# ebiggers/libdeflate

Hardware: AMD Instinct MI355X
Metric: compress+decompress MB/s, 64 KiB chunks level 6 (higher is better)
Workload: dtype u8

## Files before the change

libdeflate_amd/csrc/deflate_huffman.h:

```cpp

template <int N, typename W = u32> struct huff_scratch {
	W A[N];
	W NW[N];
	W P[N];
	u32 cntI[40];
	u32 cnt[40];
	u32 start[16];
	u32 nc[16];
	u16 S[2 * N];
};

#ifdef LDA_SMALL
typedef huff_scratch<288, u16> huff_litlen_t;
#define HUFF_LITLEN(L) ((huff_litlen_t *)(L)->nxtA)
static_assert(sizeof(((struct deflate_lds *)0)->nxtA) >= sizeof(huff_litlen_t) &&
	      sizeof(((struct deflate_lds *)0)->M) >= 2048 && RING + 1 < 65536,
	      "the staging area holds the litlen tree's scratch, M[] the keys");
#else
typedef huff_scratch<288, u32> huff_litlen_t;
#define HUFF_LITLEN(L) ((huff_litlen_t *)((L)->M + 512))
static_assert(sizeof(((struct deflate_lds *)0)->M) >= 2048 + sizeof(huff_litlen_t),
	      "M[] holds the block-end scratch");
#endif

template <int N, typename W> static __device__ void
make_code(const u32 *freq, u32 n, u32 maxlen, u8 *lens, u16 *codes,
	  u16 *sorted, huff_scratch<N, W> *H, u32 used, bool presorted, u32 lane)
{
	PROF_DECL;
	PROF_START();
	__builtin_amdgcn_s_setprio(3);
	for (u32 s = lane; s < n; s += 64)
		lens[s] = 0;
	if (!presorted) {
		used = 0;
		for (u32 s0 = 0; s0 < n; s0 += 64) {
			u32 s = s0 + lane;
			u32 f = s < n ? freq[s] : 0;
			used += __builtin_popcountll(__ballot(f != 0));
		}
		for (u32 s = lane; s < n; s += 64) {
			u32 f = freq[s];
			if (!f)
				continue;
			u32 key = (f << 9) | s, rank = 0;
			for (u32 t = 0; t < n; t++) {
				u32 ft = freq[t];
				rank += (ft != 0) & (((ft << 9) | t) < key);
			}
			sorted[rank] = (u16)s;
		}
	}
	wave_sync();
	const u32 m = used;
	if (m < 2) {
		if (lane == 0) {
			u32 s = m ? sorted[0] : 0;
			u32 other = s ? 0 : 1;
			lens[s] = 1;
			lens[other] = 1;
			for (u32 d = 0; d < 16; d++)
				H->cnt[d] = 0;
			H->cnt[1] = 2;
		}
		wave_sync();
	} else {
		for (u32 i = lane; i < m; i += 64)
			H->A[i] = freq[sorted[i]];
		if (lane < 40)
			H->cntI[lane] = 0;
		wave_sync();
		if (N == 288) PROF_MARK(13);
		u32 leaf = 0, node = 0, made = 0;
#define MERGE_ROUNDS 40u
		if (m >= 24) {
			const u32 INF = 0x7FFFFFFFu;
			for (u32 round = 0; round < MERGE_ROUNDS && made + 1 < m; round++) {
				const u32 wl0 = leaf < m ? H->A[leaf] : INF;
				const u32 wl1 = leaf + 1 < m ? H->A[leaf + 1] : INF;
				const u32 wn0 = node < made ? H->NW[node] : INF;
				const u32 wn1 = node + 1 < made ? H->NW[node + 1] : INF;
				u32 T = wl0 + wl1;
				T = wl0 + wn0 < T ? wl0 + wn0 : T;
				T = wn0 + wn1 < T ? wn0 + wn1 : T;
				u32 cl = 0;
				for (u32 b0 = leaf; b0 < m; b0 += 64) {
					const u32 i = b0 + lane;
					const u32 c = (u32)__builtin_popcountll(__ballot(i < m && H->A[i] <= T));
					cl += c;
					if (c < 64)
						break;
				}
				u32 cn = made - node;
				if ((cl + cn) & 1) {
					if (cn && (cl == 0 || H->NW[node + cn - 1] >= H->A[leaf + cl - 1]))
						cn--;
					else
						cl--;
				}
				const u32 tot = cl + cn;
				for (u32 k = lane; k < tot; k += 64)
					H->S[k] = 0xFFFF;
				wave_sync();
				const u32 wnode = lane < cn ? H->NW[node + lane] : 0;
				const u32 cn64 = cn < 64 ? cn : 64;
				for (u32 i0 = 0; i0 < cl; i0 += 64) {
					const u32 i = i0 + lane;
					const u32 wv = i < cl ? H->A[leaf + i] : 0;
					u32 r = i;
					for (u32 j = 0; j < cn64; j++)
						r += bcast_lane(wnode, j) < wv;
					for (u32 j = 64; j < cn; j++)
						r += H->NW[node + j] < wv;
					if (i < cl)
						H->S[r] = (u16)i;
				}
				wave_sync();
				u32 nfree = 0;
				for (u32 k0 = 0; k0 < tot; k0 += 64) {
					const u32 k = k0 + lane;
					const bool fr = k < tot && H->S[k] == 0xFFFF;
					const u64 mk = __ballot(fr);
					if (fr)
						H->S[k] = (u16)(0x8000u | (nfree + rank_below(mk)));
					nfree += (u32)__builtin_popcountll(mk);
				}
				wave_sync();
				for (u32 q = lane; q < tot / 2; q += 64) {
					const u32 a = H->S[2 * q], b = H->S[2 * q + 1];
					const u32 wa = a & 0x8000 ? H->NW[node + (a & 0x7FFF)] : H->A[leaf + a];
					const u32 wb = b & 0x8000 ? H->NW[node + (b & 0x7FFF)] : H->A[leaf + b];
					if (a & 0x8000)
						H->P[node + (a & 0x7FFF)] = made + q;
					if (b & 0x8000)
						H->P[node + (b & 0x7FFF)] = made + q;
					H->NW[made + q] = wa + wb;
				}
				wave_sync();
				leaf += cl;
				node += cn;
				made += tot / 2;
			}
		}
		if (lane == 0 && made + 1 < m) {
			u32 wl = leaf < m ? H->A[leaf] : 0xFFFFFFFFu;
			u32 wn = node < made ? H->NW[node] : 0xFFFFFFFFu;
			for (u32 k = made; k + 1 < m; k++) {
				u32 w;
				if (leaf < m && wl <= wn) {
					w = wl;
					leaf++;
					wl = leaf < m ? H->A[leaf] : 0xFFFFFFFFu;
				} else {
					w = wn;
					H->P[node] = k;
					node++;
					wn = node < k ? H->NW[node] : 0xFFFFFFFFu;
				}
				if (leaf < m && wl <= wn) {
					w += wl;
					leaf++;
					wl = leaf < m ? H->A[leaf] : 0xFFFFFFFFu;
				} else {
					w += wn;
					H->P[node] = k;
					node++;
					wn = node < k ? H->NW[node] : 0xFFFFFFFFu;
				}
				H->NW[k] = w;
				if (node == k)
					wn = w;
			}
		}
		wave_sync();
		if (N == 288) PROF_MARK(14);
		{
			const u32 root = m - 2;
			enum { NJ = (N + 63) / 64 };
			u32 dd[NJ], hh[NJ];
#pragma unroll
			for (u32 j = 0; j < NJ; j++) {
				u32 k = lane + 64 * j;
				dd[j] = (k < root) ? 1 : 0;
				hh[j] = (k < root) ? H->P[k] : root;
			}
			wave_sync();
#pragma unroll
			for (u32 j = 0; j < NJ; j++) {
				u32 k = lane + 64 * j;
				if (k <= root) {
					H->NW[k] = dd[j];
					H->A[k] = hh[j];
				}
			}
			wave_sync();
			for (u32 r = 0; r < 6; r++) {
#pragma unroll
				for (u32 j = 0; j < NJ; j++) {
					u32 k = lane + 64 * j;
					if (k <= root) {
						u32 h = H->A[k];
						dd[j] = H->NW[k] + H->NW[h];
						hh[j] = H->A[h];
					}
				}
				wave_sync();
#pragma unroll
				for (u32 j = 0; j < NJ; j++) {
					u32 k = lane + 64 * j;
					if (k <= root) {
						H->NW[k] = dd[j];
						H->A[k] = hh[j];
					}
				}
				wave_sync();
			}
#pragma unroll
			for (u32 j = 0; j < NJ; j++) {
				u32 k = lane + 64 * j;
				if (k <= root)
					atomicAdd((u32 *)&H->cntI[dd[j] < 39 ? dd[j] : 39], 1u);
			}
			wave_sync();
			if (lane < 40)
				H->cnt[lane] = lane ? 2 * H->cntI[lane - 1] - H->cntI[lane] : 0;
			wave_sync();
		}
		if (N == 288) PROF_MARK(15);
		if (lane == 0) {
			u32 over = 0;
			for (u32 d = maxlen + 1; d < 40; d++) {
				over += H->cnt[d];
				H->cnt[maxlen] += H->cnt[d];
				H->cnt[d] = 0;
			}
			if (over) {
				u32 kraft = 0;
				for (u32 d = 1; d <= maxlen; d++)
					kraft += H->cnt[d] << (maxlen - d);
				while (kraft > (1u << maxlen)) {
					u32 d = maxlen - 1;
					while (H->cnt[d] == 0)
						d--;
					H->cnt[d]--;
					H->cnt[d + 1] += 2;
					H->cnt[maxlen]--;
					kraft -= 1;
				}
			}
			u32 at = 0;
			for (u32 d = maxlen; d >= 1; d--) {
				H->start[d] = at;
				at += H->cnt[d];
			}
		}
		wave_sync();
		for (u32 i = lane; i < m; i += 64) {
			u32 d = 1;
			for (u32 q = 2; q <= maxlen; q++)
				if (H->cnt[q] && i >= H->start[q] &&
				    i < H->start[q] + H->cnt[q])
					d = q;
			lens[sorted[i]] = (u8)d;
		}
		wave_sync();
	}
	if (N == 288) PROF_MARK(17);
	if (lane == 0) {
		u32 code = 0;
		H->nc[0] = 0;
		for (u32 d = 1; d < 16; d++) {
			code = (code + (d > 1 ? H->cnt[d - 1] : 0)) << 1;
			H->nc[d] = code;
		}
	}
	wave_sync();
	{
		u32 run[16];
#pragma unroll
		for (u32 d = 1; d < 16; d++)
			run[d] = H->nc[d];
		for (u32 s0 = 0; s0 < n; s0 += 64) {
			u32 s = s0 + lane;
			u32 l = s < n ? lens[s] : 0;
			u32 mycode = 0;
#pragma unroll
			for (u32 d = 1; d < 16; d++) {
				u64 mm = __ballot(l == d);
				if (l == d)
					mycode = run[d] + __builtin_popcountll(mm & ((1ull << lane) - 1));
				run[d] += __builtin_popcountll(mm);
			}
			if (s < n)
				codes[s] = l ? (u16)(__brev(mycode) >> (32 - l)) : 0;
		}
	}
	wave_sync();
	__builtin_amdgcn_s_setprio(0);
}
```

libdeflate_amd/csrc/deflate_kernel.hip:

```cpp
#include <stddef.h>
#include "device_common.h"
#include "kernels.h"


#ifndef NT
#define NT LDA_DEFLATE_THREADS
#endif
#define VPT (1024 / NT)
#define NWAVES (NT / 64)
#ifndef TILE
#define TILE 4096
#endif
#ifndef RING
#define RING 32768u
#endif
#define RMASK (RING - 1)
#define LOOKAHEAD 272u
#ifndef HASH_BITS
#define HASH_BITS 13
#endif
#ifndef HASH3_BITS
#define HASH3_BITS 12
#endif
#define MAX_BLOCK_LEN 65536u
#define TOK_MATCH 0x80000000u
#define TOK_TILE_MAX (TILE + 8)
#define TOK_CAP (MAX_BLOCK_LEN + 2 * TILE + 64)
#define SEQ_GCAP (TOK_CAP / 2)
#define SEQ_STRIDE (SEQ_GCAP + (TILE + 8) / 2 + 320 + 256 + (TILE + 8) / 2)
#define S3_WALK 8
#define S3_EVMIN 1u
#define S3_TAIL 256u
#define S3_CLAIM 24u
#define S3_RA_DEPTH 2u
#define S6_ALWAYS_FLUSH 0
#define S3_HALF_SHIFT 1
#define S3_HALF 1
#define P1_PASSES 0xFFFFFFFFu
#ifdef LDA_SMALL
#define RB_DEFER 0
#define RA_PAIR 0
#else
#define RB_DEFER 1
#define RA_PAIR 1
#endif
#define RB_TAIL_WAVES 8u
static_assert(!RB_DEFER || RB_TAIL_WAVES + 3 <= NWAVES,
	      "wave 0 parses, the last two waves insert: the tail waves lie between them");
#define S3_ROUNDS 1u
#ifndef WQ_CAP
#define WQ_CAP 2048u
#endif
#define WQ_SEG (WQ_CAP / NWAVES)
#define RA_PREF_TAIL NWAVES
#define ABSH(o, pos) (pos)
#define WQ_LIMIT WQ_CAP
#define NXT_ELEMS (2 * WQ_CAP + 8)
#define STG_WORDS (NXT_ELEMS / 2 - 8)

#define M_VALID 0x40000u

struct deflate_lds {
	u8 in[RING + 32];
	u16 prev[RING];
	u16 head[1u << HASH_BITS];
	u16 head3[(1u << HASH3_BITS) + 2];
	u32 M[TILE + 8];
	u64 dhalf[TILE / 64];
	u64 dfull[TILE / 64];
	u8 seen8[256];
	u32 freq[320];
	union {
		struct {
			u8 lens[320];
			u16 codes[320];
			u16 sorted[288];
			u32 hw[288];
			u16 pre_items[320 + 8];
			u32 pre_freq[19];
			u8 pre_lens[20];
			u16 pre_codes[20];
		};
		u16 nxtB[NXT_ELEMS];
	};
	u16 nxtA[NXT_ELEMS] __attribute__((aligned(16)));
	u32 scan[2][NWAVES + 1];
	u32 carry[6];
	u32 obs[1][10];
	u32 vars[24] __attribute__((aligned(16)));
	u64 pm[TILE / 64];
	u64 lit1[TILE / 64];
	u64 lit2[TILE / 64];
	u64 pmA[TILE / 64];
	u64 lit1A[TILE / 64];
	u64 lit2A[TILE / 64];
	u32 qn[4];
	u32 gbase[TILE / 64];
	u32 rdy[TILE / 64 + 1];
	u8 lslot[256];
};

#ifdef __HIP_DEVICE_COMPILE__
#define AS3 __attribute__((address_space(3)))
#else
#define AS3
#endif
typedef AS3 struct deflate_lds lds_t;

#ifdef LDA_SMALL
static_assert(sizeof(struct deflate_lds) <= 163840 / SMALL_WGS, "SMALL_WGS workgroups per CU");
static_assert(RING >= TILE && NXT_ELEMS * 2 >= 3600, "the whole buffer is resident; block-end tables fit nxtB");
#else
static_assert(sizeof(struct deflate_lds) <= 163840, "LDS of one CU");
static_assert(NXT_ELEMS == TILE + 8, "levels 10-12 keep one u16 per position in nxtA");
#endif
static_assert(offsetof(struct deflate_lds, in) == 0, "ld32/ld64 assume in[] at LDS offset 0");
#define PREV_OFF ((u32)offsetof(struct deflate_lds, prev))

enum {
	V_NSEQ = 0, V_ENTRY, V_WALKPOS_LO, V_SPLIT, V_TMP0, V_TMP1, V_TMP2,
	V_TMP3, V_CTR, V_MINLEN, V_NPRE, V_NSEQ_PRE, V_WPOS_PRE, V_FIT, V_UNUSED0,
	V_CTR2, V_PFLAG, V_CTR3, V_STDONE, V_EMDONE, V_TAILDONE, V_CTR4, V_ST2DONE,
	V_COUNT
};
static_assert(V_COUNT <= sizeof(((struct deflate_lds *)0)->vars) / sizeof(u32), "vars[] holds them all");

#define DC_SHALLOW 0
#define DC_HALF 1
#define DC_FULL 2

struct level_params {
	u32 depth;
	u32 nice;
	u32 mode;
};


#define LDS32(byteoff) (*(const __attribute__((address_space(3))) u32 *)(uintptr_t)(byteoff))
#define LDS16(byteoff) (*(const __attribute__((address_space(3))) u16 *)(uintptr_t)(byteoff))

static __device__ __forceinline__ u32 ld32(const AS3 u8 *ring, u32 pos)
{
	(void)ring;
	u32 o = pos & RMASK, i = o & ~3u;
	return __builtin_amdgcn_alignbyte(LDS32(i + 4), LDS32(i), ABSH(o, pos));
}

static __device__ __forceinline__ u64 ld64(const AS3 u8 *ring, u32 pos)
{
	(void)ring;
	u32 o = pos & RMASK, i = o & ~3u;
	u32 a = LDS32(i), b = LDS32(i + 4), c = LDS32(i + 8);
	u32 lo = __builtin_amdgcn_alignbyte(b, a, ABSH(o, pos));
	u32 hi = __builtin_amdgcn_alignbyte(c, b, ABSH(o, pos));
	return ((u64)hi << 32) | lo;
}

static __device__ __forceinline__ u32 hash3(u32 w)
{
	return ((w & 0xFFFFFFu) * 0x1E35A7BDu) >> (32 - HASH3_BITS);
}

static __device__ __forceinline__ u32 hash4(u32 w)
{
	return (w * 0x1E35A7BDu) >> (32 - HASH_BITS);
}

struct deflate_lds;
static __device__ u32
find_len3(const lds_t *L, u32 p, u32 cur, u32 c3_16, u32 dmax,
	  u32 dlim, u32 *best);

static __device__ __forceinline__ bool lane_bit(u64 uniform_mask)
{
	return __builtin_amdgcn_inverse_ballot_w64(uniform_mask);
}

static __device__ __forceinline__ u32 rank_below(u64 uniform_mask)
{
	return __builtin_amdgcn_mbcnt_hi((u32)(uniform_mask >> 32),
					 __builtin_amdgcn_mbcnt_lo((u32)uniform_mask, 0));
}

static __device__ u32 block_scan(lds_t *L, u32 v, u32 *total)
{
	const u32 lane = threadIdx.x & 63, wave = threadIdx.x >> 6;
	u32 incl = wave_scan_incl(v);

	if (lane == 63)
		L->scan[0][wave] = incl;
	__syncthreads();
	const u32 sw = lane < NWAVES ? L->scan[0][lane] : 0;
	const u32 iw = wave_scan_incl(sw);
	const u32 base = bcast_lane(iw - sw, wave);
	__syncthreads();
	*total = bcast_lane(iw, NWAVES - 1);
	return base + incl - v;
}

static __device__ u32 block_scan1(lds_t *L, u32 v, u32 *total,
				  u32 *tog)
{
	const u32 lane = threadIdx.x & 63, wave = threadIdx.x >> 6;
	u32 incl = wave_scan_incl(v);
	u32 *sc = L->scan[*tog];

	*tog ^= 1;
	if (lane == 63)
		sc[wave] = incl;
	__syncthreads();
	const u32 sw = lane < NWAVES ? sc[lane] : 0;
	const u32 iw = wave_scan_incl(sw);
	*total = bcast_lane(iw, NWAVES - 1);
	return bcast_lane(iw - sw, wave) + incl - v;
}

static __device__ __forceinline__ void
length_code(u32 len, u32 *slot, u32 *xbits, u32 *xval)
{
	u32 l = len - 3;
	if (l < 8) {
		*slot = l; *xbits = 0; *xval = 0;
	} else if (len == 258) {
		*slot = 28; *xbits = 0; *xval = 0;
	} else {
		u32 hb = 31 - __builtin_clz(l);
		*xbits = hb - 2;
		*slot = 4 * (hb - 1) + ((l >> (hb - 2)) & 3);
		*xval = l & ((1u << (hb - 2)) - 1);
	}
}

static __device__ __forceinline__ void
dist_code(u32 dist, u32 *slot, u32 *xbits, u32 *xval)
{
	u32 d = dist - 1;
	if (d < 4) {
		*slot = d; *xbits = 0; *xval = 0;
	} else {
		u32 hb = 31 - __builtin_clz(d);
		*xbits = hb - 1;
		*slot = 2 * hb + ((d >> (hb - 1)) & 1);
		*xval = d & ((1u << (hb - 1)) - 1);
	}
}

static __device__ u32 choose_min_len(u32 used_literals, u32 depth)
{
	u32 m = used_literals >= 80 ? 3 : used_literals >= 45 ? 4 :
		used_literals >= 16 ? 5 : used_literals >= 10 ? 6 :
		used_literals >= 8 ? 7 : used_literals >= 6 ? 8 : 9;
	if (depth < 16) {
		u32 cap = depth < 5 ? 4 : depth < 10 ? 5 : 7;
		if (m > cap)
			m = cap;
	}
	return m;
}

static __device__ __forceinline__ u32
min_len_policy(u32 distinct, u32 nbytes, u32 depth, bool use3)
{
	const u32 ml = nbytes < 512 ? 3 : choose_min_len(distinct, depth);

	return use3 || ml > 4 ? ml : 4;
}

static __device__ u32
find_len3(const lds_t *L, u32 p, u32 cur, u32 c3_16, u32 dmax,
	  u32 dlim, u32 *best)
{
	if (dmax > dlim)
		dmax = dlim;
	if (p >= 8) {
		const u64 w8 = ld64(L->in, p - 8);
		const u32 A = (u32)w8, B = (u32)(w8 >> 32);
		const u32 cur3 = cur & 0xFFFFFFu;
		u32 bd = 0;
#define LEN3_TRY(d, hi, lo, sel) bd = __builtin_amdgcn_perm(hi, lo, sel) == cur3 ? (d) : bd
		LEN3_TRY(8, A, A, 0x0C020100u);
		LEN3_TRY(7, A, A, 0x0C030201u);
		LEN3_TRY(6, B, A, 0x0C040302u);
		LEN3_TRY(5, B, A, 0x0C050403u);
		LEN3_TRY(4, B, B, 0x0C020100u);
		LEN3_TRY(3, B, B, 0x0C030201u);
		LEN3_TRY(2, cur, B, 0x0C040302u);
		LEN3_TRY(1, cur, B, 0x0C050403u);
#undef LEN3_TRY
		if (bd && bd <= dmax) {
			*best = 3;
			return bd;
		}
	}
	u32 d = (p - c3_16) & 0xFFFF;
	if (d && d <= dmax && ((ld32(L->in, p - d) ^ cur) & 0xFFFFFFu) == 0) {
		*best = 3;
		return d;
	}
	return 0;
}

static __device__ __forceinline__ u32
token_step(u32 m0, u32 m1, u32 m2, u32 mode, u32 nice)
{
	const u32 l0 = m0 & 0xFFFF, l1 = m1 & 0xFFFF, l2 = m2 & 0xFFFF;
	if (mode == 0)
		return l0 ? l0 : 1;
	const s32 z0 = (s32)__builtin_clz((m0 >> 16) | 1), z1 = (s32)__builtin_clz((m1 >> 16) | 1),
		  z2 = (s32)__builtin_clz((m2 >> 16) | 1);
	const bool lazy = mode >= 1 && l0 < nice;
	const bool c1 = lazy && l1 >= l0 && 4 * (s32)(l1 - l0) + (z1 - z0) > 2;
	const bool c2 = lazy && mode >= 2 && l2 >= l0 && 4 * (s32)(l2 - l0) + (z2 - z0) > 6;
	u32 st = c2 ? 2 : l0;
	st = c1 ? 1 : st;
	return l0 == 0 ? 1 : st;
}

#include "deflate_opt.h"
#include "deflate_huffman.h"


struct outstate {
	u8 *out;
	u64 avail;
	u64 sg;
	u64 bits;
};

static __device__ __forceinline__ u32 *stg_of(lds_t *L)
{
	return (u32 *)L->nxtA;
}

static __device__ __forceinline__ void
stg_put(lds_t *L, const struct outstate *os, u64 bitpos, u64 code,
	u32 nbits)
{
	if (!nbits)
		return;
	u64 rel = bitpos - 8 * os->sg;
	u32 w = (u32)(rel >> 5), s = (u32)rel & 31;
	u32 *stg = stg_of(L);
	u64 lo = code << s;
	atomicOr((u32 *)&stg[w], (u32)lo);
	if (s + nbits > 32)
		atomicOr((u32 *)&stg[w + 1], (u32)(lo >> 32));
	if (s + nbits > 64)
		atomicOr((u32 *)&stg[w + 2], (u32)(code >> (64 - s)));
}

static __device__ __forceinline__ void
stg_flush(lds_t *L, struct outstate *os, bool final)
{
	u32 *stg = stg_of(L);
	u8 *stgb = (u8 *)stg;
	const u32 tid = threadIdx.x;
	u64 done_bytes = final ? (os->bits + 7) / 8 : os->bits / 8;
	u64 rel_end = done_bytes - os->sg;
	s64 first = -(s64)os->sg;
	u32 start = first > 0 ? (u32)first : 0;
	u32 units = final ? (u32)((rel_end + 15) / 16) : (u32)(rel_end / 16);

	__syncthreads();
	for (u32 u = tid; u < units; u += NT) {
		u32 b0 = u * 16, b1 = b0 + 16;
		u8 *g = os->out + (s64)(os->sg + b0);
		if (b0 >= start && b1 <= rel_end) {
			*(uint4 *)g = *(const uint4 *)(stgb + b0);
		} else {
			for (u32 b = b0 < start ? start : b0; b < b1 && b < rel_end; b++)
				g[b - b0] = stgb[b];
		}
	}
	u32 keep_from = units * 16;
	u32 total_words = (u32)((os->bits - 8 * os->sg + 31) / 32) + 1;
	u32 keep_words = final ? 0 : total_words - keep_from / 4;
	u32 v = 0;
	if (tid < keep_words && keep_from / 4 + tid < STG_WORDS + 8)
		v = stg[keep_from / 4 + tid];
	__syncthreads();
	for (u32 i = tid; i < STG_WORDS + 8; i += NT)
		stg[i] = 0;
	if (tid < keep_words)
		stg[tid] = v;
	os->sg += keep_from;
}

static __device__ __forceinline__ void stg_restore(lds_t *L)
{
	u32 *stg = stg_of(L);

	__syncthreads();
	for (u32 i = threadIdx.x; i < STG_WORDS + 8; i += NT)
		stg[i] = i < 6 ? L->carry[i] : 0;
	__syncthreads();
}

static __device__ __forceinline__ void stg_save(lds_t *L, struct outstate *os)
{
	stg_flush(L, os, false);
	if (threadIdx.x < 6)
		L->carry[threadIdx.x] = stg_of(L)[threadIdx.x];
	__syncthreads();
}


static __device__ __forceinline__ u32 lds_mskor_rtn(u32 byteaddr, u32 mask, u32 val)
{
	u32 old;
	asm volatile("ds_mskor_rtn_b32 %0, %1, %2, %3"
		     : "=v"(old) : "v"(byteaddr), "v"(mask), "v"(val) : "memory");
	return old;
}

static __device__ __forceinline__ void lds_wait8(u32 *o)
{
	asm volatile("s_waitcnt lgkmcnt(0)"
		     : "+v"(o[0]), "+v"(o[1]), "+v"(o[2]), "+v"(o[3]),
		       "+v"(o[4]), "+v"(o[5]), "+v"(o[6]), "+v"(o[7]) :: "memory");
}

#define HEAD_OFF ((u32)offsetof(struct deflate_lds, head))
#define HEAD3_OFF ((u32)offsetof(struct deflate_lds, head3))

#define MH_H3_SHIFT 19
#define MH_V3 0x80000000u

static __device__ __forceinline__ void
insert_tile(lds_t *L, u32 t, u32 tend, u32 n, u32 lane)
{
	const u32 ngroups = (tend - t + 63) / 64;

	for (u32 g0 = 0; g0 < ngroups; g0 += 8) {
		u32 o[8], sh[8], wv[8];
#pragma unroll
		for (u32 k = 0; k < 8; k++)
			wv[k] = ld32(L->in, t + (g0 + k) * 64 + lane);
#pragma unroll
		for (u32 k = 0; k < 8; k++) {
			const u32 p = t + (g0 + k) * 64 + lane;
			const u32 h = hash4(wv[k]);
			const bool ok = g0 + k < ngroups && p + 4 <= n;
			sh[k] = (h & 1) << 4;
			o[k] = lds_mskor_rtn(HEAD_OFF + ((h >> 1) << 2),
					     ok ? 0xFFFFu << sh[k] : 0,
					     ok ? (p & 0xFFFF) << sh[k] : 0);
		}
		lds_wait8(o);
#pragma unroll
		for (u32 k = 0; k < 8; k++) {
			const u32 i = (g0 + k) * 64 + lane;
			L->prev[(t + i) & RMASK] = (u16)(o[k] >> sh[k]);
		}
	}
}

static __device__ __forceinline__ void
insert_tile3(lds_t *L, u16 *__restrict__ c3, u32 t, u32 tend, u32 n, u32 lane)
{
	const u32 ngroups = (tend - t + 63) / 64;
	AS3 u16 *const h3tab = (AS3 u16 *)L->head3;

	for (u32 g0 = 0; g0 < ngroups; g0 += 8) {
		u32 wv[8], v[8];
#pragma unroll
		for (u32 k = 0; k < 8; k++)
			wv[k] = ld32(L->in, t + (g0 + k) * 64 + lane);
#pragma unroll
		for (u32 k = 0; k < 8; k++) {
			const u32 p = t + (g0 + k) * 64 + lane;
			const bool ok = g0 + k < ngroups && p + 3 <= n;
			const u32 slot = ok ? hash3(wv[k]) : (1u << HASH3_BITS);
			v[k] = h3tab[slot];
			h3tab[slot] = (u16)p;
			v[k] = ok ? v[k] : 0x8000;
		}
#pragma unroll
		for (u32 k = 0; k < 8; k++)
			c3[4 + (g0 + k) * 64 + lane] = (u16)v[k];
	}
}

static __device__ __forceinline__ u32 claim_issue(u32 lds_byteaddr)
{
	u32 r;
	u64 save;
	asm volatile("s_mov_b64 %1, exec\n\ts_mov_b64 exec, 1\n\tds_add_rtn_u32 %0, %2, %3\n\ts_mov_b64 exec, %1"
		     : "=&v"(r), "=&s"(save) : "v"(lds_byteaddr), "v"(1u) : "memory");
	return r;
}

static __device__ __forceinline__ u32 claim_get(u32 r)
{
	u32 g;
	asm volatile("s_waitcnt lgkmcnt(0)\n\tv_readfirstlane_b32 %0, %1"
		     : "=s"(g) : "v"(r) : "memory");
	return g;
}

static __device__ __forceinline__ void lds_add_lane0(u32 lds_byteaddr, u32 v)
{
	u64 save;
	asm volatile("s_mov_b64 %0, exec\n\ts_mov_b64 exec, 1\n\tds_add_u32 %1, %2\n\ts_mov_b64 exec, %0"
		     : "=&s"(save) : "v"(lds_byteaddr), "v"(v) : "memory");
}
#define VAR_ADDR(idx) ((u32)offsetof(struct deflate_lds, vars) + 4 * (idx))


#define RAW(i, k) LDS32((i) + (k))
#define AB(hi, lo, sh) __builtin_amdgcn_alignbyte((hi), (lo), (sh))
#define HAVE4(a, b, c, d) asm volatile("" :: "v"(a), "v"(b), "v"(c), "v"(d))
static __device__ __forceinline__ u64 mk64(u32 lo, u32 hi)
{
	return ((u64)hi << 32) | lo;
}

static __device__ __forceinline__ u32
match_length(const lds_t *L, bool ev, u32 p, u32 cp, u32 cur, u64 nxt8,
	       u32 maxlen, u32 lane)
{
	(void)L;
	const u32 op = p & RMASK, ip = op & ~3u, sp = op & 3;
	const u32 oc = cp & RMASK, ic = oc & ~3u, sc = oc & 3;
	const u32 b0 = RAW(ic, 0), b1 = RAW(ic, 4), b2 = RAW(ic, 8), b3 = RAW(ic, 12);
	const u64 x = nxt8 ^ mk64(AB(b2, b1, sc), AB(b3, b2, sc));
	u32 len = 4 + ((u32)__builtin_ctzll(x | (1ull << 63)) >> 3);
	ev = ev && AB(b1, b0, sc) == cur;
	bool more = ev && x == 0 && 12 < maxlen;
	if (__ballot(more)) {
		const u32 p3 = RAW(ip, 12), p4 = RAW(ip, 16), p5 = RAW(ip, 20);
		const u32 b4 = RAW(ic, 16), b5 = RAW(ic, 20);
		HAVE4(p3, p5, b4, b5);
		const u64 y = mk64(AB(p4, p3, sp), AB(p5, p4, sp)) ^ mk64(AB(b4, b3, sc), AB(b5, b4, sc));
		if (more) {
			len = 12 + ((u32)__builtin_ctzll(y | (1ull << 63)) >> 3);
			more = y == 0 && 20 < maxlen;
		}
		if (__ballot(more)) {
			const u32 p6 = RAW(ip, 24), p7 = RAW(ip, 28);
			const u32 b6 = RAW(ic, 24), b7 = RAW(ic, 28);
			HAVE4(p6, p7, b6, b7);
			const u64 z = mk64(AB(p6, p5, sp), AB(p7, p6, sp)) ^
				      mk64(AB(b6, b5, sc), AB(b7, b6, sc));
			if (more) {
				len = 20 + ((u32)__builtin_ctzll(z | (1ull << 63)) >> 3);
				more = z == 0 && 28 < maxlen;
			}
		}
	}
	for (u64 mm = __ballot(more); mm; mm &= mm - 1) {
		u32 src = (u32)__builtin_ctzll(mm);
		u32 bp = bcast_lane(p, src);
		u32 bc = bcast_lane(cp, src);
		u32 bmax = bcast_lane(maxlen, src);
		u32 off = 28 + 4 * lane;
		u32 x4 = 1;
		if (off < bmax) {
			const u32 o1 = (bp + off) & RMASK, i1 = o1 & ~3u;
			const u32 o2 = (bc + off) & RMASK, i2 = o2 & ~3u;
			const u32 w0 = RAW(i1, 0), w1 = RAW(i1, 4), v0 = RAW(i2, 0), v1 = RAW(i2, 4);
			x4 = AB(w1, w0, o1 & 3) ^ AB(v1, v0, o2 & 3);
		}
		u64 ne = __ballot(x4 != 0);
		u32 tot = bmax;
		if (ne) {
			u32 kk = (u32)__builtin_ctzll(ne);
			u32 xk = bcast_lane(x4, kk);
			u32 o = 28 + 4 * kk;
			if (o < bmax)
				tot = o + ((u32)__builtin_ctz(xk) >> 3);
		}
		if (lane == src)
			len = tot;
	}
	if (len > maxlen)
		len = maxlen;
	return ev ? len : 0;
}

template <class F> static __device__ __forceinline__ void
match_length2_p(const lds_t *L, bool ev1, bool ev2, u32 p, u32 cp1, u32 cp2, u32 cur,
		u64 nxt8, u32 maxlen, u32 lane, u32 *len1o, u32 *len2o, F &&hook)
{
	(void)L;
	const u32 op = p & RMASK, ip = op & ~3u, sp = op & 3;
	const u32 o1 = cp1 & RMASK, i1 = o1 & ~3u, s1 = o1 & 3;
	const u32 o2 = cp2 & RMASK, i2 = o2 & ~3u, s2 = o2 & 3;
	const u32 b0 = RAW(i1, 0), b1 = RAW(i1, 4), b2 = RAW(i1, 8), b3 = RAW(i1, 12);
	const u32 e0 = RAW(i2, 0), e1 = RAW(i2, 4), e2 = RAW(i2, 8), e3 = RAW(i2, 12);
	hook();
	const u64 x1 = nxt8 ^ mk64(AB(b2, b1, s1), AB(b3, b2, s1));
	const u64 x2 = nxt8 ^ mk64(AB(e2, e1, s2), AB(e3, e2, s2));
	u32 len1 = 4 + ((u32)__builtin_ctzll(x1 | (1ull << 63)) >> 3);
	u32 len2 = 4 + ((u32)__builtin_ctzll(x2 | (1ull << 63)) >> 3);
	ev1 = ev1 && AB(b1, b0, s1) == cur;
	ev2 = ev2 && AB(e1, e0, s2) == cur;
	bool m1 = ev1 && x1 == 0 && 12 < maxlen, m2 = ev2 && x2 == 0 && 12 < maxlen;
	if (__ballot(m1 || m2)) {
		const u32 p3 = RAW(ip, 12), p4 = RAW(ip, 16), p5 = RAW(ip, 20);
		const u32 b4 = RAW(i1, 16), b5 = RAW(i1, 20);
		const u32 e4 = RAW(i2, 16), e5 = RAW(i2, 20);
		HAVE4(p3, p5, b4, b5);
		HAVE4(p4, e4, e5, e5);
		const u64 pw = mk64(AB(p4, p3, sp), AB(p5, p4, sp));
		const u64 y1 = pw ^ mk64(AB(b4, b3, s1), AB(b5, b4, s1));
		const u64 y2 = pw ^ mk64(AB(e4, e3, s2), AB(e5, e4, s2));
		if (m1) {
			len1 = 12 + ((u32)__builtin_ctzll(y1 | (1ull << 63)) >> 3);
			m1 = y1 == 0 && 20 < maxlen;
		}
		if (m2) {
			len2 = 12 + ((u32)__builtin_ctzll(y2 | (1ull << 63)) >> 3);
			m2 = y2 == 0 && 20 < maxlen;
		}
		if (__ballot(m1 || m2)) {
			const u32 p6 = RAW(ip, 24), p7 = RAW(ip, 28);
			const u32 b6 = RAW(i1, 24), b7 = RAW(i1, 28);
			const u32 e6 = RAW(i2, 24), e7 = RAW(i2, 28);
			HAVE4(p6, p7, b6, b7);
			HAVE4(e6, e7, e7, e7);
			const u64 pz = mk64(AB(p6, p5, sp), AB(p7, p6, sp));
			const u64 z1 = pz ^ mk64(AB(b6, b5, s1), AB(b7, b6, s1));
			const u64 z2 = pz ^ mk64(AB(e6, e5, s2), AB(e7, e6, s2));
			if (m1) {
				len1 = 20 + ((u32)__builtin_ctzll(z1 | (1ull << 63)) >> 3);
				m1 = z1 == 0 && 28 < maxlen;
			}
			if (m2) {
				len2 = 20 + ((u32)__builtin_ctzll(z2 | (1ull << 63)) >> 3);
				m2 = z2 == 0 && 28 < maxlen;
			}
		}
	}
#pragma unroll
	for (u32 c = 0; c < 2; c++) {
		const u32 cp = c ? cp2 : cp1;
		for (u64 mm = __ballot(c ? m2 : m1); mm; mm &= mm - 1) {
			u32 src = (u32)__builtin_ctzll(mm);
			u32 bp = bcast_lane(p, src);
			u32 bc = bcast_lane(cp, src);
			u32 bmax = bcast_lane(maxlen, src);
			u32 off = 28 + 4 * lane;
			u32 x4 = 1;
			if (off < bmax) {
				const u32 oa = (bp + off) & RMASK, ia = oa & ~3u;
				const u32 ob = (bc + off) & RMASK, ib = ob & ~3u;
				const u32 w0 = RAW(ia, 0), w1 = RAW(ia, 4), v0 = RAW(ib, 0), v1 = RAW(ib, 4);
				x4 = AB(w1, w0, oa & 3) ^ AB(v1, v0, ob & 3);
			}
			u64 ne = __ballot(x4 != 0);
			u32 tot = bmax;
			if (ne) {
				u32 kk = (u32)__builtin_ctzll(ne);
				u32 xk = bcast_lane(x4, kk);
				u32 o = 28 + 4 * kk;
				if (o < bmax)
					tot = o + ((u32)__builtin_ctz(xk) >> 3);
			}
			if (lane == src) {
				if (c)
					len2 = tot;
				else
					len1 = tot;
			}
		}
	}
	if (len1 > maxlen)
		len1 = maxlen;
	if (len2 > maxlen)
		len2 = maxlen;
	*len1o = ev1 ? len1 : 0;
	*len2o = ev2 ? len2 : 0;
}

static __device__ __forceinline__ u32
wave_distinct_bytes(lds_t *L, u32 t0, u32 lim, u32 lane)
{
	AS3 u32 *const s32p = (AS3 u32 *)L->seen8;

	s32p[lane] = 0;
	wave_sync();
#pragma unroll
	for (u32 j = 0; j < TILE / 1024; j++) {
		const u32 off = (TILE / 64) * lane + 16 * j;
		const uint4 v = *(const AS3 uint4 *)&L->in[(t0 + off) & RMASK];
		const u32 w[4] = { v.x, v.y, v.z, v.w };
#pragma unroll
		for (u32 i = 0; i < 16; i++)
			if (off + i < lim)
				L->seen8[(w[i >> 2] >> (8 * (i & 3))) & 0xFF] = 1;
	}
	wave_sync();
	return wave_sum((u32)__builtin_popcount(s32p[lane] & 0x01010101u));
}

static __device__ __forceinline__ void
stage_input(lds_t *L, const u8 *__restrict__ inp, u32 loaded, u32 want,
	    bool aligned_in, u32 tid)
{
	if (aligned_in) {
		const u32 from = loaded & ~15u;
		for (u32 p = from + tid * 16; p < want; p += NT * 16) {
			uint4 v = *(const uint4 *)(inp + p);
			*(uint4 *)&L->in[p & RMASK] = v;
			if ((p & RMASK) < 32)
				*(uint4 *)&L->in[RING + (p & RMASK)] = v;
		}
// ... 608 lines not shown
								bestd = m >> 16;
							}
						} else {
							dep = my_i >= TILE - S3_TAIL ? drain : depth;
						}
						best0 = best;
						boff = best - 3;
						curb = boff ? ld32(L->in, p + boff) : cur;
						dprev = 0;
						cnt = 0;
						ended = false;
						have = true;
						if (best >= maxlen) {
							have = false;
							fin = true;
						}
					} else {
						fin = true;
						best = best0 = 3;
					}
				}
			}
			PROF_SEC(0);
			continue;
		}
#pragma unroll
		for (int s = 0; s < S3_WALK; s++) {
			u32 d = (p - c16) & 0xFFFF;
			bool chain = dep && d > dprev && d <= dmaxp;
			bool stall = ended || cnt >= 4;
			bool ok = !stall && chain;
			u32 cp = p - d;
			u32 w = ld32(L->in, cp + boff);
			u32 c16n = LDS16(PREV_OFF + 2 * (cp & RMASK));
			bool hit = ok && w == curb;
			c16 = ok ? c16n : c16;
			dprev = ok ? d : dprev;
			dep -= ok ? 1 : 0;
			ended = ended || (!stall && !chain);
			q = hit ? ((q << 16) | d) : q;
			cnt += hit ? 1 : 0;
		}
		if (!have)
			cnt = 0;
		PROF_SEC(1);
		bool done = false;
		u32 nev = __builtin_popcountll(__ballot(cnt > 0));
		u32 nwalk = __builtin_popcountll(__ballot(have && !ended && cnt < 4));
		while (nev && (nev >= S3_EVMIN || !nwalk)) {
			bool ev = cnt > 0;
			u32 d = (u32)(q >> (16 * ((cnt - 1) & 3))) & 0xFFFF;
			cnt -= ev ? 1 : 0;
			u32 len = match_length(L, ev, p, p - d, cur, nxt8, maxlen, lane);
			if (ev && len > best) {
				best = len;
				bestd = d;
				if (len >= nice || len >= maxlen) {
					done = true;
					cnt = 0;
				} else {
					boff = len - 3;
					curb = ld32(L->in, p + boff);
				}
			}
			if (have && (done || (ended && cnt == 0))) {
				have = false;
				fin = true;
				done = false;
			}
			nev = __builtin_popcountll(__ballot(cnt > 0));
			nwalk = __builtin_popcountll(__ballot(have && !ended && cnt < 4));
		}
		if (have && ended && cnt == 0) {
			have = false;
			fin = true;
		}
		PROF_SEC(2);
	}
	PROF_SEC_FLUSH(17);
}

#ifdef LDA_PROFILE
#define PROF_GEN(g) do { if (threadIdx.x == 0) { unsigned long long n_ = __builtin_readcyclecounter(); \
	atomicAdd(&lda_prof[35 + ((g) < 3 ? (g) : 3)], n_ - pg_); pg_ = n_; } } while (0)
#else
#define PROF_GEN(g) do { } while (0)
#endif
static __device__ __forceinline__ u32 rb_trim_depth(u32 depth)
{
	const u32 npass = depth >= 256 ? 4 : depth >= 32 ? 2 : 1;
	const u32 quantum = 8 * npass;
	for (u32 g = 1, end = quantum; end < depth; g++, end += quantum * g)
		if (depth - end <= depth / 8)
			depth = end;
	if (depth >= 16 && (depth & 7) <= depth / 8)
		depth &= ~7u;
	return depth;
}

static __device__ __forceinline__ void
rb_gen_params(u32 depth, u32 gen, u32 *before, u32 *npass_g)
{
	const u32 npass = depth >= 256 ? 4 : depth >= 32 ? 2 : 1;
	const u32 quantum = 8 * npass;
	*npass_g = npass * (gen + 1);
	*before = quantum * (gen * (gen + 1) / 2);
}

static __device__ __forceinline__ bool
rb_batch(lds_t *L, u32 t, u32 n, u32 lo_pos, u32 min_len, u32 depth, u32 nice,
	 u32 e, bool have, u32 gen, u32 lane, u32 *next)
{
	const u32 half = depth >> S3_HALF_SHIFT ? depth >> S3_HALF_SHIFT : 1;
	u32 before, npass_g;
	rb_gen_params(depth, gen, &before, &npass_g);
	const u32 qg = 8 * npass_g;
	const u32 i = e & 0xFFF, p = t + i;
	const u32 cdepth = ((e >> 12) & 3) == DC_FULL ? depth : half;
	u32 dep = before < cdepth ? cdepth - before : 0;
	dep = dep < qg ? dep : qg;
	u32 dprev = gen ? (p - (e >> 16)) & 0xFFFF : 0;
	u32 c16 = LDS16(PREV_OFF + 2 * ((p - dprev) & RMASK));
	const u32 m = L->M[4 + i], l0 = m & 0xFFFF;
	const u32 cur = ld32(L->in, p);
	const u64 nxt8 = ld64(L->in, p + 4);
	const u32 maxlen = n - p < 258 ? n - p : 258;
	const u32 dmaxp = p - lo_pos;
	const u32 nic = nice < maxlen ? nice : maxlen;
	u32 best = l0 >= 4 ? l0 : 3, bestd = l0 >= 4 ? m >> 16 : 0;
	const u32 best0 = best;
	u32 boff = best - 3;
	u32 curb = ld32(L->in, p + boff);
	bool act = have && p + 4 <= n && best < nic && dep;
	u64 endm = 0;
	for (u32 ps = 0; ps < npass_g; ps++) {
		u64 h1 = 0, h2 = 0;
		u32 qh = 0, nok = 0;
		const u32 dep0 = dep;
		const u64 actm = __ballot(act);
#pragma unroll
		for (int s = 0; s < 8; s++) {
			u32 d, c16x2;
			asm("v_sub_u16 %0, %1, %2" : "=v"(d) : "v"(p), "v"(c16));
			if (RING == 32768u)
				asm("v_lshlrev_b16 %0, 1, %1" : "=v"(c16x2) : "v"(c16));
			else
				c16x2 = 2 * (c16 & RMASK);
			const u64 chainm = __ballot(dep0 > (u32)s) & __ballot(d > dprev) &
					   __ballot(d <= dmaxp);
			const u64 stallm = endm | h2;
			const u64 okm = actm & ~stallm & chainm;
			const u32 w = ld32(L->in, c16 + boff);
			const u32 c16n = LDS16(PREV_OFF + c16x2);
			const u64 hitm = okm & __ballot(w == curb);
			const bool ok = lane_bit(okm);
			c16 = ok ? c16n : c16;
			dprev = ok ? d : dprev;
			nok = ok ? (u32)s + 1 : nok;
			endm |= actm & ~stallm & ~chainm;
			qh = lane_bit(hitm) ? ((qh << 16) | d) : qh;
			h2 |= h1 & hitm;
			h1 |= hitm;
			PROF_COUNT(20, __builtin_popcountll(okm));
			PROF_COUNT(17, __builtin_popcountll(hitm));
		}
		PROF_COUNT(13, __builtin_popcountll(__ballot(have)));
		PROF_COUNT(21, (h1 != 0) + (h2 != 0));
		dep = dep0 - nok;
		if (h1) {
			const bool ev = lane_bit(h1);
			const u32 d = lane_bit(h2) ? qh >> 16 : qh & 0xFFFF;
			const u32 len = match_length(L, ev, p, p - d, cur, nxt8, maxlen, lane);
			if (ev && len > best) {
				best = len;
				bestd = d;
			}
		}
		if (h2) {
			const bool ev = lane_bit(h2);
			const u32 d = qh & 0xFFFF;
			const u32 len = match_length(L, ev, p, p - d, cur, nxt8, maxlen, lane);
			if (ev && len > best) {
				best = len;
				bestd = d;
			}
		}
		if (best >= nic)
			act = false;
		if (npass_g > 1) {
			if (!__ballot(act && !lane_bit(endm) && dep))
				break;
			boff = best - 3;
			curb = ld32(L->in, p + boff);
		}
	}
	const bool ended = lane_bit(endm);
	if (best > best0)
		L->M[4 + i] = best >= min_len ? best | (bestd << 16) : 0;
	*next = (e & 0x3FFF) | (((p - dprev) & 0xFFFF) << 16);
	return act && !ended && before + qg < cdepth;
}

static __device__ __forceinline__ void
search_queue(lds_t *L, u32 t, u32 n, u32 lo_pos, u32 min_len, u32 depth,
	     u32 nice, AS3 u32 *WA, AS3 u32 *WB, u32 wc, u32 tid,
	     bool defer, u32 *tail_n, u32 *tail_gen, AS3 u32 **tail_list)
{
	const u32 lane = tid & 63, wave = tid >> 6;
	depth = rb_trim_depth(depth);
	const u64 lt = (1ull << lane) - 1;
	u32 ncur = wc;
#ifdef LDA_PROFILE
	unsigned long long pg_ = __builtin_readcyclecounter();
#endif

	*tail_n = 0;
	PROF_COUNT(15, wc);
	PROF_COUNT(18, 1);
	for (u32 gen = 0;; gen++) {
		PROF_COUNT(16, 1);
		PROF_COUNT(14, (ncur + 63) / 64);
		PROF_COUNT(19, ncur);
		AS3 u32 *cur_l = gen & 1 ? WB : WA, *nxt_l = gen & 1 ? WA : WB;
		AS3 u32 *ctr = &L->qn[gen % 3];
		u32 before, npass_g;
		rb_gen_params(depth, gen, &before, &npass_g);
		if (RB_DEFER && defer && gen && before + 8 * npass_g >= depth &&
		    ncur <= 64 * RB_TAIL_WAVES) {
			*tail_n = ncur;
			*tail_gen = gen;
			*tail_list = cur_l;
			return;
		}
		if (tid == 0)
			L->qn[(gen + 1) % 3] = 0;
		for (u32 base = 64 * wave; base < ncur; base += 64 * NWAVES) {
			const bool have = base + lane < ncur;
			const u32 e = have ? cur_l[base + lane] : 0;
			u32 nx;
			const bool surv = rb_batch(L, t, n, lo_pos, min_len, depth, nice, e, have,
						   gen, lane, &nx);
			const u64 b = __ballot(surv);
			u32 at = 0;
			if (lane == 0 && b)
				at = atomicAdd((u32 *)ctr, (u32)__builtin_popcountll(b));
			at = bcast_first(at);
			if (surv)
				nxt_l[at + __builtin_popcountll(b & lt)] = nx;
		}
		__syncthreads();
		PROF_GEN(gen);
		ncur = bcast_first(*(volatile AS3 u32 *)ctr);
		if (!ncur)
			break;
	}
}

static __device__ __forceinline__ void
split_stats(lds_t *L, u32 walkpos, u32 block_start, bool fit_split, u32 lane)
{
	static_assert(TOK_TILE_MAX < (1u << 13) && TOK_CAP < (1u << 17), "32-bit products");
	AS3 u32 *const acc = (AS3 u32 *)&L->scan[1][0];
	if (lane < 10)
		acc[lane] = 0;
	wave_sync();
#pragma unroll
	for (u32 j = 0; j < 4; j++)
		atomicAdd((u32 *)&acc[2 * j + (lane & 1)], L->freq[lane + 64 * j]);
	if (lane < 29)
		atomicAdd((u32 *)&acc[8 + (lane >= 6)], L->freq[257 + lane]);
	wave_sync();
	const u32 now = lane < 10 ? acc[lane] : 0;
	const u32 prev = lane < 10 ? L->obs[0][lane] : 0;
	const u32 d = now - prev;
	const u32 nprev = row16_sum(prev), nnew = row16_sum(d);
	const u32 a = d * nprev, e = prev * nnew;
	const u32 df = a > e ? a - e : e - a;
	const u64 delta = ((u64)row16_sum(df >> 16) << 16) + row16_sum(df & 0xFFFF);
	bool sp = nprev && walkpos - block_start >= 5000 &&
		  delta >= (u64)nnew * 200 / 512 * nprev;
	if (fit_split && walkpos - block_start >= 5000)
		sp = true;
	wave_sync();
	if (lane < 10)
		L->obs[0][lane] = sp ? 0 : now;
	if (lane == 0)
		L->vars[V_SPLIT] = !sp ? 0 :
			L->vars[V_WPOS_PRE] - block_start >= 5000 ? 2 : 1;
}

#ifdef LDA_DEBUG_SPLIT
static __device__ u32 lda_dbg[2048];
extern "C" __attribute__((visibility("default"))) void libdeflate_amd_debug_read(u32 *out)
{
	(void)hipDeviceSynchronize();
	(void)hipMemcpyFromSymbol(out, HIP_SYMBOL(lda_dbg), sizeof(lda_dbg));
}
#define DBG(tile, k, v) do { if ((tile) < 250) lda_dbg[8 * (tile) + (k)] = (v); } while (0)
#else
#define DBG(tile, k, v) do { } while (0)
#endif


template <bool OPT> static __device__ __forceinline__ void
deflate_batch_body(u8 *lds_raw, u64 n_chunks, int format, int level, u32 depth,
		   u32 nice, u32 mode,
		   const u8 *__restrict__ in_base,
		   const u64 *__restrict__ in_offsets,
		   const u64 *__restrict__ in_nbytes,
		   u8 *__restrict__ out_base,
		   const u64 *__restrict__ out_offsets,
		   const u64 *__restrict__ out_avail_arr,
		   u64 *__restrict__ out_nbytes,
		   const u32 *__restrict__ sums,
		   u64 *__restrict__ seq_scratch,
		   const u32 *__restrict__ seg_info,
		   u32 *__restrict__ next_chunk,
		   const u8 *__restrict__ dict_pre)
{
	lds_t *L = (lds_t *)(uintptr_t)0;
	const u32 tid = threadIdx.x;
	if ((u32)(uintptr_t)(__attribute__((address_space(3))) u8 *)lds_raw != 0)
		__builtin_trap();
	u64 *__restrict__ seqg = seq_scratch + (size_t)blockIdx.x * SEQ_STRIDE;
	u32 *__restrict__ tokg = (u32 *)seqg;
	u32 *__restrict__ msave = (u32 *)(seqg + SEQ_GCAP);
	u32 *__restrict__ fsave = msave + TILE + 8;
	u32 *__restrict__ bsave = fsave + 640;
	u16 *__restrict__ c3g = (u16 *)(bsave + 512);
	u32 tog = 0;
	PROF_DECL;

	for (u32 i = tid; i < 256; i += NT) {
		u32 sl, xb, xv;
		length_code(i + 3, &sl, &xb, &xv);
		L->lslot[i] = (u8)sl;
	}
	for (;;) {
		__syncthreads();
		if (tid == 0)
			L->vars[V_TMP0] = atomicAdd(next_chunk, 1u);
		__syncthreads();
		const u64 c = bcast_first(L->vars[V_TMP0]);
		if (c >= n_chunks)
			break;
		const u8 *inp = in_base + in_offsets[c];
		u64 n64 = in_nbytes[c];
		const u32 sinfo = dict_pre ? (n64 ? ((const u32 *)dict_pre)[0] : 0x80000000u) :
				  seg_info ? seg_info[c] : 0x80000000u;
		const u32 dict_len = sinfo & 0xFFFFu;
		const u32 lo_min = (sinfo >> 16) & 0x7FFFu;
		const bool seg_last = sinfo >> 31;
		const u32 pre_len = dict_pre ? dict_len : 0;
		inp -= pre_len;
		n64 += pre_len;
		struct outstate os;
		os.out = out_base + out_offsets[c];
		os.avail = out_avail_arr[c];
		const u32 hdr_bytes = format == LDA_FMT_GZIP ? 10 :
				      format == LDA_FMT_ZLIB ? (dict_pre ? 6 : 2) : 0;
		const u32 ftr_bytes = format == LDA_FMT_GZIP ? 8 :
				      format == LDA_FMT_ZLIB ? 4 : 0;
		bool overflow = false;

		if (os.avail <= hdr_bytes + ftr_bytes && (hdr_bytes + ftr_bytes))
			overflow = true;
		if (n64 > 0xFFFFFF00u)
			overflow = true;
#ifdef LDA_SMALL
		if (n64 > RING)
			overflow = true;
#endif
		const u32 n = (u32)n64;

		__syncthreads();
		PROF_START();
		for (u32 i = tid; i < (1u << HASH_BITS) / 2; i += NT)
			((u32 *)L->head)[i] = 0x80008000u;
		for (u32 i = tid; i < (1u << HASH3_BITS) / 2; i += NT)
			((u32 *)L->head3)[i] = 0x80008000u;
		for (u32 i = tid; i < 320; i += NT)
			L->freq[i] = 0;
		if (tid < 10)
			L->obs[0][tid] = 0;
		if (tid < TILE / 64 + 1)
			L->rdy[tid] = 0;
		for (u32 i = tid; i < STG_WORDS + 8; i += NT)
			stg_of(L)[i] = 0;
		if (tid < 8)
			L->M[tid] = 0;
		if (tid == 0) {
			L->vars[V_NSEQ] = 0;
			L->vars[V_ENTRY] = 0;
			L->vars[V_PFLAG] = 0;
		}
		os.sg = (u64)(0 - ((uintptr_t)os.out & 15));
		os.bits = 0;
		__syncthreads();

		if (!overflow && hdr_bytes) {
			if (tid == 0) {
				if (format == LDA_FMT_GZIP) {
					u32 xfl = level < 2 ? 4 : level >= 8 ? 2 : 0;
					stg_put(L, &os, 0, 0x00088B1Full, 32);
					stg_put(L, &os, 32, 0, 32);
					stg_put(L, &os, 64, xfl | (0xFFu << 8), 16);
				} else {
					u32 fl = level < 2 ? 0 : level < 6 ? 1 :
						 level < 8 ? 2 : 3;
					u32 h = (0x78u << 8) | (fl << 6);
					if (dict_pre) {
						h |= 0x20;
						h += (31 - h % 31) % 31;
						stg_put(L, &os, 16, __builtin_bswap32(((const u32 *)dict_pre)[1]), 32);
					} else {
						h |= 31 - (h % 31);
					}
					stg_put(L, &os, 0, ((h & 0xFF) << 8) | (h >> 8), 16);
				}
			}
			os.bits = 8 * hdr_bytes;
		}
		__syncthreads();
		stg_save(L, &os);

		u32 loaded = 0;
		u32 block_start = dict_len;
		u32 walkpos = dict_len;
		const bool aligned_in = ((uintptr_t)inp & 15) == 0;

		const bool stored_only = level == 0 ||
			n - dict_len <= (u32)(55 - 4 * (level > 12 ? 12 : level));
		u32 num_tiles = (n + TILE - 1) / TILE;
		if (num_tiles == 0)
			num_tiles = 1;
		if (pre_len && !stored_only && !overflow) {
			stage_prefix(L, dict_pre + 64, pre_len, tid);
			loaded = pre_len;
		}

		const bool ra_all = depth <= 4;
		const bool optm = OPT && mode == 3;
		const u32 rounds = optm || ra_all ? 0 : S3_ROUNDS;
		const u32 dlim3 = mode ? 8192u : 4096u;
		const u32 ra_depth = ra_all ? depth : S3_RA_DEPTH;
		const u32 ra_class = ra_all ? DC_FULL :
				     ra_depth >= (depth >> S3_HALF_SHIFT) ? DC_HALF : DC_SHALLOW;
		const u32 wq_limit = mode == 1 && depth < 100 && WQ_LIMIT > 64 * NWAVES ?
				     64 * NWAVES : WQ_LIMIT;
		const bool use3 = level >= 2;
		const bool splits = use3 && n - dict_len >= 5000;
		bool mx_pending = false;
		u32 tail_n = 0, tail_gen = 0, tail_e = 0;
		u32 ml_cur = 3, ml_nxt = 3;
		u32 carryv = 0;

		for (u32 it = 0; it <= num_tiles && !overflow; it++) {
			const bool have_cur = it >= 1;
			const u32 tile = it - 1;
			const u32 t = have_cur ? tile * TILE : 0;
			const u32 tend = t + TILE < n ? t + TILE : n;
			const bool last_tile = it == num_tiles;
			const bool cur_real = have_cur && t >= dict_len;
			const u32 tn = it * TILE;
			const u32 tnend = tn + TILE < n ? tn + TILE : n;
			const bool nxt_real = it < num_tiles && tn >= dict_len;
			const bool have_ins = it + 1 < num_tiles;
			u32 tid_opaque = threadIdx.x;
			asm volatile("" : "+v"(tid_opaque));
			const u32 tid = tid_opaque, lane = tid & 63, wave = tid >> 6;

			PROF_MARK(0);
			if (stored_only) {
				if (!cur_real)
					continue;
				walkpos = tend;
			} else {
				AS3 u32 *const MX = (AS3 u32 *)L->nxtB;
#ifdef LDA_SMALL
				const u32 lo_cur = 0, lo_nxt = 0;
				(void)lo_min;
#else
				const s32 lo_s = (s32)(t + 2 * TILE + LOOKAHEAD) - (s32)RING;
				const u32 lo_cur = lo_s > (s32)lo_min ? (u32)lo_s : lo_min;
				const s32 lo_n = (s32)(tn + 2 * TILE + LOOKAHEAD) - (s32)RING;
				const u32 lo_nxt = lo_n > (s32)lo_min ? (u32)lo_n : lo_min;
#endif
				u16 *c3nxt = c3g + (it & 1) * (TILE + 8);
				u16 *c3ins = c3g + ((it + 1) & 1) * (TILE + 8);
				const s32 limit = last_tile ? (s32)(tend - t) : (s32)TILE - 2;

				const bool wl_copies = cur_real && !optm && rounds && mx_pending;
				if (cur_real) {
					if (mx_pending && !wl_copies)
						for (u32 i = tid; i < TILE; i += NT)
							L->M[4 + i] = MX[4 + i];
					if (tid < 4) {
						L->M[tid] = carryv;
						L->M[TILE + 4 + tid] = 0;
					}
					mx_pending = false;
					ml_cur = ml_nxt;
					for (u32 i = tid; i < 320; i += NT)
						fsave[i] = L->freq[i];
					if (tid == 0) {
						L->vars[V_NSEQ_PRE] = L->vars[V_NSEQ];
						L->vars[V_WPOS_PRE] = walkpos;
					}
					if (!wl_copies)
						__syncthreads();
					PROF_MARK(6);
				}
				const u32 s0_want0 = (it + 2) * TILE + LOOKAHEAD;
				const u32 s0_want = s0_want0 < n ? s0_want0 : n;
				const u32 s0_p = (loaded & ~15u) + tid * 16;
				const bool s0_pre = aligned_in && s0_p < s0_want;
				uint4 s0_v = make_uint4(0, 0, 0, 0);
				if (s0_pre)
					s0_v = *(const uint4 *)(inp + s0_p);
				tail_n = 0;
				if (cur_real && !optm) {
					if (rounds) {
						const u32 wc = build_worklist(L, (AS3 u32 *)L->nxtB,
									      wl_copies ? (const AS3 u32 *)MX : NULL,
									      mode, nice, wq_limit, tid);
						PROF_MARK(39);
						if (wc) {
							AS3 u32 *tl = (AS3 u32 *)L->nxtB;
							search_queue(L, t, n, lo_cur, ml_cur, depth, nice,
								     (AS3 u32 *)L->nxtB, (AS3 u32 *)L->nxtA, wc, tid,
								     nxt_real, &tail_n, &tail_gen, &tl);
							if (tail_n && wave >= 1 && wave <= RB_TAIL_WAVES) {
								const u32 k = 64 * (wave - 1) + lane;
								tail_e = k < tail_n ? tl[k] : 0;
							}
						}
						PROF_MARK(3);
					}
					if (!tail_n)
						stage_steps(L, limit, mode, nice, tid);
				}
				if (cur_real && optm) {
					const bool opt_first = walkpos == block_start;
					const u32 opt_last = level >= 11 ? 2 : 1;
					u32 opt_stage = 0;
					const u32 ent0 = L->vars[V_ENTRY], nseq0 = L->vars[V_NSEQ];
					if (opt_first) {
						for (u32 i = tid; i < TILE + 8; i += NT)
							msave[i] = L->M[i];
						if (tid == 0)
							L->vars[V_FIT] = 0;
					} else {
						const u32 fit = opt_build_costs(L, tid, false, true, t, tend - t, bsave);
						opt_stage = fit ? 0 : 1;
						if (tid == 0) {
							L->vars[V_FIT] = fit;
							if (c == 0) {
								DBG(tile, 6, 100 + fit);
								DBG(tile, 7, L->vars[V_TMP3]);
							}
						}
					}
					for (;;) {
						u32 tid_opaque2 = threadIdx.x;
						asm volatile("" : "+v"(tid_opaque2));
						const u32 tid = tid_opaque2, lane = tid & 63, wave = tid >> 6;
						const u32 s4mode = opt_stage ? 0 : 2;
						if (opt_stage) {
							const s32 ent = (s32)ent0;
							const s32 pend = (s32)(tend - t);
							s32 lo = (s32)(OPT_SEG * wave), hi = lo + OPT_SEG;
							if (wave == 0 && ent < 0)
								lo = ent;
							if (hi > limit)
								hi = limit;
							s32 e = hi + OPT_WARM;
							if (e > pend)
								e = pend;
							if (lo < hi)
								opt_parse_wave(L, L->nxtA, t, lo, hi, e, lane);
							__syncthreads();
							for (s32 i = (s32)tid + (ent < 0 ? ent : 0); i < limit; i += NT) {
								u32 c = L->nxtA[i + 4], m = L->M[i + 4];
								L->M[i + 4] = c >= 3 ? c | (m & 0xFFFF0000u) : 0;
							}
							__syncthreads();
						}
						stage_steps(L, limit, s4mode, nice, tid);
						if (tid == 0)
							L->vars[V_CTR2] = 0;
						__syncthreads();
						if (wave == 0)
							parse_and_base(L, tokg, t, limit, s4mode, nice, lane);
						__syncthreads();
						PROF_MARK(12);
						emit_groups(L, tokg, t, lane);
						__syncthreads();
						PROF_MARK(5);
						if (!opt_first || opt_stage == opt_last)
							break;
						opt_build_costs(L, tid, opt_stage == 0, false, t, tend - t, bsave);
						for (u32 i = tid; i < 320; i += NT)
							L->freq[i] = 0;
						for (u32 i = tid; i < TILE + 8; i += NT)
							L->M[i] = msave[i];
						if (tid == 0) {
							L->vars[V_ENTRY] = ent0;
							L->vars[V_NSEQ] = nseq0;
						}
						__syncthreads();
						opt_stage++;
					}
				}

				{
					const u32 want = s0_want;
					if (s0_pre) {
						*(uint4 *)&L->in[s0_p & RMASK] = s0_v;
						if ((s0_p & RMASK) < 32)
							*(uint4 *)&L->in[RING + (s0_p & RMASK)] = s0_v;
					}
					if (aligned_in) {
						if ((loaded & ~15u) + NT * 16 < want)
							stage_input(L, inp, (loaded & ~15u) + NT * 16, want, true, tid);
					} else {
						stage_input(L, inp, loaded, want, false, tid);
					}
					loaded = want > loaded ? want : loaded;
					if (tid == 0) {
						L->vars[V_CTR] = 0;
						L->vars[V_CTR2] = 0;
						L->vars[V_CTR3] = 0;
						L->vars[V_STDONE] = 0;
						L->vars[V_EMDONE] = 0;
						L->vars[V_TAILDONE] = 0;
						L->vars[V_CTR4] = 0;
						L->vars[V_ST2DONE] = 0;
					}
					if (tid < 4 && nxt_real) {
						AS3 u32 *const Mo = cur_real ? MX : (AS3 u32 *)L->M;
						if (!tail_n)
							Mo[tid] = cur_real ? L->M[TILE + tid] : 0;
						Mo[TILE + 4 + tid] = 0;
					}
					if (nxt_real && it)
						ml_nxt = bcast_first(L->vars[V_MINLEN]);
					__syncthreads();
				}
				PROF_MARK(1);
				if (it == 0) {
					if (wave == NWAVES - 1)
						insert_tile(L, 0, tnend, n, lane);
					if (wave == NWAVES - 2 && use3) {
						insert_tile3(L, c3nxt, 0, tnend, n, lane);
						__builtin_amdgcn_fence(__ATOMIC_RELEASE, "workgroup");
					}
					if (wave == NWAVES - 3 && nxt_real) {
						const u32 nd = wave_distinct_bytes(L, 0, loaded < TILE ? loaded : TILE, lane);
						if (lane == 0)
							L->vars[V_MINLEN] = min_len_policy(nd, n - dict_len, depth, use3);
					}
					__syncthreads();
					if (nxt_real)
						ml_nxt = bcast_first(L->vars[V_MINLEN]);
					PROF_MARK(2);
				}
				__builtin_amdgcn_fence(__ATOMIC_ACQUIRE, "workgroup");

				{
					const bool do_p2 = cur_real && !optm;
					AS3 u32 *const Mo = cur_real ? MX : (AS3 u32 *)L->M;
					PROF_WDECL;
					PROF_W0();
					if (wave == NWAVES - 1) {
						__builtin_amdgcn_s_setprio(3);
						if (have_ins)
							insert_tile(L, tnend, tnend + TILE < n ? tnend + TILE : n,
								    n, lane);
						__builtin_amdgcn_s_setprio(0);
						PROF_W(24);
					} else if (wave == NWAVES - 2) {
						__builtin_amdgcn_s_setprio(2);
						if (have_ins && use3) {
							insert_tile3(L, c3ins, tnend,
								     tnend + TILE < n ? tnend + TILE : n, n, lane);
							__builtin_amdgcn_fence(__ATOMIC_RELEASE, "workgroup");
						}
						__builtin_amdgcn_s_setprio(0);
						if (have_ins && tnend >= dict_len) {
							const u32 nd = wave_distinct_bytes(L, tnend,
								loaded - tnend < TILE ? loaded - tnend : TILE, lane);
							if (lane == 0)
								L->vars[V_MINLEN] = min_len_policy(nd, n - dict_len, depth, use3);
						}
						PROF_W(25);
					} else if (wave == 0 && do_p2) {
						if (tail_n)
							wait_lds_eq(L, V_ST2DONE, TILE / 64);
						__builtin_amdgcn_s_setprio(3);
						parse_and_base(L, tokg, t, limit, mode, nice, lane);
						__builtin_amdgcn_fence(__ATOMIC_RELEASE, "workgroup");
						if (lane == 0)
							*(volatile AS3 u32 *)&L->vars[V_PFLAG] = it;
						__builtin_amdgcn_s_setprio(0);
						if (tail_n && nxt_real && lane < 4)
							Mo[lane] = L->M[TILE + lane];
						PROF_W(26);
					} else if (RB_DEFER && tail_n && wave <= RB_TAIL_WAVES) {
						__builtin_amdgcn_s_setprio(2);
						if (64 * (wave - 1) < tail_n) {
							u32 nx;
							(void)rb_batch(L, t, n, lo_nxt, ml_cur, rb_trim_depth(depth), nice,
								       tail_e, tail_e != 0, tail_gen, lane, &nx);
						}
						__builtin_amdgcn_fence(__ATOMIC_RELEASE, "workgroup");
						if (lane == 0)
							atomicAdd((u32 *)&L->vars[V_TAILDONE], 1u);
						wait_lds_eq(L, V_TAILDONE, RB_TAIL_WAVES);
						stage_steps_cur_claimed(L, limit, mode, nice, lane);
						__builtin_amdgcn_s_setprio(0);
					}
					if (nxt_real) {
						if (optm) {
							if (wave < NWAVES - 2)
								search_items(L, Mo, tn, n, lo_nxt, ml_nxt, depth, nice,
									     NULL, TILE, NWAVES - 2, tid);
						} else {
							round_a(L, Mo, c3nxt, tn, tnend, n, lo_nxt, ml_nxt, ra_depth,
								ra_class, nice, dlim3, it + 1, tid);
						}
					}
					if (wave == 1)
						PROF_W(27);
					if (nxt_real && rounds) {
						const s32 lim_n = it + 1 == num_tiles ? (s32)(tnend - tn) : (s32)TILE - 2;
						stage_steps_claimed(L, Mo, lim_n, mode, nice, it + 1, lane);
						if (wave == 0) {
							u64 mk;
							wait_lds_eq(L, V_STDONE, TILE / 64);
							const u32 e = entry_skip(Mo, (s32)L->vars[V_ENTRY],
										 (u32)(lim_n + 4), mode, nice);
							(void)parse_tile(Mo, (const AS3 u64 *)L->lit1A,
									 (const AS3 u64 *)L->lit2A, (AS3 u64 *)L->pmA,
									 lane, (s32)e - 4, lim_n, &mk, P1_PASSES);
						}
						if (wave == 1)
							PROF_W(33);
						if (wave == 0)
							PROF_W(34);
					}
					if (do_p2) {
						while (*(volatile AS3 u32 *)&L->vars[V_PFLAG] != it)
							__builtin_amdgcn_s_sleep(4);
						__builtin_amdgcn_fence(__ATOMIC_ACQUIRE, "workgroup");
						if (wave == 1)
							PROF_W(28);
						emit_groups(L, tokg, t, lane);
						if (wave == 1)
							PROF_W(29);
						if (wave == NWAVES - 1 && splits && !last_tile) {
							wait_lds_eq(L, V_EMDONE, TILE / 64);
							split_stats(L, bcast_first(L->vars[V_WALKPOS_LO]), block_start, false, lane);
						}
					}
					__syncthreads();
					if (wave == 1)
						PROF_W(30);
					if (wave == 0)
						PROF_W(31);
					if (optm && nxt_real) {
						PROF_MARK(16);
						if (ml_nxt <= 3) {
							for (u32 i = tid; i < TILE; i += NT) {
								u32 p = tn + i, b3 = 0;
								if (p + 3 <= n && Mo[4 + i] == 0) {
									u32 bd = find_len3(L, p, ld32(L->in, p),
											   c3nxt[4 + i], p - lo_nxt,
											   dlim3, &b3);
									if (bd)
										Mo[4 + i] = 3 | (bd << 16);
								}
							}
						}
						__syncthreads();
					}
					mx_pending = cur_real && nxt_real;
				}
				PROF_MARK(4);
				if (!cur_real)
					continue;

				if (OPT && mode == 3)
					walkpos = bcast_first(L->vars[V_WALKPOS_LO]);
				if (tid < 4)
					carryv = L->M[TILE + tid];
				if (splits && wave == NWAVES - 1 && optm) {
					split_stats(L, walkpos, block_start, L->vars[V_FIT] == 2, lane);
				}
			}
			if (OPT && mode == 3)
				__syncthreads();
			PROF_MARK(32);

			u32 splitv, nseq_now;
			if (OPT && mode == 3) {
				splitv = splits && !stored_only && !last_tile ?
					 bcast_first(L->vars[V_SPLIT]) : 0;
				nseq_now = stored_only ? 0 : bcast_first(L->vars[V_NSEQ]);
			} else {
				const uint4 pv = *(const AS3 uint4 *)&L->vars[V_NSEQ];
				static_assert(V_NSEQ == 0 && V_WALKPOS_LO == 2 && V_SPLIT == 3, "one 16-byte read");
				if (!stored_only)
					walkpos = bcast_first(pv.z);
				splitv = splits && !stored_only && !last_tile ? bcast_first(pv.w) : 0;
				nseq_now = stored_only ? 0 : bcast_first(pv.x);
			}
			bool end_block = last_tile || splitv ||
				(!stored_only && nseq_now + 2 * TOK_TILE_MAX > TOK_CAP) ||
				walkpos - block_start > MAX_BLOCK_LEN;
			if (!end_block)
				continue;
			if (tid < 10)
				L->obs[0][tid] = 0;

			const bool retro = splitv == 2;
			const u32 bstart = block_start;
			const u32 bend = last_tile ? n : retro ? bcast_first(L->vars[V_WPOS_PRE]) : walkpos;
			const u32 blen = bend - bstart;
			const u32 nseq_all = nseq_now;
			const u32 nseq = retro ? bcast_first(L->vars[V_NSEQ_PRE]) : nseq_all;
			const u32 is_final = last_tile && seg_last ? 1 : 0;
			if (retro) {
				for (u32 i = tid; i < 320; i += NT) {
					u32 f = L->freq[i], fp = fsave[i];
					fsave[320 + i] = f - fp;
					L->freq[i] = fp;
				}
				__syncthreads();
			}

			u32 btype = 0;
			if (!stored_only) {
				if (mx_pending) {
					const AS3 u32 *MXs = (const AS3 u32 *)L->nxtB;
					for (u32 i = tid; i < TILE; i += NT)
						msave[4 + i] = MXs[4 + i];
				}
				if (tid == 0)
					L->freq[256]++;
				__syncthreads();
				{
					u32 *keys = L->M;
					u32 *usedv = L->M + 320;
					u16 *sortedO = (u16 *)(L->M + 324);
					if (tid < 2)
						usedv[tid] = 0;
					__syncthreads();
					for (u32 vt = tid; vt < 320; vt += NT) {
						const u32 f = L->freq[vt];
						if (f) {
							if (vt < 288)
								keys[atomicAdd(&usedv[0], 1u)] = (f << 9) | vt;
							else
								keys[288 + atomicAdd(&usedv[1], 1u)] =
									(f << 9) | (vt - 288);
						}
					}
					__syncthreads();
					{
						const u32 m1 = usedv[0], m2 = usedv[1];
						for (u32 i = tid; i < m1 + m2; i += NT) {
							const bool lit = i < m1;
							const u32 lo = lit ? 0 : 288, m = lit ? m1 : m2;
							const u32 key = keys[lit ? i : 288 + i - m1];
							u32 r = 0;
							for (u32 q = 0; q < m; q++)
								r += keys[lo + q] < key;
							if (lit)
								L->sorted[r] = (u16)(key & 511);
							else
								sortedO[r] = (u16)(key & 511);
						}
					}
					__syncthreads();
					PROF_MARK(10);
					if (wave == 0)
						make_code(L->freq, 288, 15, L->lens, L->codes,
							  L->sorted, HUFF_LITLEN(L),
							  usedv[0], true, lane);
					else if (wave == 1)
						make_code(L->freq + 288, 32, 15, L->lens + 288,
							  L->codes + 288, sortedO,
							  (huff_scratch<32> *)L->hw,
							  usedv[1], true, lane);
				}
				__syncthreads();
				PROF_MARK(11);
				{
					u32 *starts = L->M;
					if (tid == 0) {
						L->vars[V_TMP1] = 257;
						L->vars[V_TMP2] = 1;
					}
					if (tid < 19)
						L->pre_freq[tid] = 0;
					__syncthreads();
					for (u32 vt = tid; vt < 320; vt += NT) {
						if (vt < 288 && vt >= 257 && L->lens[vt])
							atomicMax((u32 *)&L->vars[V_TMP1], vt + 1);
						if (vt >= 288 && L->lens[vt])
							atomicMax((u32 *)&L->vars[V_TMP2], vt - 288 + 1);
					}
					__syncthreads();
					const u32 nlit = L->vars[V_TMP1], noff = L->vars[V_TMP2];
					const u32 total = nlit + noff;
					u32 isst[VPT], nst = 0;
#pragma unroll
					for (u32 j = 0; j < VPT; j++) {
						const u32 e = tid * VPT + j;
						isst[j] = 0;
						if (e < total) {
							u32 v = L->lens[e < nlit ? e : 288 + (e - nlit)];
							u32 pv = 0xFF;
							if (e)
								pv = L->lens[e - 1 < nlit ? e - 1 :
									     288 + (e - 1 - nlit)];
							isst[j] = pv != v;
						}
						nst += isst[j];
					}
					u32 nruns;
					u32 ridx = block_scan(L, nst, &nruns);
#pragma unroll
					for (u32 j = 0; j < VPT; j++) {
						if (isst[j])
							starts[ridx] = tid * VPT + j;
						ridx += isst[j];
					}
					if (tid == 0)
						starts[nruns] = total;
					__syncthreads();
					u32 rv[VPT], rlen[VPT], nitems[VPT], nit = 0;
#pragma unroll
					for (u32 j = 0; j < VPT; j++) {
						const u32 r = tid * VPT + j;
						rv[j] = rlen[j] = nitems[j] = 0;
						if (r < nruns) {
							u32 st = starts[r];
							rlen[j] = starts[r + 1] - st;
							rv[j] = L->lens[st < nlit ? st : 288 + (st - nlit)];
							if (rv[j] == 0) {
								u32 full = rlen[j] / 138, rem = rlen[j] % 138;
								nitems[j] = full + (rem >= 3 ? 1 : rem);
							} else if (rlen[j] >= 4) {
								u32 l1 = rlen[j] - 1;
								nitems[j] = 1 + l1 / 6 + (l1 % 6 >= 3 ? 1 : l1 % 6);
							} else {
								nitems[j] = rlen[j];
							}
						}
						nit += nitems[j];
					}
					u32 ni;
					u32 at = block_scan(L, nit, &ni);
#pragma unroll
					for (u32 j = 0; j < VPT; j++) {
						if (tid * VPT + j < nruns) {
							u32 left = rlen[j];
							const u32 rvj = rv[j];
							if (rvj == 0) {
								while (left >= 11) {
									u32 r = left > 138 ? 138 : left;
									L->pre_items[at++] = 18 | ((r - 11) << 5);
									atomicAdd((u32 *)&L->pre_freq[18], 1u);
									left -= r;
								}
								if (left >= 3) {
									L->pre_items[at++] = 17 | ((left - 3) << 5);
									atomicAdd((u32 *)&L->pre_freq[17], 1u);
									left = 0;
								}
							} else if (left >= 4) {
								L->pre_items[at++] = (u16)rvj;
								left--;
								u32 n16 = 0;
								while (left >= 3) {
									u32 r = left > 6 ? 6 : left;
									L->pre_items[at++] = 16 | ((r - 3) << 5);
									n16++;
									left -= r;
								}
								atomicAdd((u32 *)&L->pre_freq[16], n16);
								atomicAdd((u32 *)&L->pre_freq[rvj], 1u);
							}
							if (left)
								atomicAdd((u32 *)&L->pre_freq[rvj], left);
							while (left) {
								L->pre_items[at++] = (u16)rvj;
								left--;
							}
						}
					}
					if (tid == 0)
						L->vars[V_NPRE] = ni;
				}
				__syncthreads();
				PROF_MARK(23);
				if (wave == 0)
					make_code(L->pre_freq, 19, 7, L->pre_lens, L->pre_codes,
						  L->sorted, (huff_scratch<32> *)L->hw,
						  0, false, lane);
				__syncthreads();
				PROF_MARK(22);
				u32 dyn = 0, stat = 0;
				for (u32 vt = tid; vt < 320; vt += NT) {
					u32 f = L->freq[vt];
					u32 xb = 0, sl = 8;
					if (vt < 288) {
						sl = vt < 144 ? 8 : vt < 256 ? 9 : vt < 280 ? 7 : 8;
						if (vt >= 265 && vt < 285)
							xb = (vt - 261) >> 2;
					} else {
						u32 ds = vt - 288;
						sl = 5;
						if (ds >= 4)
							xb = (ds >> 1) - 1;
					}
					dyn += f * (L->lens[vt] + xb);
					stat += f * (sl + xb);
				}
				if (tid < 19) {
					u32 xb = tid == 16 ? 2 : tid == 17 ? 3 : tid == 18 ? 7 : 0;
					dyn += L->pre_freq[tid] * (L->pre_lens[tid] + xb);
				}
				u32 dyn_tot, stat_tot;
				(void)block_scan(L, dyn, &dyn_tot);
				(void)block_scan(L, stat, &stat_tot);
				static const u8 perm[19] = { 16, 17, 18, 0, 8, 7, 9, 6, 10,
							     5, 11, 4, 12, 3, 13, 2, 14,
							     1, 15 };
				u32 nexp = 19;
				while (nexp > 4 && L->pre_lens[perm[nexp - 1]] == 0)
					nexp--;
				u32 cost_dyn = 3 + 5 + 5 + 4 + 3 * nexp + dyn_tot;
				u32 cost_stat = 3 + stat_tot;
				u32 pieces = blen ? (blen + 65534) / 65535 : 1;
				u32 pad = (u32)((0 - (os.bits + 3)) & 7);
				u64 cost_stored = 3 + pad + 32 + 8ull * blen +
						  (u64)(pieces - 1) * 40;
				u64 best = cost_stored;
				btype = 0;
				if (cost_stat < best) {
					best = cost_stat;
					btype = 1;
				}
				if (cost_dyn < best) {
					best = cost_dyn;
					btype = 2;
				}
				if ((os.bits + best + 7) / 8 + ftr_bytes > os.avail)
					overflow = true;
				L->vars[V_TMP3] = nexp;
			} else {
				u32 pieces = blen ? (blen + 65534) / 65535 : 1;
				u64 cost = (u64)pieces * 40 + 8ull * blen;
				if ((os.bits + cost + 7) / 8 + ftr_bytes > os.avail)
					overflow = true;
			}
			if (overflow)
				break;

			PROF_MARK(7);
			stg_restore(L);
			if (btype == 0) {
				u32 done = 0;
				do {
					u32 piece = blen - done > 65535 ? 65535 : blen - done;
					u32 fin = (is_final && done + piece == blen) ? 1 : 0;
					u32 pad = (u32)((0 - (os.bits + 3)) & 7);
					if (tid == 0) {
						stg_put(L, &os, os.bits, fin, 3);
						u64 b = os.bits + 3 + pad;
						stg_put(L, &os, b, piece | ((u64)(piece ^ 0xFFFF) << 16), 32);
					}
					os.bits += 3 + pad + 32;
					__syncthreads();
					for (u32 w0 = 0; w0 < piece; w0 += 2048) {
						u32 cnt = piece - w0 < 2048 ? piece - w0 : 2048;
						stg_flush(L, &os, false);
						__syncthreads();
						for (u32 j = tid; j < cnt; j += NT) {
							u32 pos = bstart + done + w0 + j;
							stg_put(L, &os, os.bits + 8ull * j, inp[pos], 8);
						}
						os.bits += 8ull * cnt;
						__syncthreads();
					}
					done += piece;
				} while (done < blen);
				stg_flush(L, &os, false);
			} else {
				if (btype == 1) {
					__syncthreads();
					for (u32 s = tid; s < 320; s += NT)
						L->lens[s] = s < 144 ? 8 : s < 256 ? 9 :
							     s < 280 ? 7 : s < 288 ? 8 : 5;
					__syncthreads();
					if (tid == 0) {
						u32 nc[16] = { 0 }, bl[16] = { 0 };
						for (u32 s = 0; s < 288; s++)
							bl[L->lens[s]]++;
						u32 code = 0;
						for (u32 d = 1; d < 16; d++) {
							code = (code + bl[d - 1]) << 1;
							nc[d] = code;
						}
						for (u32 s = 0; s < 288; s++) {
							u32 l = L->lens[s];
							L->codes[s] = (u16)(__brev(nc[l]++) >> (32 - l));
						}
						for (u32 s = 0; s < 32; s++)
							L->codes[288 + s] = (u16)(__brev(s) >> 27);
					}
					__syncthreads();
				}
				{
					u64 hcode[VPT];
					u32 hbits[VPT], hsum = 0;
					const u32 nexp = btype == 2 ? L->vars[V_TMP3] : 0;
					const u32 ni = btype == 2 ? L->vars[V_NPRE] : 0;
#pragma unroll
					for (u32 j = 0; j < VPT; j++) {
						const u32 vt = tid * VPT + j;
						hcode[j] = 0;
						hbits[j] = 0;
						if (vt == 0) {
							hcode[j] = is_final | (btype << 1);
							hbits[j] = 3;
							if (btype == 2) {
								u32 nlit = L->vars[V_TMP1], noff = L->vars[V_TMP2];
								hcode[j] |= (u64)((nlit - 257) | ((noff - 1) << 5) |
										  ((nexp - 4) << 10)) << 3;
								hbits[j] = 17;
							}
						} else if (vt <= nexp) {
							static const u8 perm2[19] = { 16, 17, 18, 0, 8, 7,
								9, 6, 10, 5, 11, 4, 12, 3, 13, 2, 14, 1, 15 };
							hcode[j] = L->pre_lens[perm2[vt - 1]];
							hbits[j] = 3;
						} else if (vt <= nexp + ni) {
							u32 it = L->pre_items[vt - nexp - 1];
							u32 sym = it & 31, ex = it >> 5;
							u32 l = L->pre_lens[sym];
							u32 xb = sym == 16 ? 2 : sym == 17 ? 3 :
								 sym == 18 ? 7 : 0;
							hcode[j] = L->pre_codes[sym] | ((u64)ex << l);
							hbits[j] = l + xb;
						}
						hsum += hbits[j];
					}
					u32 htot;
					u32 hoff = block_scan(L, hsum, &htot);
#pragma unroll
					for (u32 j = 0; j < VPT; j++) {
						stg_put(L, &os, os.bits + hoff, hcode[j], hbits[j]);
						hoff += hbits[j];
					}
					os.bits += htot;
				}
				stg_flush(L, &os, false);

				PROF_MARK(9);
				__builtin_amdgcn_fence(__ATOMIC_ACQUIRE, "workgroup");
				u32 tok_nxt = tid < nseq ? tokg[tid] : 0;
				for (u32 b0 = 0; b0 < nseq; b0 += NT) {
					u64 code = 0;
					u32 nb = 0;
					const u32 tok = tok_nxt;
					if (b0 + NT + tid < nseq)
						tok_nxt = tokg[b0 + NT + tid];
					if (b0 + tid < nseq) {
						if (tok & TOK_MATCH) {
							const u32 len = (tok & 0xFF) + 3, dist = ((tok >> 8) & 0x7FFF) + 1;
							u32 sl, xb, xv, ds, dxb, dxv;
							length_code(len, &sl, &xb, &xv);
							dist_code(dist, &ds, &dxb, &dxv);
							u32 ll = L->lens[257 + sl];
							u32 dl = L->lens[288 + ds];
							u64 v = L->codes[257 + sl];
							u32 sh = ll;
							v |= (u64)xv << sh;
							sh += xb;
							v |= (u64)L->codes[288 + ds] << sh;
							sh += dl;
							v |= (u64)dxv << sh;
							sh += dxb;
							code = v;
							nb = sh;
						} else {
							code = L->codes[tok];
							nb = L->lens[tok];
						}
					}
					u32 tot;
					u32 off = block_scan1(L, nb, &tot, &tog);
					stg_put(L, &os, os.bits + off, code, nb);
					os.bits += tot;
					if (S6_ALWAYS_FLUSH || os.bits - 8 * os.sg + 48 * NT + 64 > 32 * STG_WORDS)
						stg_flush(L, &os, false);
				}
				stg_flush(L, &os, false);
				__syncthreads();
				if (tid == 0)
					stg_put(L, &os, os.bits, L->codes[256], L->lens[256]);
				os.bits += L->lens[256];
				__syncthreads();
			}

			stg_save(L, &os);
			PROF_MARK(8);
			if (OPT && mode == 3 && tid < 256)
				bsave[tid] = 0;
			if (retro) {
				const u32 cnt = nseq_all - nseq;
				enum { RPT = (TOK_TILE_MAX + NT - 1) / NT };
				u32 mv[RPT];
#pragma unroll
				for (u32 k = 0; k < RPT; k++)
					mv[k] = tid + NT * k < cnt ? tokg[nseq + tid + NT * k] : 0;
				__syncthreads();
#pragma unroll
				for (u32 k = 0; k < RPT; k++)
					if (tid + NT * k < cnt)
						tokg[tid + NT * k] = mv[k];
				for (u32 i = tid; i < 320; i += NT)
					L->freq[i] = fsave[320 + i];
				if (tid == 0)
					L->vars[V_NSEQ] = cnt;
				__builtin_amdgcn_fence(__ATOMIC_RELEASE, "workgroup");
			} else {
				for (u32 i = tid; i < 320; i += NT)
					L->freq[i] = 0;
				if (tid == 0)
					L->vars[V_NSEQ] = 0;
			}
			carryv = 0;
			if (mx_pending) {
				for (u32 i = tid; i < TILE; i += NT)
					L->M[4 + i] = msave[4 + i];
				mx_pending = false;
			}
			block_start = bend;
			__syncthreads();
		}

		__syncthreads();
		if (!overflow && !seg_last &&
		    (os.bits + 3 + 7) / 8 + 4 > os.avail)
			overflow = true;
		if (!overflow) {
			stg_restore(L);
			if (!seg_last) {
				u64 fb = 8 * ((os.bits + 3 + 7) / 8);
				if (tid == 0)
					stg_put(L, &os, fb, 0xFFFF0000ull, 32);
				os.bits = fb + 32;
				__syncthreads();
			}
			if (ftr_bytes) {
				u32 sum = sums ? sums[c] : 0;
				u64 fb = 8 * ((os.bits + 7) / 8);
				if (tid == 0) {
					if (format == LDA_FMT_GZIP) {
						stg_put(L, &os, fb, sum, 32);
						stg_put(L, &os, fb + 32, n, 32);
					} else {
						stg_put(L, &os, fb, __builtin_bswap32(sum), 32);
					}
				}
				os.bits = fb + 8 * ftr_bytes;
				__syncthreads();
			}
			stg_flush(L, &os, true);
			if (tid == 0)
				out_nbytes[c] = (os.bits + 7) / 8;
		} else if (tid == 0) {
			out_nbytes[c] = 0;
		}
		__syncthreads();
	}
}

#define DEFLATE_KERNEL_PARAMS                                                  \
	u64 n_chunks, int format, int level, u32 depth, u32 nice, u32 mode,    \
	const u8 *__restrict__ in_base, const u64 *__restrict__ in_offsets,    \
	const u64 *__restrict__ in_nbytes, u8 *__restrict__ out_base,          \
	const u64 *__restrict__ out_offsets,                                   \
	const u64 *__restrict__ out_avail_arr, u64 *__restrict__ out_nbytes,   \
	const u32 *__restrict__ sums, u64 *__restrict__ seq_scratch,           \
	const u32 *__restrict__ seg_info, u32 *__restrict__ next_chunk,       \
	const u8 *__restrict__ dict_pre
#define DEFLATE_KERNEL_ARGS                                                    \
	lds_raw, n_chunks, format, level, depth, nice, mode, in_base,          \
	in_offsets, in_nbytes, out_base, out_offsets, out_avail_arr,           \
	out_nbytes, sums, seq_scratch, seg_info, next_chunk, dict_pre

#ifdef LDA_SMALL
extern "C" __global__ void __launch_bounds__(NT, SMALL_WGS)
lda_deflate_small_kernel(DEFLATE_KERNEL_PARAMS)
{
	extern __shared__ __attribute__((aligned(16))) u8 lds_raw[];
	deflate_batch_body<false>(DEFLATE_KERNEL_ARGS);
}

extern "C" size_t lda_deflate_small_lds_bytes(void)
{
	return sizeof(struct deflate_lds);
}

extern "C" size_t lda_deflate_small_max(void)
{
	return RING;
}

extern "C" size_t lda_deflate_small_wgs(void)
{
	return SMALL_WGS;
}

LDA_PROF_DEFINE_READER(libdeflate_amd_profile_read_deflate_small)
#else
extern "C" __global__ void __launch_bounds__(NT)
lda_deflate_batch_kernel(DEFLATE_KERNEL_PARAMS)
{
	extern __shared__ __attribute__((aligned(16))) u8 lds_raw[];
	deflate_batch_body<false>(DEFLATE_KERNEL_ARGS);
}

extern "C" __global__ void __launch_bounds__(NT)
lda_deflate_opt_kernel(DEFLATE_KERNEL_PARAMS)
{
	extern __shared__ __attribute__((aligned(16))) u8 lds_raw[];
	deflate_batch_body<true>(DEFLATE_KERNEL_ARGS);
}

extern "C" size_t lda_deflate_lds_bytes(void)
{
	return sizeof(struct deflate_lds);
}

extern "C" size_t lda_deflate_tile(void)
{
	return TILE;
}

extern "C" size_t lda_deflate_seq_words(void)
{
	return SEQ_STRIDE;
}

LDA_PROF_DEFINE_READER(libdeflate_amd_profile_read_deflate)

#endif
```

libdeflate_amd/csrc/host_compress.hip:

```cpp
#include <stdio.h>
#include <stdlib.h>
#include <string.h>
#include <atomic>
#include <new>
#include <algorithm>
#include <vector>

#include "host_objects.h"
#include "kernels.h"

namespace lda {
bool pick_allocator(const struct libdeflate_options *options,
		    malloc_func_t *m, free_func_t *f);
}
using namespace lda;

struct level_cfg { uint32_t depth, nice, mode; };
static const level_cfg k_levels[13] = {
	{ 0, 0, 0 },
	{ 2, 32, 0 },
	{ 6, 10, 0 },
	{ 12, 14, 0 },
	{ 16, 30, 0 },
	{ 16, 30, 1 },
	{ 35, 65, 1 },
	{ 100, 130, 1 },
	{ 300, 258, 2 },
	{ 600, 258, 2 },
	{ 150, 258, 3 },
	{ 300, 258, 3 },
	{ 2000, 258, 3 },
};

extern "C" LIBDEFLATEAPI struct libdeflate_compressor *
libdeflate_alloc_compressor_ex(int level, const struct libdeflate_options *options)
{
	malloc_func_t m;
	free_func_t f;

	if (!pick_allocator(options, &m, &f))
		return NULL;
	if (level == -1)
		level = 6;
	if (level < 0 || level > 12)
		return NULL;
	if (!device_ctx()) {
		fprintf(stderr, "libdeflate_amd: alloc_compressor: no usable "
			"gfx950 device (%s); no CPU fallback\n",
			libdeflate_amd_last_error());
		return NULL;
	}
	void *mem = m(sizeof(struct libdeflate_compressor));
	if (!mem)
		return NULL;
	struct libdeflate_compressor *c = new (mem) libdeflate_compressor();
	c->free_func = f;
	c->malloc_func = m;
	c->level = level;
	c->device = 0;
	(void)hipGetDevice(&c->device);
	for (int k = 0; k < LDA_MAX_SHARDS; k++)
		c->shard[k] = NULL;
	return c;
}

extern "C" LIBDEFLATEAPI struct libdeflate_compressor *
libdeflate_alloc_compressor(int level)
{
	return libdeflate_alloc_compressor_ex(level, NULL);
}

extern "C" LIBDEFLATEAPI void
libdeflate_free_compressor(struct libdeflate_compressor *c)
{
	if (!c)
		return;
	for (int k = 0; k < LDA_MAX_SHARDS; k++)
		libdeflate_free_compressor(c->shard[k]);
	DeviceGuard on(c->device);
	c->scratch.release();
	c->stage.release();
	c->pinned.release();
	c->meta.release();
	c->streams.release();
	free_func_t f = c->free_func;
	c->~libdeflate_compressor();
	f(c);
}

extern "C" LIBDEFLATEAPI size_t
libdeflate_deflate_compress_bound(struct libdeflate_compressor *c, size_t n)
{
	(void)c;
	size_t blocks = (n + 4999) / 5000;
	if (blocks < 1)
		blocks = 1;
	return 5 * blocks + n;
}

extern "C" LIBDEFLATEAPI size_t
libdeflate_zlib_compress_bound(struct libdeflate_compressor *c, size_t n)
{
	return 6 + libdeflate_deflate_compress_bound(c, n);
}

extern "C" LIBDEFLATEAPI size_t
libdeflate_gzip_compress_bound(struct libdeflate_compressor *c, size_t n)
{
	return 18 + libdeflate_deflate_compress_bound(c, n);
}

static size_t dict_window(void)
{
	const size_t tile = lda_deflate_tile();
	return (32768 - 2 * tile - 272) / tile * tile;
}

struct dict_shape { uint32_t tail, pre_len, sinfo; };

static dict_shape shape_dict(int level, size_t dict_nbytes)
{
	const size_t tile = lda_deflate_tile();
	dict_shape d;
	d.tail = level == 0 ? 0 : (uint32_t)std::min(dict_nbytes, dict_window());
	d.pre_len = (uint32_t)((d.tail + tile - 1) / tile * tile);
	d.sinfo = d.pre_len | ((d.pre_len - d.tail) << 16) | 0x80000000u;
	return d;
}

static int
compress_batch_impl(struct libdeflate_compressor *c, int format, size_t n,
		    const void *d_in, const uint64_t *d_in_offsets,
		    const uint64_t *d_in_nbytes, void *d_out,
		    const uint64_t *d_out_offsets, const uint64_t *d_out_avail,
		    uint64_t *d_out_nbytes, void *stream,
		    const uint32_t *d_seg_info, size_t max_in_nbytes = SIZE_MAX,
		    const void *d_dict = NULL, size_t dict_nbytes = 0)
{
	if (!c) {
		set_error("compress_batch: bad argument");
		return LIBDEFLATE_AMD_BAD_ARG;
	}
	DeviceGuard on(c->device);
	if (!on.ok())
		return LIBDEFLATE_AMD_NO_DEVICE;
	DeviceCtx *ctx = device_ctx();
	hipStream_t st = (hipStream_t)stream;

	if (!ctx)
		return LIBDEFLATE_AMD_NO_DEVICE;
	if (n == 0)
		return LIBDEFLATE_AMD_OK;
	if (!c || !d_in || !d_in_offsets || !d_in_nbytes || !d_out ||
	    !d_out_offsets || !d_out_avail || !d_out_nbytes ||
	    format < LIBDEFLATE_AMD_DEFLATE || format > LIBDEFLATE_AMD_GZIP) {
		set_error("compress_batch: bad argument");
		return LIBDEFLATE_AMD_BAD_ARG;
	}
	const bool dict = d_dict && dict_nbytes;
	const bool small = max_in_nbytes <= lda_deflate_small_max() &&
			   c->level <= 9 && !d_seg_info && !dict && !env_cfg().no_small;
	size_t grid_max = (size_t)ctx->num_cus * (small ? lda_deflate_small_wgs() : 1);
	size_t grid = n < grid_max ? n : grid_max;
	size_t seq_bytes = grid * lda_deflate_seq_words() * 8;
	const size_t blk_at = align_up(seq_bytes + 16 + n * 4, 64);
	uint8_t *scr = (uint8_t *)c->scratch.reserve(
		dict ? blk_at + LDA_DICT_BLK_HDR + dict_window() : seq_bytes + 16 + n * 4);
	if (!scr)
		return LIBDEFLATE_AMD_OOM;
	uint32_t *next_chunk = (uint32_t *)(scr + seq_bytes);
	LDA_HIP_TRY(hipMemsetAsync(next_chunk, 0, 16, st), LIBDEFLATE_AMD_NO_DEVICE);
	uint8_t *blk = NULL;
	if (dict) {
		const dict_shape sh = shape_dict(c->level, dict_nbytes);
		blk = scr + blk_at;
		hipLaunchKernelGGL(lda_dict_prep_kernel, dim3(1), dim3(256), 0, st,
				   (const uint8_t *)d_dict, (uint64_t)dict_nbytes, sh.tail,
				   sh.pre_len, sh.sinfo, blk);
		LDA_HIP_TRY(hipGetLastError(), LIBDEFLATE_AMD_NO_DEVICE);
		if (format == LIBDEFLATE_AMD_ZLIB) {
			int rc = libdeflate_amd_adler32_batch(1, d_dict, (const uint64_t *)(blk + 16),
							      (const uint64_t *)(blk + 24), NULL,
							      (uint32_t *)(blk + 4), stream);
			if (rc != LIBDEFLATE_AMD_OK)
				return rc;
		}
	}
	uint32_t *sums = NULL;
	if (format != LIBDEFLATE_AMD_DEFLATE) {
		sums = (uint32_t *)(scr + seq_bytes + 16);
		int rc = format == LIBDEFLATE_AMD_GZIP ?
			libdeflate_amd_crc32_batch(n, d_in, d_in_offsets,
						   d_in_nbytes, NULL, sums, stream) :
			libdeflate_amd_adler32_batch(n, d_in, d_in_offsets,
						     d_in_nbytes, NULL, sums, stream);
		if (rc != LIBDEFLATE_AMD_OK)
			return rc;
	}
	const size_t lds = small ? lda_deflate_small_lds_bytes() : lda_deflate_lds_bytes();
	if (!ctx->deflate_attr_set.load(std::memory_order_acquire)) {
		LDA_HIP_TRY(hipFuncSetAttribute(
				(const void *)lda_deflate_small_kernel,
				hipFuncAttributeMaxDynamicSharedMemorySize,
				(int)lda_deflate_small_lds_bytes()), LIBDEFLATE_AMD_NO_DEVICE);
		LDA_HIP_TRY(hipFuncSetAttribute(
				(const void *)lda_deflate_batch_kernel,
				hipFuncAttributeMaxDynamicSharedMemorySize,
				(int)lda_deflate_lds_bytes()), LIBDEFLATE_AMD_NO_DEVICE);
		LDA_HIP_TRY(hipFuncSetAttribute(
				(const void *)lda_deflate_opt_kernel,
				hipFuncAttributeMaxDynamicSharedMemorySize,
				(int)lda_deflate_lds_bytes()), LIBDEFLATE_AMD_NO_DEVICE);
		ctx->deflate_attr_set.store(true, std::memory_order_release);
	}
	const level_cfg &lv = k_levels[c->level];
	hipLaunchKernelGGL(small ? lda_deflate_small_kernel :
			   lv.mode == 3 ? lda_deflate_opt_kernel :
					  lda_deflate_batch_kernel, dim3((unsigned)grid),
			   dim3(small ? LDA_DEFLATE_SMALL_THREADS : LDA_DEFLATE_THREADS),
			   lds, st, (uint64_t)n, format, c->level,
			   lv.depth, lv.nice, lv.mode, (const uint8_t *)d_in,
			   d_in_offsets, d_in_nbytes, (uint8_t *)d_out,
			   d_out_offsets, d_out_avail, d_out_nbytes, sums,
			   (uint64_t *)scr, d_seg_info, next_chunk, (const uint8_t *)blk);
	LDA_HIP_TRY(hipGetLastError(), LIBDEFLATE_AMD_NO_DEVICE);
	return LIBDEFLATE_AMD_OK;
}

extern "C" LIBDEFLATEAPI int
libdeflate_amd_compress_batch_dict(struct libdeflate_compressor *c, int format,
				   size_t n, const void *d_dict, size_t dict_nbytes,
				   const void *d_in, const uint64_t *d_in_offsets,
				   const uint64_t *d_in_nbytes, void *d_out,
				   const uint64_t *d_out_offsets,
				   const uint64_t *d_out_avail,
				   uint64_t *d_out_nbytes, void *stream)
{
	if (format != LIBDEFLATE_AMD_DEFLATE && format != LIBDEFLATE_AMD_ZLIB) {
		set_error("compress_batch_dict: format %d takes no dictionary", format);
		return LIBDEFLATE_AMD_BAD_ARG;
	}
	if (dict_nbytes && !d_dict) {
		set_error("compress_batch_dict: bad argument");
		return LIBDEFLATE_AMD_BAD_ARG;
	}
	return compress_batch_impl(c, format, n, d_in, d_in_offsets, d_in_nbytes,
				   d_out, d_out_offsets, d_out_avail,
				   d_out_nbytes, stream, NULL, SIZE_MAX, d_dict, dict_nbytes);
}

extern "C" LIBDEFLATEAPI int
libdeflate_amd_compress_batch(struct libdeflate_compressor *c, int format,
			      size_t n, const void *d_in,
			      const uint64_t *d_in_offsets,
			      const uint64_t *d_in_nbytes, void *d_out,
			      const uint64_t *d_out_offsets,
			      const uint64_t *d_out_avail,
			      uint64_t *d_out_nbytes, void *stream)
{
	return compress_batch_impl(c, format, n, d_in, d_in_offsets, d_in_nbytes,
				   d_out, d_out_offsets, d_out_avail,
				   d_out_nbytes, stream, NULL);
}

extern "C" LIBDEFLATEAPI int
libdeflate_amd_compress_batch_bounded(struct libdeflate_compressor *c, int format,
				      size_t n, const void *d_in,
				      const uint64_t *d_in_offsets,
				      const uint64_t *d_in_nbytes, void *d_out,
				      const uint64_t *d_out_offsets,
				      const uint64_t *d_out_avail,
				      uint64_t *d_out_nbytes, size_t max_in_nbytes,
				      void *stream)
{
	return compress_batch_impl(c, format, n, d_in, d_in_offsets, d_in_nbytes,
				   d_out, d_out_offsets, d_out_avail,
				   d_out_nbytes, stream, NULL, max_in_nbytes);
}

static int compress_batch_host_body(struct libdeflate_compressor *c, int format,
				   size_t n, const void *const *in,
				   const size_t *in_nbytes, void *const *out,
				   const size_t *out_avail, size_t *out_nbytes);

extern "C" LIBDEFLATEAPI int
libdeflate_amd_compress_batch_host(struct libdeflate_compressor *c, int format,
				   size_t n, const void *const *in,
				   const size_t *in_nbytes, void *const *out,
				   const size_t *out_avail, size_t *out_nbytes)
{
	return no_unwind("compress_batch_host", (int)LIBDEFLATE_AMD_OOM, [&]() {
		if (!c || !in_nbytes || n == 0)
			return compress_batch_host_body(c, format, n, in, in_nbytes, out, out_avail,
							out_nbytes);
		size_t bounds[LDA_MAX_SHARDS + 1];
		int devs[LDA_MAX_SHARDS];
		const size_t shards = fanout_plan(c->device, n, in_nbytes, bounds, devs);
		fanout_note(shards);
		if (shards < 2)
			return compress_batch_host_body(c, format, n, in, in_nbytes, out, out_avail,
							out_nbytes);
		if (!in || !out || !out_avail || !out_nbytes) {
			set_error("compress_batch_host: NULL argument");
			return (int)LIBDEFLATE_AMD_BAD_ARG;
		}
		for (size_t k = 1; k < shards; k++) {
			if (c->shard[k])
				continue;
			DeviceGuard on(devs[k]);
			struct libdeflate_options o = {};
			o.sizeof_options = sizeof(o);
			o.malloc_func = c->malloc_func;
			o.free_func = c->free_func;
			if (on.ok())
				c->shard[k] = libdeflate_alloc_compressor_ex(c->level, &o);
			if (!c->shard[k]) {
				fanout_note(1);
				return compress_batch_host_body(c, format, n, in, in_nbytes, out, out_avail,
							out_nbytes);
			}
		}
		return fanout_run(shards, [&](size_t k) {
			const size_t lo = bounds[k], cnt = bounds[k + 1] - lo;
			return compress_batch_host_body(k ? c->shard[k] : c, format, cnt, in + lo,
							in_nbytes + lo, out + lo, out_avail + lo,
							out_nbytes + lo);
		});
	});
}

static int compress_batch_host_body(struct libdeflate_compressor *c, int format,
				   size_t n, const void *const *in,
				   const size_t *in_nbytes, void *const *out,
				   const size_t *out_avail, size_t *out_nbytes)
{
	if (n == 0)
		return device_ctx() ? LIBDEFLATE_AMD_OK : LIBDEFLATE_AMD_NO_DEVICE;
	if (!c || !in || !in_nbytes || !out || !out_avail || !out_nbytes) {
		set_error("compress_batch_host: NULL argument");
		return LIBDEFLATE_AMD_BAD_ARG;
	}
	DeviceGuard on(c->device);
	if (!on.ok() || !device_ctx())
		return LIBDEFLATE_AMD_NO_DEVICE;
	enum { MAX_SLICES = 8 };
	size_t bounds[MAX_SLICES + 1];
	const size_t ns = slice_by_bytes(n, in_nbytes, MAX_SLICES, (size_t)64 << 20, bounds);
	size_t cmp_len[MAX_SLICES], cmp_pos[MAX_SLICES], ncmp = 0;
	for (size_t k = 0; k < ns; k++) {
		cmp_pos[k] = ncmp;
		cmp_len[k] = libdeflate_amd_compact_offsets_len(bounds[k + 1] - bounds[k]);
		ncmp += cmp_len[k];
	}
	std::vector<uint64_t> desc(5 * n + ncmp);
	uint64_t *in_off = &desc[0], *in_n = &desc[n], *out_off = &desc[2 * n],
		 *out_av = &desc[3 * n], *out_n = &desc[4 * n], *cmp_off = &desc[5 * n];
	size_t pos = align_up(desc.size() * 8, 64);
	for (size_t i = 0; i < n; i++) {
		in_off[i] = pos;
		in_n[i] = in_nbytes[i];
		pos = align_up(pos + in_nbytes[i] + 16, 16);
	}
	size_t total_avail = 0;
	size_t avail_before[MAX_SLICES + 1];
	for (size_t k = 0, i = 0; k < ns; k++) {
		avail_before[k] = total_avail;
		for (; i < bounds[k + 1]; i++) {
			out_off[i] = pos;
			out_av[i] = out_avail[i];
			pos = align_up(pos + out_avail[i] + 16, 16);
			total_avail += out_avail[i];
		}
	}
	const size_t cmp_at = pos;
	uint8_t *st = (uint8_t *)c->stage.reserve(cmp_at + total_avail + 64 * ns + 64);
	if (!st)
		return LIBDEFLATE_AMD_OOM;
	if (!c->streams.ensure())
		return LIBDEFLATE_AMD_NO_DEVICE;
	size_t max_in = 0;
	for (size_t i = 0; i < n; i++)
		max_in = in_nbytes[i] > max_in ? in_nbytes[i] : max_in;
	{
		size_t max_nk = 0;
		for (size_t k = 0; k < ns; k++)
			max_nk = bounds[k + 1] - bounds[k] > max_nk ? bounds[k + 1] - bounds[k] : max_nk;
		const bool small = max_in <= lda_deflate_small_max() && c->level <= 9 &&
				   !env_cfg().no_small;
		const size_t grid_max = (size_t)device_ctx()->num_cus * (small ? lda_deflate_small_wgs() : 1);
		const size_t grid = max_nk < grid_max ? max_nk : grid_max;
		if (!c->scratch.reserve(grid * lda_deflate_seq_words() * 8 + 16 + max_nk * 4))
			return LIBDEFLATE_AMD_OOM;
	}
	uint64_t *h_back = (uint64_t *)c->meta.ensure((n + ncmp) * 8);
	if (!h_back)
		return LIBDEFLATE_AMD_OOM;
	out_n = h_back;
	cmp_off = h_back + n;
	hipStream_t s_copy = c->streams.copy, s_comp = c->streams.comp;
	LDA_HIP_TRY(hipMemcpyAsync(st, desc.data(), 4 * n * 8, hipMemcpyHostToDevice,
				   s_copy), LIBDEFLATE_AMD_NO_DEVICE);
	uint64_t *d_desc = (uint64_t *)st;
	hipEvent_t ev_done[MAX_SLICES] = {};
	int rc = LIBDEFLATE_AMD_OK;
	auto cleanup = [&]() {
		(void)hipStreamSynchronize(s_comp);
		(void)hipStreamSynchronize(s_copy);
		for (size_t k = 0; k < ns; k++)
			if (ev_done[k])
				(void)hipEventDestroy(ev_done[k]);
	};
	auto drain = [&](size_t k) -> int {
		const size_t lo = bounds[k], nk = bounds[k + 1] - lo;
		LDA_HIP_TRY(hipEventSynchronize(ev_done[k]), LIBDEFLATE_AMD_NO_DEVICE);
		for (size_t i = lo; i < lo + nk; i++)
			out_nbytes[i] = out_n[i];
		return copy_out_packed(&c->pinned, st + cmp_at + avail_before[k] + 64 * k, nk,
				       out + lo, out_n + lo, cmp_off + cmp_pos[k], s_copy);
	};
	for (size_t k = 0; k < ns && rc == LIBDEFLATE_AMD_OK; k++) {
		const size_t lo = bounds[k], nk = bounds[k + 1] - lo;
		rc = copy_in_packed(&c->pinned, st, nk, in + lo, in_nbytes + lo, in_off + lo, s_copy);
		if (rc != LIBDEFLATE_AMD_OK)
			break;
		rc = libdeflate_amd_compress_batch_bounded(
			c, format, nk, st, d_desc + lo, d_desc + n + lo, st, d_desc + 2 * n + lo,
			d_desc + 3 * n + lo, d_desc + 4 * n + lo, max_in, s_comp);
		if (rc != LIBDEFLATE_AMD_OK)
			break;
		rc = libdeflate_amd_compact_batch(nk, st, d_desc + 2 * n + lo, d_desc + 4 * n + lo,
						  st + cmp_at + avail_before[k] + 64 * k,
						  d_desc + 5 * n + cmp_pos[k], s_comp);
		if (rc != LIBDEFLATE_AMD_OK)
			break;
		if (hipMemcpyAsync(out_n + lo, d_desc + 4 * n + lo, nk * 8, hipMemcpyDeviceToHost,
				   s_comp) != hipSuccess ||
		    hipMemcpyAsync(cmp_off + cmp_pos[k], d_desc + 5 * n + cmp_pos[k], (nk + 1) * 8,
				   hipMemcpyDeviceToHost, s_comp) != hipSuccess ||
		    hipEventCreateWithFlags(&ev_done[k], hipEventDisableTiming) != hipSuccess ||
		    hipEventRecord(ev_done[k], s_comp) != hipSuccess) {
			set_error("compress_batch_host: %s", hipGetErrorString(hipGetLastError()));
			rc = LIBDEFLATE_AMD_NO_DEVICE;
			break;
		}
		if (k)
			rc = drain(k - 1);
	}
	if (rc == LIBDEFLATE_AMD_OK)
		rc = drain(ns - 1);
	cleanup();
	return rc;
}

#define LDA_SEG_BYTES 65536u
#define LDA_LARGE_MIN (2 * LDA_SEG_BYTES)

static uint32_t crc_mulmod(uint32_t a, uint32_t b)
{
	uint32_t p = 0;
	for (uint32_t m = 0x80000000u; m; m >>= 1) {
		if (a & m)
			p ^= b;
		b = (b & 1) ? (b >> 1) ^ 0xEDB88320u : b >> 1;
	}
	return p;
}

uint32_t lda::crc32_shift(uint64_t len)
{
	uint32_t xp = 0x80000000u;
	uint32_t base = 0x00800000u;
	for (uint64_t k = len; k; k >>= 1) {
		if (k & 1)
			xp = crc_mulmod(xp, base);
		base = crc_mulmod(base, base);
	}
	return xp;
}

uint32_t lda::crc32_concat_shift(uint32_t crc_a, uint32_t crc_b, uint32_t shift_b)
{
	return crc_mulmod(crc_a, shift_b) ^ crc_b;
}

uint32_t lda::crc32_concat(uint32_t crc_a, uint32_t crc_b, uint64_t len_b)
{
	return crc32_concat_shift(crc_a, crc_b, crc32_shift(len_b));
}

uint32_t lda::adler32_concat(uint32_t ad_a, uint32_t ad_b, uint64_t len_b)
{
	const uint32_t M = 65521;
	uint32_t a1 = ad_a & 0xFFFF, b1 = ad_a >> 16;
	uint32_t a2 = ad_b & 0xFFFF, b2 = ad_b >> 16;
	uint32_t rem = (uint32_t)(len_b % M);
	uint32_t a = (a1 + a2 + M - 1) % M;
	uint32_t b = (uint32_t)(((uint64_t)rem * a1 + b1 + b2 + M - rem) % M);
	return (b << 16) | a;
}

static size_t large_fail(const char *what)
{
	hipError_t e = hipGetLastError();
	if (e != hipSuccess)
		set_error("%s: %s", what, hipGetErrorString(e));
	complain("libdeflate_*_compress", LIBDEFLATE_AMD_NO_DEVICE);
	return 0;
}

static size_t compress_large(struct libdeflate_compressor *c, int format,
			     const uint8_t *in, size_t n, uint8_t *out,
			     size_t out_avail, const uint8_t *dict = NULL,
			     size_t dict_nbytes = 0)
{
	size_t S = LDA_SEG_BYTES;
	if (dict && n < LDA_LARGE_MIN)
		S = n ? n : 1;
	else if (env_cfg().seg_bytes)
		S = env_cfg().seg_bytes;
	else if (n <= ((size_t)4 << 20))
		S = 16384;
	else if (n <= ((size_t)8 << 20))
		S = 32768;
	const size_t tile = lda_deflate_tile();
	const size_t D = dict_window();
	const size_t nseg = n ? (n + S - 1) / S : 1;
	const size_t slot = align_up(libdeflate_deflate_compress_bound(c, S) + 32, 16);
	const dict_shape dsh = shape_dict(c->level, dict ? dict_nbytes : 0);
	const size_t pre = dict && n ? dsh.pre_len : 0;
	const uint32_t hdr = format == LIBDEFLATE_AMD_GZIP ? 10 :
			     format == LIBDEFLATE_AMD_ZLIB ? (dict ? 6 : 2) : 0;
	const uint32_t ftr = format == LIBDEFLATE_AMD_GZIP ? 8 :
			     format == LIBDEFLATE_AMD_ZLIB ? 4 : 0;

	if (out_avail <= hdr + ftr)
		return 0;
	DeviceCtx *ctx = device_ctx();
	if (!ctx || !c->streams.ensure())
		return large_fail("streams");
	hipStream_t s_copy = c->streams.copy, s_comp = c->streams.comp;
	const size_t per_slice = std::max<size_t>(1, ((size_t)32 << 20) / S);
	const size_t ns = (nseg + per_slice - 1) / per_slice;
	std::vector<size_t> cmp_pos(ns + 1);
	cmp_pos[0] = 0;
	for (size_t k = 0; k < ns; k++)
		cmp_pos[k + 1] = cmp_pos[k] + libdeflate_amd_compact_offsets_len(
			std::min(per_slice, nseg - k * per_slice));
	const size_t ncmp = cmp_pos[ns];
	const size_t desc_bytes = align_up(nseg * (7 * 8 + 4 + 4) + 64, 64);
	const size_t cmp_at = desc_bytes, in_at = align_up(cmp_at + ncmp * 8 + 64, 64) + pre;
	const size_t out_at = align_up(in_at + n + 64, 64);
	const size_t pk_at = align_up(out_at + nseg * slot + 64, 64);
	uint8_t *st = (uint8_t *)c->stage.reserve(pk_at + nseg * slot + 64);
	if (!st) {
		complain("libdeflate_*_compress (device memory)", LIBDEFLATE_AMD_OOM);
		return 0;
	}
	{
		const size_t g = std::min<size_t>(std::min(per_slice, nseg), (size_t)ctx->num_cus);
		if (!c->scratch.reserve(g * lda_deflate_seq_words() * 8 + 16 + std::min(per_slice, nseg) * 4)) {
			complain("libdeflate_*_compress (device memory)", LIBDEFLATE_AMD_OOM);
			return 0;
		}
	}
	std::vector<uint64_t> d64(7 * nseg);
	std::vector<uint32_t> d32(nseg);
	uint64_t *in_off = &d64[0], *in_n = &d64[nseg], *out_off = &d64[2 * nseg],
		 *out_av = &d64[3 * nseg], *pc_off = &d64[5 * nseg], *pc_n = &d64[6 * nseg];
	for (size_t i = 0; i < nseg; i++) {
		const size_t prime = i ? std::min(D, i * S) / tile * tile : 0;
		const size_t len = i + 1 < nseg ? S : n - i * S;
		in_off[i] = in_at + i * S - prime;
		in_n[i] = prime + len;
		out_off[i] = out_at + i * slot;
		out_av[i] = slot;
		pc_off[i] = in_at + i * S;
		pc_n[i] = len;
		d32[i] = (uint32_t)prime | (i + 1 == nseg ? 0x80000000u : 0);
	}
	std::vector<uint8_t> prefix(pre);
	if (pre) {
		in_off[0] -= pre;
		in_n[0] += pre;
		d32[0] |= dsh.sinfo & 0x7FFFFFFFu;
		memcpy(&prefix[pre - dsh.tail], dict + dict_nbytes - dsh.tail, dsh.tail);
	}
	uint64_t *d_desc = (uint64_t *)st;
	uint32_t *d_seg = (uint32_t *)(st + 7 * 8 * nseg);
	uint32_t *d_sums = d_seg + nseg;
	uint64_t *d_cmp = (uint64_t *)(st + cmp_at);
	uint64_t *h_back = (uint64_t *)c->meta.ensure(nseg * 12 + ns * 8 + 64);
	if (!h_back)
		return large_fail("pinned memory");
	uint64_t *h_out_n = h_back, *h_tot = h_back + nseg;
	uint32_t *h_sums = (uint32_t *)(h_back + nseg + ns);
	if (hipMemcpyAsync(d_desc, d64.data(), 7 * 8 * nseg, hipMemcpyHostToDevice, s_copy) != hipSuccess ||
	    hipMemcpyAsync(d_seg, d32.data(), 4 * nseg, hipMemcpyHostToDevice, s_copy) != hipSuccess ||
	    (pre && hipMemcpyAsync(st + in_at - pre, prefix.data(), pre, hipMemcpyHostToDevice,
				   s_copy) != hipSuccess))
		return large_fail("copy in");
	std::vector<hipEvent_t> ev_done(ns, nullptr);
	const size_t piece = ns > 1 ? (size_t)1 << 20 : 0;
	size_t total = hdr;
	bool fits = true, failed = false;
	auto cleanup = [&]() {
		(void)hipStreamSynchronize(s_comp);
		(void)hipStreamSynchronize(s_copy);
		for (size_t k = 0; k < ns; k++)
			if (ev_done[k])
				(void)hipEventDestroy(ev_done[k]);
	};
	auto drain = [&](size_t k) -> bool {
		const size_t lo = k * per_slice, nk = std::min(per_slice, nseg - lo);
		if (hipEventSynchronize(ev_done[k]) != hipSuccess)
			return false;
		for (size_t i = lo; i < lo + nk; i++)
			if (h_out_n[i] == 0)
				fits = false;
		const size_t tk = (size_t)h_tot[k];
		if (!fits || total + tk + ftr > out_avail) {
			fits = false;
			return true;
		}
		if (tk && span_out(&c->pinned, st, pk_at + lo * slot, out + total, tk, s_copy, piece) != LIBDEFLATE_AMD_OK)
			return false;
		total += tk;
		return true;
	};
	for (size_t k = 0; k < ns && fits && !failed; k++) {
		const size_t lo = k * per_slice, nk = std::min(per_slice, nseg - lo);
		const size_t a = lo * S, b = std::min(n, (lo + nk) * S);
		if (b > a ? span_in(&c->pinned, st, in_at + a, in + a, b - a, s_copy, piece) != LIBDEFLATE_AMD_OK :
			    hipStreamSynchronize(s_copy) != hipSuccess) {
			failed = true;
			break;
		}
		int rc = compress_batch_impl(c, LIBDEFLATE_AMD_DEFLATE, nk, st, d_desc + lo,
					     d_desc + nseg + lo, st, d_desc + 2 * nseg + lo,
					     d_desc + 3 * nseg + lo, d_desc + 4 * nseg + lo, s_comp,
					     d_seg + lo);
		if (rc == LIBDEFLATE_AMD_OK && ftr)
			rc = format == LIBDEFLATE_AMD_GZIP ?
				libdeflate_amd_crc32_batch(nk, st, d_desc + 5 * nseg + lo,
							   d_desc + 6 * nseg + lo, NULL, d_sums + lo, s_comp) :
				libdeflate_amd_adler32_batch(nk, st, d_desc + 5 * nseg + lo,
							     d_desc + 6 * nseg + lo, NULL, d_sums + lo, s_comp);
		if (rc == LIBDEFLATE_AMD_OK)
			rc = libdeflate_amd_compact_batch(nk, st, d_desc + 2 * nseg + lo,
							  d_desc + 4 * nseg + lo, st + pk_at + lo * slot,
							  d_cmp + cmp_pos[k], s_comp);
		if (rc != LIBDEFLATE_AMD_OK ||
		    hipMemcpyAsync(h_out_n + lo, d_desc + 4 * nseg + lo, nk * 8, hipMemcpyDeviceToHost,
				   s_comp) != hipSuccess ||
		    hipMemcpyAsync(h_tot + k, d_cmp + cmp_pos[k] + nk, 8, hipMemcpyDeviceToHost,
				   s_comp) != hipSuccess ||
		    (ftr && hipMemcpyAsync(h_sums + lo, d_sums + lo, nk * 4, hipMemcpyDeviceToHost,
					   s_comp) != hipSuccess) ||
		    hipEventCreateWithFlags(&ev_done[k], hipEventDisableTiming) != hipSuccess ||
		    hipEventRecord(ev_done[k], s_comp) != hipSuccess) {
			failed = true;
			break;
		}
		if (k && !drain(k - 1))
			failed = true;
	}
	if (!failed && fits && !drain(ns - 1))
		failed = true;
	cleanup();
	if (failed)
		return large_fail("segmented compress");
	if (!fits || total + ftr > out_avail)
		return 0;
	const size_t at = total;
	total += ftr;
	if (format == LIBDEFLATE_AMD_GZIP) {
		uint32_t crc = 0;
		const uint32_t shS = crc32_shift(S);
		for (size_t i = 0; i < nseg; i++)
			crc = !i ? h_sums[0] :
			      pc_n[i] == S ? crc32_concat_shift(crc, h_sums[i], shS) :
					     crc32_concat(crc, h_sums[i], pc_n[i]);
		const uint8_t xfl = c->level < 2 ? 4 : c->level >= 8 ? 2 : 0;
		const uint8_t h[10] = { 0x1F, 0x8B, 8, 0, 0, 0, 0, 0, xfl, 0xFF };
		memcpy(out, h, 10);
		uint32_t isize = (uint32_t)n;
		for (int k = 0; k < 4; k++) {
			out[at + k] = (uint8_t)(crc >> (8 * k));
			out[at + 4 + k] = (uint8_t)(isize >> (8 * k));
		}
	} else if (format == LIBDEFLATE_AMD_ZLIB) {
		uint32_t ad = 1;
		for (size_t i = 0; i < nseg; i++)
			ad = i ? adler32_concat(ad, h_sums[i], pc_n[i]) : h_sums[0];
		uint32_t fl = c->level < 2 ? 0 : c->level < 6 ? 1 : c->level < 8 ? 2 : 3;
		uint32_t hw = (0x78u << 8) | (fl << 6);
		if (dict) {
			hw |= 0x20;
			hw += (31 - hw % 31) % 31;
			const uint32_t id = libdeflate_adler32(1, dict, dict_nbytes);
			for (int k = 0; k < 4; k++)
				out[2 + k] = (uint8_t)(id >> (8 * (3 - k)));
		} else {
			hw |= 31 - (hw % 31);
		}
		out[0] = (uint8_t)(hw >> 8);
		out[1] = (uint8_t)hw;
		for (int k = 0; k < 4; k++)
			out[at + k] = (uint8_t)(ad >> (8 * (3 - k)));
	}
	return total;
}

static size_t compress_one(struct libdeflate_compressor *c, int format,
			   const void *in, size_t in_nbytes, void *out,
			   size_t out_avail)
{
	if (!c)
		return 0;
	DeviceGuard on(c->device);
	if (!on.ok()) {
		complain("libdeflate_*_compress", LIBDEFLATE_AMD_NO_DEVICE);
		return 0;
	}
	if (in_nbytes >= LDA_LARGE_MIN && c->level > 0 &&
	    (!env_cfg().no_segments || in_nbytes >= 0xFFFF0000u))
		return no_unwind("libdeflate_*_compress", (size_t)0, [&]() {
			return compress_large(c, format, (const uint8_t *)in, in_nbytes,
					      (uint8_t *)out, out_avail);
		});
	const void *ins[1] = { in };
	void *outs[1] = { out };
	size_t got = 0;
	int rc = libdeflate_amd_compress_batch_host(c, format, 1, ins, &in_nbytes,
						    outs, &out_avail, &got);

	if (rc != LIBDEFLATE_AMD_OK) {
		complain("libdeflate_*_compress", rc);
		return 0;
	}
	return got;
}

extern "C" LIBDEFLATEAPI size_t
libdeflate_deflate_compress(struct libdeflate_compressor *c, const void *in,
			    size_t in_nbytes, void *out, size_t out_avail)
{
	return compress_one(c, LIBDEFLATE_AMD_DEFLATE, in, in_nbytes, out,
			    out_avail);
}

extern "C" LIBDEFLATEAPI size_t
libdeflate_zlib_compress(struct libdeflate_compressor *c, const void *in,
			 size_t in_nbytes, void *out, size_t out_avail)
{
	return compress_one(c, LIBDEFLATE_AMD_ZLIB, in, in_nbytes, out, out_avail);
}

extern "C" LIBDEFLATEAPI size_t
libdeflate_gzip_compress(struct libdeflate_compressor *c, const void *in,
			 size_t in_nbytes, void *out, size_t out_avail)
{
	return compress_one(c, LIBDEFLATE_AMD_GZIP, in, in_nbytes, out, out_avail);
}

extern "C" LIBDEFLATEAPI size_t
libdeflate_amd_compress_dict(struct libdeflate_compressor *c, int format,
			     const void *dict, size_t dict_nbytes, const void *in,
			     size_t in_nbytes, void *out, size_t out_avail)
{
	if (format != LIBDEFLATE_AMD_DEFLATE && format != LIBDEFLATE_AMD_ZLIB) {
		set_error("libdeflate_amd_compress_dict: format %d takes no dictionary", format);
		return 0;
	}
	if (!dict_nbytes)
		return compress_one(c, format, in, in_nbytes, out, out_avail);
	if (!c || !dict || (!in && in_nbytes) || !out) {
		set_error("libdeflate_amd_compress_dict: bad argument");
		return 0;
	}
	DeviceGuard on(c->device);
	if (!on.ok()) {
		complain("libdeflate_amd_compress_dict", LIBDEFLATE_AMD_NO_DEVICE);
		return 0;
	}
	return no_unwind("libdeflate_amd_compress_dict", (size_t)0, [&]() {
		return compress_large(c, format, (const uint8_t *)in, in_nbytes, (uint8_t *)out,
				      out_avail, (const uint8_t *)dict, dict_nbytes);
	});
}
```

libdeflate_amd/csrc/kernels.h:

```cpp
#ifndef LDA_KERNELS_H
#define LDA_KERNELS_H

#include <hip/hip_runtime.h>
#include <stdint.h>

extern "C" __global__ void
lda_crc32_batch_kernel(uint64_t n_chunks, const uint8_t *base,
		       const uint64_t *offsets, const uint64_t *nbytes,
		       const uint32_t *init, uint32_t *out,
		       const uint32_t *g_tables, const uint32_t *xpow8);
extern "C" __global__ void
lda_adler32_batch_kernel(uint64_t n_chunks, const uint8_t *base,
			 const uint64_t *offsets, const uint64_t *nbytes,
			 const uint32_t *init, uint32_t *out);
#define LDA_DICT_BLK_HDR 64
extern "C" __global__ void
lda_dict_prep_kernel(const uint8_t *dict, uint64_t dict_nbytes, uint32_t tail,
		     uint32_t pre_len, uint32_t sinfo, uint8_t *blk);

extern "C" __global__ void
lda_inflate_batch_kernel(uint64_t n_chunks, int format, uint32_t lpw,
			 const uint8_t *in_base,
			 const uint64_t *in_offsets, const uint64_t *in_nbytes,
			 uint8_t *out_base, const uint64_t *out_offsets,
			 const uint64_t *out_avail, int32_t *results,
			 uint64_t *actual_in, uint64_t *actual_out,
			 const uint8_t *dict, uint32_t dict_len,
			 const uint32_t *dict_id);
extern "C" __global__ void
lda_inflate_wave_kernel(uint64_t n_chunks, int format, uint32_t *tokscratch,
			uint32_t *next_stream, const uint32_t *order,
			const uint8_t *in_base,
			const uint64_t *in_offsets, const uint64_t *in_nbytes,
			uint8_t *out_base, const uint64_t *out_offsets,
			const uint64_t *out_avail, int32_t *results,
			uint64_t *actual_in, uint64_t *actual_out,
			const uint8_t *dict, uint32_t dict_len,
			const uint32_t *dict_id);
extern "C" __global__ void
lda_inflate_order_kernel(uint64_t n, const uint64_t *in_nbytes, const uint64_t *out_avail,
			 uint32_t *order);
extern "C" size_t lda_inflate_tokcap(void);
extern "C" size_t lda_inflate_window_bytes(void);
extern "C" __global__ void
lda_inflate_finalize_kernel(uint64_t n_chunks, int format, int exact_fill,
			    const uint8_t *in_base, const uint64_t *in_offsets,
			    const uint64_t *out_avail, const uint32_t *sums,
			    int32_t *results, uint64_t *actual_in,
			    uint64_t *actual_out);

#define LDA_DEFLATE_THREADS 1024
extern "C" __global__ void
lda_deflate_batch_kernel(uint64_t n_chunks, int format, int level,
			 uint32_t depth, uint32_t nice, uint32_t mode,
			 const uint8_t *in_base, const uint64_t *in_offsets,
			 const uint64_t *in_nbytes, uint8_t *out_base,
			 const uint64_t *out_offsets, const uint64_t *out_avail,
			 uint64_t *out_nbytes, const uint32_t *sums,
			 uint64_t *seq_scratch, const uint32_t *seg_info,
			 uint32_t *next_chunk, const uint8_t *dict_pre);
extern "C" __global__ void
lda_deflate_opt_kernel(uint64_t n_chunks, int format, int level,
		       uint32_t depth, uint32_t nice, uint32_t mode,
		       const uint8_t *in_base, const uint64_t *in_offsets,
		       const uint64_t *in_nbytes, uint8_t *out_base,
		       const uint64_t *out_offsets, const uint64_t *out_avail,
		       uint64_t *out_nbytes, const uint32_t *sums,
		       uint64_t *seq_scratch, const uint32_t *seg_info,
		       uint32_t *next_chunk, const uint8_t *dict_pre);
#define LDA_DEFLATE_SMALL_THREADS 256
extern "C" __global__ void
lda_deflate_small_kernel(uint64_t n_chunks, int format, int level,
			 uint32_t depth, uint32_t nice, uint32_t mode,
			 const uint8_t *in_base, const uint64_t *in_offsets,
			 const uint64_t *in_nbytes, uint8_t *out_base,
			 const uint64_t *out_offsets, const uint64_t *out_avail,
			 uint64_t *out_nbytes, const uint32_t *sums,
			 uint64_t *seq_scratch, const uint32_t *seg_info,
			 uint32_t *next_chunk, const uint8_t *dict_pre);
extern "C" size_t lda_deflate_small_lds_bytes(void);
extern "C" size_t lda_deflate_small_max(void);
extern "C" size_t lda_deflate_small_wgs(void);
extern "C" size_t lda_deflate_tile(void);
extern "C" size_t lda_deflate_lds_bytes(void);
extern "C" size_t lda_deflate_seq_words(void);

extern "C" size_t lda_inflate_lds_per_stream(void);
extern "C" size_t lda_inflate_lds_shared(void);

extern "C" __global__ void
lda_scan_local_kernel(uint64_t n, const uint64_t *sizes, uint64_t *offsets,
		      uint64_t *block_sums);
extern "C" __global__ void
lda_scan_blocks_kernel(uint64_t nblocks, uint64_t *block_sums);
extern "C" __global__ void
lda_compact_copy_kernel(uint64_t n, const uint8_t *in_base,
			const uint64_t *in_offsets, const uint64_t *sizes,
			uint8_t *out_base, uint64_t *offsets,
			const uint64_t *block_sums);

extern "C" __global__ void
lda_selfcheck_lds_order_kernel(uint64_t *counters);
extern "C" __global__ void
lda_selfcheck_visibility_kernel(uint8_t *buf, uint64_t *counters);
extern "C" size_t lda_selfcheck_region_bytes(void);

#define LDA_CRC_TABLE_WORDS (17 * 256)
#define LDA_CRC_XPOW_WORDS 1024

#endif
```

Measured before the change: 30760.

## Split deflate into match-finding, separate entropy kernel, and fused fallback

Adds a separate entropy-coding kernel of 256-thread workgroups that builds Huffman codes and emits bits from tokens and per-block frequencies written to global buffers by the match-finding batch kernel. Large batches are processed in slices with three launches each (batch, entropy, fused fallback), so block-end Huffman work no longer runs inside the 1024-thread match-finding workgroup. Non-split cases launch a fused kernel instead. The cost is extra global traffic for tokens and block descriptors, more launches, and larger scratch reservations.

Result: faster. 33170, median of 6 (+7.8%).

```diff
diff --git a/libdeflate_amd/csrc/deflate_blockend.h b/libdeflate_amd/csrc/deflate_blockend.h
--- /dev/null
+++ b/libdeflate_amd/csrc/deflate_blockend.h
@@ -0,0 +1,599 @@
+
+static __device__ u32 block_scan(lds_t *L, u32 v, u32 *total)
+{
+	const u32 lane = threadIdx.x & 63, wave = threadIdx.x >> 6;
+	u32 incl = wave_scan_incl(v);
+
+	if (lane == 63)
+		L->scan[0][wave] = incl;
+	__syncthreads();
+	const u32 sw = lane < NWAVES ? L->scan[0][lane] : 0;
+	const u32 iw = wave_scan_incl(sw);
+	const u32 base = bcast_lane(iw - sw, wave);
+	__syncthreads();
+	*total = bcast_lane(iw, NWAVES - 1);
+	return base + incl - v;
+}
+
+static __device__ u32 block_scan1(lds_t *L, u32 v, u32 *total,
+				  u32 *tog)
+{
+	const u32 lane = threadIdx.x & 63, wave = threadIdx.x >> 6;
+	u32 incl = wave_scan_incl(v);
+	u32 *sc = L->scan[*tog];
+
+	*tog ^= 1;
+	if (lane == 63)
+		sc[wave] = incl;
+	__syncthreads();
+	const u32 sw = lane < NWAVES ? sc[lane] : 0;
+	const u32 iw = wave_scan_incl(sw);
+	*total = bcast_lane(iw, NWAVES - 1);
+	return bcast_lane(iw - sw, wave) + incl - v;
+}
+
+static __device__ __forceinline__ void
+length_code(u32 len, u32 *slot, u32 *xbits, u32 *xval)
+{
+	u32 l = len - 3;
+	if (l < 8) {
+		*slot = l; *xbits = 0; *xval = 0;
+	} else if (len == 258) {
+		*slot = 28; *xbits = 0; *xval = 0;
+	} else {
+		u32 hb = 31 - __builtin_clz(l);
+		*xbits = hb - 2;
+		*slot = 4 * (hb - 1) + ((l >> (hb - 2)) & 3);
+		*xval = l & ((1u << (hb - 2)) - 1);
+	}
+}
+
+static __device__ __forceinline__ void
+dist_code(u32 dist, u32 *slot, u32 *xbits, u32 *xval)
+{
+	u32 d = dist - 1;
+	if (d < 4) {
+		*slot = d; *xbits = 0; *xval = 0;
+	} else {
+		u32 hb = 31 - __builtin_clz(d);
+		*xbits = hb - 1;
+		*slot = 2 * hb + ((d >> (hb - 1)) & 1);
+		*xval = d & ((1u << (hb - 1)) - 1);
+	}
+}
+
+
+struct outstate {
+	u8 *out;
+	u64 avail;
+	u64 sg;
+	u64 bits;
+};
+
+static __device__ __forceinline__ u32 *stg_of(lds_t *L)
+{
+	return (u32 *)L->nxtA;
+}
+
+static __device__ __forceinline__ void
+stg_put(lds_t *L, const struct outstate *os, u64 bitpos, u64 code,
+	u32 nbits)
+{
+	if (!nbits)
+		return;
+	u64 rel = bitpos - 8 * os->sg;
+	u32 w = (u32)(rel >> 5), s = (u32)rel & 31;
+	u32 *stg = stg_of(L);
+	u64 lo = code << s;
+	atomicOr((u32 *)&stg[w], (u32)lo);
+	if (s + nbits > 32)
+		atomicOr((u32 *)&stg[w + 1], (u32)(lo >> 32));
+	if (s + nbits > 64)
+		atomicOr((u32 *)&stg[w + 2], (u32)(code >> (64 - s)));
+}
+
+static __device__ __forceinline__ void
+stg_flush(lds_t *L, struct outstate *os, bool final)
+{
+	u32 *stg = stg_of(L);
+	u8 *stgb = (u8 *)stg;
+	const u32 tid = threadIdx.x;
+	u64 done_bytes = final ? (os->bits + 7) / 8 : os->bits / 8;
+	u64 rel_end = done_bytes - os->sg;
+	s64 first = -(s64)os->sg;
+	u32 start = first > 0 ? (u32)first : 0;
+	u32 units = final ? (u32)((rel_end + 15) / 16) : (u32)(rel_end / 16);
+
+	__syncthreads();
+	for (u32 u = tid; u < units; u += NT) {
+		u32 b0 = u * 16, b1 = b0 + 16;
+		u8 *g = os->out + (s64)(os->sg + b0);
+		if (b0 >= start && b1 <= rel_end) {
+			*(uint4 *)g = *(const uint4 *)(stgb + b0);
+		} else {
+			for (u32 b = b0 < start ? start : b0; b < b1 && b < rel_end; b++)
+				g[b - b0] = stgb[b];
+		}
+	}
+	u32 keep_from = units * 16;
+	u32 total_words = (u32)((os->bits - 8 * os->sg + 31) / 32) + 1;
+	u32 keep_words = final ? 0 : total_words - keep_from / 4;
+	u32 v = 0;
+	if (tid < keep_words && keep_from / 4 + tid < STG_WORDS + 8)
+		v = stg[keep_from / 4 + tid];
+	__syncthreads();
+	for (u32 i = tid; i < STG_WORDS + 8; i += NT)
+		stg[i] = 0;
+	if (tid < keep_words)
+		stg[tid] = v;
+	os->sg += keep_from;
+}
+
+static __device__ __forceinline__ void stg_restore(lds_t *L)
+{
+	u32 *stg = stg_of(L);
+
+	__syncthreads();
+	for (u32 i = threadIdx.x; i < STG_WORDS + 8; i += NT)
+		stg[i] = i < 6 ? L->carry[i] : 0;
+	__syncthreads();
+}
+
+static __device__ __forceinline__ void stg_save(lds_t *L, struct outstate *os)
+{
+	stg_flush(L, os, false);
+	if (threadIdx.x < 6)
+		L->carry[threadIdx.x] = stg_of(L)[threadIdx.x];
+	__syncthreads();
+}
+
+static __device__ __forceinline__ void
+put_container_header(lds_t *L, struct outstate *os, int format, int level,
+		     const u8 *__restrict__ dict_pre, u32 hdr_bytes, u32 tid)
+{
+	if (tid == 0) {
+		if (format == LDA_FMT_GZIP) {
+			u32 xfl = level < 2 ? 4 : level >= 8 ? 2 : 0;
+			stg_put(L, os, 0, 0x00088B1Full, 32);
+			stg_put(L, os, 32, 0, 32);
+			stg_put(L, os, 64, xfl | (0xFFu << 8), 16);
+		} else {
+			u32 fl = level < 2 ? 0 : level < 6 ? 1 :
+				 level < 8 ? 2 : 3;
+			u32 h = (0x78u << 8) | (fl << 6);
+			if (dict_pre) {
+				h |= 0x20;
+				h += (31 - h % 31) % 31;
+				stg_put(L, os, 16, __builtin_bswap32(((const u32 *)dict_pre)[1]), 32);
+			} else {
+				h |= 31 - (h % 31);
+			}
+			stg_put(L, os, 0, ((h & 0xFF) << 8) | (h >> 8), 16);
+		}
+	}
+	os->bits = 8 * hdr_bytes;
+}
+
+static __device__ __forceinline__ bool
+block_emit(lds_t *L, struct outstate *os, const u32 *__restrict__ tokg, u32 nseq,
+	   const u8 *__restrict__ inp, u32 bstart, u32 blen, u32 is_final,
+	   bool stored_only, u32 ftr_bytes, u32 *tog, u32 tid, u32 lane, u32 wave)
+{
+	PROF_DECL;
+	PROF_START();
+	u32 btype = 0;
+	if (!stored_only) {
+		if (tid == 0)
+			L->freq[256]++;
+		__syncthreads();
+		{
+			u32 *keys = L->M;
+			u32 *usedv = L->M + 320;
+			u16 *sortedO = (u16 *)(L->M + 324);
+			if (tid < 2)
+				usedv[tid] = 0;
+			__syncthreads();
+			for (u32 vt = tid; vt < 320; vt += NT) {
+				const u32 f = L->freq[vt];
+				if (f) {
+					if (vt < 288)
+						keys[atomicAdd(&usedv[0], 1u)] = (f << 9) | vt;
+					else
+						keys[288 + atomicAdd(&usedv[1], 1u)] =
+							(f << 9) | (vt - 288);
+				}
+			}
+			__syncthreads();
+			{
+				const u32 m1 = usedv[0], m2 = usedv[1];
+				for (u32 i = tid; i < m1 + m2; i += NT) {
+					const bool lit = i < m1;
+					const u32 lo = lit ? 0 : 288, m = lit ? m1 : m2;
+					const u32 key = keys[lit ? i : 288 + i - m1];
+					u32 r = 0;
+					for (u32 q = 0; q < m; q++)
+						r += keys[lo + q] < key;
+					if (lit)
+						L->sorted[r] = (u16)(key & 511);
+					else
+						sortedO[r] = (u16)(key & 511);
+				}
+			}
+			__syncthreads();
+			PROF_MARK(10);
+			if (wave == 0)
+				make_code(L->freq, 288, 15, L->lens, L->codes,
+					  L->sorted, HUFF_LITLEN(L),
+					  usedv[0], true, lane);
+			else if (wave == 1)
+				make_code(L->freq + 288, 32, 15, L->lens + 288,
+					  L->codes + 288, sortedO,
+					  (huff_scratch<32> *)L->hw,
+					  usedv[1], true, lane);
+		}
+		__syncthreads();
+		PROF_MARK(11);
+		{
+			u32 *starts = L->M;
+			if (tid == 0) {
+				L->vars[V_TMP1] = 257;
+				L->vars[V_TMP2] = 1;
+			}
+			if (tid < 19)
+				L->pre_freq[tid] = 0;
+			__syncthreads();
+			for (u32 vt = tid; vt < 320; vt += NT) {
+				if (vt < 288 && vt >= 257 && L->lens[vt])
+					atomicMax((u32 *)&L->vars[V_TMP1], vt + 1);
+				if (vt >= 288 && L->lens[vt])
+					atomicMax((u32 *)&L->vars[V_TMP2], vt - 288 + 1);
+			}
+			__syncthreads();
+			const u32 nlit = L->vars[V_TMP1], noff = L->vars[V_TMP2];
+			const u32 total = nlit + noff;
+			u32 isst[VPT], nst = 0;
+#pragma unroll
+			for (u32 j = 0; j < VPT; j++) {
+				const u32 e = tid * VPT + j;
+				isst[j] = 0;
+				if (e < total) {
+					u32 v = L->lens[e < nlit ? e : 288 + (e - nlit)];
+					u32 pv = 0xFF;
+					if (e)
+						pv = L->lens[e - 1 < nlit ? e - 1 :
+							     288 + (e - 1 - nlit)];
+					isst[j] = pv != v;
+				}
+				nst += isst[j];
+			}
+			u32 nruns;
+			u32 ridx = block_scan(L, nst, &nruns);
+#pragma unroll
+			for (u32 j = 0; j < VPT; j++) {
+				if (isst[j])
+					starts[ridx] = tid * VPT + j;
+				ridx += isst[j];
+			}
+			if (tid == 0)
+				starts[nruns] = total;
+			__syncthreads();
+			u32 rv[VPT], rlen[VPT], nitems[VPT], nit = 0;
+#pragma unroll
+			for (u32 j = 0; j < VPT; j++) {
+				const u32 r = tid * VPT + j;
+				rv[j] = rlen[j] = nitems[j] = 0;
+				if (r < nruns) {
+					u32 st = starts[r];
+					rlen[j] = starts[r + 1] - st;
+					rv[j] = L->lens[st < nlit ? st : 288 + (st - nlit)];
+					if (rv[j] == 0) {
+						u32 full = rlen[j] / 138, rem = rlen[j] % 138;
+						nitems[j] = full + (rem >= 3 ? 1 : rem);
+					} else if (rlen[j] >= 4) {
+						u32 l1 = rlen[j] - 1;
+						nitems[j] = 1 + l1 / 6 + (l1 % 6 >= 3 ? 1 : l1 % 6);
+					} else {
+						nitems[j] = rlen[j];
+					}
+				}
+				nit += nitems[j];
+			}
+			u32 ni;
+			u32 at = block_scan(L, nit, &ni);
+#pragma unroll
+			for (u32 j = 0; j < VPT; j++) {
+				if (tid * VPT + j < nruns) {
+					u32 left = rlen[j];
+					const u32 rvj = rv[j];
+					if (rvj == 0) {
+						while (left >= 11) {
+							u32 r = left > 138 ? 138 : left;
+							L->pre_items[at++] = 18 | ((r - 11) << 5);
+							atomicAdd((u32 *)&L->pre_freq[18], 1u);
+							left -= r;
+						}
+						if (left >= 3) {
+							L->pre_items[at++] = 17 | ((left - 3) << 5);
+							atomicAdd((u32 *)&L->pre_freq[17], 1u);
+							left = 0;
+						}
+					} else if (left >= 4) {
+						L->pre_items[at++] = (u16)rvj;
+						left--;
+						u32 n16 = 0;
+						while (left >= 3) {
+							u32 r = left > 6 ? 6 : left;
+							L->pre_items[at++] = 16 | ((r - 3) << 5);
+							n16++;
+							left -= r;
+						}
+						atomicAdd((u32 *)&L->pre_freq[16], n16);
+						atomicAdd((u32 *)&L->pre_freq[rvj], 1u);
+					}
+					if (left)
+						atomicAdd((u32 *)&L->pre_freq[rvj], left);
+					while (left) {
+						L->pre_items[at++] = (u16)rvj;
+						left--;
+					}
+				}
+			}
+			if (tid == 0)
+				L->vars[V_NPRE] = ni;
+		}
+		__syncthreads();
+		PROF_MARK(23);
+		if (wave == 0)
+			make_code(L->pre_freq, 19, 7, L->pre_lens, L->pre_codes,
+				  L->sorted, (huff_scratch<32> *)L->hw,
+				  0, false, lane);
+		__syncthreads();
+		PROF_MARK(22);
+		u32 dyn = 0, stat = 0;
+		for (u32 vt = tid; vt < 320; vt += NT) {
+			u32 f = L->freq[vt];
+			u32 xb = 0, sl = 8;
+			if (vt < 288) {
+				sl = vt < 144 ? 8 : vt < 256 ? 9 : vt < 280 ? 7 : 8;
+				if (vt >= 265 && vt < 285)
+					xb = (vt - 261) >> 2;
+			} else {
+				u32 ds = vt - 288;
+				sl = 5;
+				if (ds >= 4)
+					xb = (ds >> 1) - 1;
+			}
+			dyn += f * (L->lens[vt] + xb);
+			stat += f * (sl + xb);
+		}
+		if (tid < 19) {
+			u32 xb = tid == 16 ? 2 : tid == 17 ? 3 : tid == 18 ? 7 : 0;
+			dyn += L->pre_freq[tid] * (L->pre_lens[tid] + xb);
+		}
+		u32 dyn_tot, stat_tot;
+		(void)block_scan(L, dyn, &dyn_tot);
+		(void)block_scan(L, stat, &stat_tot);
+		static const u8 perm[19] = { 16, 17, 18, 0, 8, 7, 9, 6, 10,
+					     5, 11, 4, 12, 3, 13, 2, 14,
+					     1, 15 };
+		u32 nexp = 19;
+		while (nexp > 4 && L->pre_lens[perm[nexp - 1]] == 0)
+			nexp--;
+		u32 cost_dyn = 3 + 5 + 5 + 4 + 3 * nexp + dyn_tot;
+		u32 cost_stat = 3 + stat_tot;
+		u32 pieces = blen ? (blen + 65534) / 65535 : 1;
+		u32 pad = (u32)((0 - (os->bits + 3)) & 7);
+		u64 cost_stored = 3 + pad + 32 + 8ull * blen +
+				  (u64)(pieces - 1) * 40;
+		u64 best = cost_stored;
+		btype = 0;
+		if (cost_stat < best) {
+			best = cost_stat;
+			btype = 1;
+		}
+		if (cost_dyn < best) {
+			best = cost_dyn;
+			btype = 2;
+		}
+		if ((os->bits + best + 7) / 8 + ftr_bytes > os->avail)
+			return false;
+		L->vars[V_TMP3] = nexp;
+	} else {
+		u32 pieces = blen ? (blen + 65534) / 65535 : 1;
+		u64 cost = (u64)pieces * 40 + 8ull * blen;
+		if ((os->bits + cost + 7) / 8 + ftr_bytes > os->avail)
+			return false;
+	}
+
+	PROF_MARK(7);
+	stg_restore(L);
+	if (btype == 0) {
+		u32 done = 0;
+		do {
+			u32 piece = blen - done > 65535 ? 65535 : blen - done;
+			u32 fin = (is_final && done + piece == blen) ? 1 : 0;
+			u32 pad = (u32)((0 - (os->bits + 3)) & 7);
+			if (tid == 0) {
+				stg_put(L, os, os->bits, fin, 3);
+				u64 b = os->bits + 3 + pad;
+				stg_put(L, os, b, piece | ((u64)(piece ^ 0xFFFF) << 16), 32);
+			}
+			os->bits += 3 + pad + 32;
+			__syncthreads();
+			for (u32 w0 = 0; w0 < piece; w0 += 2048) {
+				u32 cnt = piece - w0 < 2048 ? piece - w0 : 2048;
+				stg_flush(L, os, false);
+				__syncthreads();
+				for (u32 j = tid; j < cnt; j += NT) {
+					u32 pos = bstart + done + w0 + j;
+					stg_put(L, os, os->bits + 8ull * j, inp[pos], 8);
+				}
+				os->bits += 8ull * cnt;
+				__syncthreads();
+			}
+			done += piece;
+		} while (done < blen);
+		stg_flush(L, os, false);
+	} else {
+		if (btype == 1) {
+			__syncthreads();
+			for (u32 s = tid; s < 320; s += NT)
+				L->lens[s] = s < 144 ? 8 : s < 256 ? 9 :
+					     s < 280 ? 7 : s < 288 ? 8 : 5;
+			__syncthreads();
+			if (tid == 0) {
+				u32 nc[16] = { 0 }, bl[16] = { 0 };
+				for (u32 s = 0; s < 288; s++)
+					bl[L->lens[s]]++;
+				u32 code = 0;
+				for (u32 d = 1; d < 16; d++) {
+					code = (code + bl[d - 1]) << 1;
+					nc[d] = code;
+				}
+				for (u32 s = 0; s < 288; s++) {
+					u32 l = L->lens[s];
+					L->codes[s] = (u16)(__brev(nc[l]++) >> (32 - l));
+				}
+				for (u32 s = 0; s < 32; s++)
+					L->codes[288 + s] = (u16)(__brev(s) >> 27);
+			}
+			__syncthreads();
+		}
+		{
+			u64 hcode[VPT];
+			u32 hbits[VPT], hsum = 0;
+			const u32 nexp = btype == 2 ? L->vars[V_TMP3] : 0;
+			const u32 ni = btype == 2 ? L->vars[V_NPRE] : 0;
+#pragma unroll
+			for (u32 j = 0; j < VPT; j++) {
+				const u32 vt = tid * VPT + j;
+				hcode[j] = 0;
+				hbits[j] = 0;
+				if (vt == 0) {
+					hcode[j] = is_final | (btype << 1);
+					hbits[j] = 3;
+					if (btype == 2) {
+						u32 nlit = L->vars[V_TMP1], noff = L->vars[V_TMP2];
+						hcode[j] |= (u64)((nlit - 257) | ((noff - 1) << 5) |
+								  ((nexp - 4) << 10)) << 3;
+						hbits[j] = 17;
+					}
+				} else if (vt <= nexp) {
+					static const u8 perm2[19] = { 16, 17, 18, 0, 8, 7,
+						9, 6, 10, 5, 11, 4, 12, 3, 13, 2, 14, 1, 15 };
+					hcode[j] = L->pre_lens[perm2[vt - 1]];
+					hbits[j] = 3;
+				} else if (vt <= nexp + ni) {
+					u32 it = L->pre_items[vt - nexp - 1];
+					u32 sym = it & 31, ex = it >> 5;
+					u32 l = L->pre_lens[sym];
+					u32 xb = sym == 16 ? 2 : sym == 17 ? 3 :
+						 sym == 18 ? 7 : 0;
+					hcode[j] = L->pre_codes[sym] | ((u64)ex << l);
+					hbits[j] = l + xb;
+				}
+				hsum += hbits[j];
+			}
+			u32 htot;
+			u32 hoff = block_scan(L, hsum, &htot);
+#pragma unroll
+			for (u32 j = 0; j < VPT; j++) {
+				stg_put(L, os, os->bits + hoff, hcode[j], hbits[j]);
+				hoff += hbits[j];
+			}
+			os->bits += htot;
+		}
+		stg_flush(L, os, false);
+
+		PROF_MARK(9);
+		__builtin_amdgcn_fence(__ATOMIC_ACQUIRE, "workgroup");
+		u32 tok_nxt = tid < nseq ? tokg[tid] : 0;
+		for (u32 b0 = 0; b0 < nseq; b0 += NT) {
+			u64 code = 0;
+			u32 nb = 0;
+			const u32 tok = tok_nxt;
+			if (b0 + NT + tid < nseq)
+				tok_nxt = tokg[b0 + NT + tid];
+			if (b0 + tid < nseq) {
+				if (tok & TOK_MATCH) {
+					const u32 len = (tok & 0xFF) + 3, dist = ((tok >> 8) & 0x7FFF) + 1;
+					u32 sl, xb, xv, ds, dxb, dxv;
+					length_code(len, &sl, &xb, &xv);
+					dist_code(dist, &ds, &dxb, &dxv);
+					u32 ll = L->lens[257 + sl];
+					u32 dl = L->lens[288 + ds];
+					u64 v = L->codes[257 + sl];
+					u32 sh = ll;
+					v |= (u64)xv << sh;
+					sh += xb;
+					v |= (u64)L->codes[288 + ds] << sh;
+					sh += dl;
+					v |= (u64)dxv << sh;
+					sh += dxb;
+					code = v;
+					nb = sh;
+				} else {
+					code = L->codes[tok];
+					nb = L->lens[tok];
+				}
+			}
+			u32 tot;
+			u32 off = block_scan1(L, nb, &tot, tog);
+			stg_put(L, os, os->bits + off, code, nb);
+			os->bits += tot;
+			if (os->bits - 8 * os->sg + 48 * NT + 64 > 32 * STG_WORDS)
+				stg_flush(L, os, false);
+		}
+		stg_flush(L, os, false);
+		__syncthreads();
+		if (tid == 0)
+			stg_put(L, os, os->bits, L->codes[256], L->lens[256]);
+		os->bits += L->lens[256];
+		__syncthreads();
+	}
+
+	stg_save(L, os);
+	PROF_MARK(8);
+	return true;
+}
+
+static __device__ __forceinline__ void
+finish_stream(lds_t *L, struct outstate *os, bool overflow, bool seg_last,
+	      int format, u32 ftr_bytes, const u32 *__restrict__ sums, u64 c, u32 n,
+	      u64 *__restrict__ out_nbytes, u32 tid)
+{
+	__syncthreads();
+	if (!overflow && !seg_last &&
+	    (os->bits + 3 + 7) / 8 + 4 > os->avail)
+		overflow = true;
+	if (!overflow) {
+		stg_restore(L);
+		if (!seg_last) {
+			u64 fb = 8 * ((os->bits + 3 + 7) / 8);
+			if (tid == 0)
+				stg_put(L, os, fb, 0xFFFF0000ull, 32);
+			os->bits = fb + 32;
+			__syncthreads();
+		}
+		if (ftr_bytes) {
+			u32 sum = sums ? sums[c] : 0;
+			u64 fb = 8 * ((os->bits + 7) / 8);
+			if (tid == 0) {
+				if (format == LDA_FMT_GZIP) {
+					stg_put(L, os, fb, sum, 32);
+					stg_put(L, os, fb + 32, n, 32);
+				} else {
+					stg_put(L, os, fb, __builtin_bswap32(sum), 32);
+				}
+			}
+			os->bits = fb + 8 * ftr_bytes;
+			__syncthreads();
+		}
+		stg_flush(L, os, true);
+		if (tid == 0)
+			out_nbytes[c] = (os->bits + 7) / 8;
+	} else if (tid == 0) {
+		out_nbytes[c] = 0;
+	}
+	__syncthreads();
+}
diff --git a/libdeflate_amd/csrc/deflate_entropy.hip b/libdeflate_amd/csrc/deflate_entropy.hip
--- /dev/null
+++ b/libdeflate_amd/csrc/deflate_entropy.hip
@@ -0,0 +1,112 @@
+#include <stddef.h>
+#include "device_common.h"
+#include "kernels.h"
+
+#define LDA_ENTROPY 1
+#define NT LDA_DEFLATE_ENTROPY_THREADS
+#define VPT (1024 / NT)
+#define NWAVES (NT / 64)
+#ifndef ENTROPY_WGS
+#define ENTROPY_WGS 4
+#endif
+static_assert(NT == 256, "ENTROPY_WGS waves per EU are ENTROPY_WGS workgroups per CU");
+#define TOK_MATCH 0x80000000u
+#define STG_WORDS 1020
+
+struct deflate_lds {
+	u32 M[1776];
+	u32 freq[320];
+	u8 lens[320];
+	u16 codes[320];
+	u16 sorted[288];
+	u32 hw[288];
+	u16 pre_items[320 + 8];
+	u32 pre_freq[19];
+	u8 pre_lens[20];
+	u16 pre_codes[20];
+	u32 nxtA[STG_WORDS + 8] __attribute__((aligned(16)));
+	u32 scan[2][NWAVES + 1];
+	u32 carry[6];
+	u32 vars[4];
+};
+static_assert(sizeof(struct deflate_lds) * ENTROPY_WGS <= 163840, "ENTROPY_WGS workgroups per CU");
+
+#ifdef __HIP_DEVICE_COMPILE__
+#define AS3 __attribute__((address_space(3)))
+#else
+#define AS3
+#endif
+typedef AS3 struct deflate_lds lds_t;
+
+enum { V_TMP1 = 0, V_TMP2, V_TMP3, V_NPRE, V_COUNT };
+static_assert(V_COUNT <= sizeof(((struct deflate_lds *)0)->vars) / sizeof(u32), "vars[] holds them all");
+
+#include "deflate_huffman.h"
+#include "deflate_blockend.h"
+
+extern "C" __global__ void __launch_bounds__(NT, ENTROPY_WGS)
+lda_deflate_entropy_kernel(u64 n_chunks, int format, int level,
+			   const u8 *__restrict__ in_base, const u64 *__restrict__ in_offsets,
+			   const u64 *__restrict__ in_nbytes, u8 *__restrict__ out_base,
+			   const u64 *__restrict__ out_offsets,
+			   const u64 *__restrict__ out_avail_arr, u64 *__restrict__ out_nbytes,
+			   const u32 *__restrict__ sums, const u32 *__restrict__ seg_info,
+			   const u32 *__restrict__ tok_buf, const u32 *__restrict__ blk_buf,
+			   u32 tok_stride, u32 blk_stride)
+{
+	extern __shared__ __attribute__((aligned(16))) u8 lds_raw[];
+	lds_t *L = (lds_t *)(uintptr_t)0;
+	const u32 tid = threadIdx.x, lane = tid & 63, wave = tid >> 6;
+	if ((u32)(uintptr_t)(__attribute__((address_space(3))) u8 *)lds_raw != 0)
+		__builtin_trap();
+	const u64 c = blockIdx.x;
+	if (c >= n_chunks)
+		return;
+	const u32 nb = blk_buf[c];
+	if (nb == LDA_BLK_FUSED)
+		return;
+	const u32 *__restrict__ desc = blk_buf + LDA_BLK_HDR_WORDS(n_chunks) +
+				       c * blk_stride * LDA_BLK_WORDS;
+	const u32 *__restrict__ tokg = tok_buf + c * tok_stride;
+	const u8 *__restrict__ inp = in_base + in_offsets[c];
+	const u32 n = (u32)in_nbytes[c];
+	const bool seg_last = seg_info ? seg_info[c] >> 31 : true;
+	const u32 hdr_bytes = format == LDA_FMT_GZIP ? 10 : format == LDA_FMT_ZLIB ? 2 : 0;
+	const u32 ftr_bytes = format == LDA_FMT_GZIP ? 8 : format == LDA_FMT_ZLIB ? 4 : 0;
+	bool overflow = nb == LDA_BLK_OVERFLOW;
+	struct outstate os;
+	os.out = out_base + out_offsets[c];
+	os.avail = out_avail_arr[c];
+	os.sg = (u64)(0 - ((uintptr_t)os.out & 15));
+	os.bits = 0;
+	u32 tog = 0;
+
+	for (u32 i = tid; i < STG_WORDS + 8; i += NT)
+		stg_of(L)[i] = 0;
+	__syncthreads();
+	if (!overflow && hdr_bytes)
+		put_container_header(L, &os, format, level, NULL, hdr_bytes, tid);
+	__syncthreads();
+	stg_save(L, &os);
+
+	for (u32 b = 0; b < nb && !overflow; b++) {
+		const u32 *__restrict__ d = desc + (size_t)b * LDA_BLK_WORDS;
+		for (u32 i = tid; i < 320; i += NT)
+			L->freq[i] = d[LDA_BLK_FREQ + i];
+		const u32 tok0 = d[LDA_BLK_TOK0], ntok = d[LDA_BLK_NTOK];
+		const u32 bstart = d[LDA_BLK_START], bend = d[LDA_BLK_END];
+		const u32 flags = d[LDA_BLK_FLAGS];
+		__syncthreads();
+		if (!block_emit(L, &os, tokg + tok0, ntok, inp, bstart, bend - bstart, flags & 1,
+				(flags & LDA_BLK_STORED) != 0, ftr_bytes, &tog, tid, lane, wave))
+			overflow = true;
+	}
+	finish_stream(L, &os, overflow, seg_last, format, ftr_bytes, sums, c, n, out_nbytes, tid);
+}
+
+extern "C" size_t lda_deflate_entropy_lds_bytes(void)
+{
+	return sizeof(struct deflate_lds);
+}
+
+LDA_PROF_DEFINE_READER(libdeflate_amd_profile_read_deflate_entropy)
diff --git a/libdeflate_amd/csrc/deflate_huffman.h b/libdeflate_amd/csrc/deflate_huffman.h
--- a/libdeflate_amd/csrc/deflate_huffman.h
+++ b/libdeflate_amd/csrc/deflate_huffman.h
@@ -1,3 +1,9 @@
+static __device__ __forceinline__ u32 rank_below(u64 uniform_mask)
+{
+	return __builtin_amdgcn_mbcnt_hi((u32)(uniform_mask >> 32),
+					 __builtin_amdgcn_mbcnt_lo((u32)uniform_mask, 0));
+}
+
 
 template <int N, typename W = u32> struct huff_scratch {
 	W A[N];
diff --git a/libdeflate_amd/csrc/deflate_kernel.hip b/libdeflate_amd/csrc/deflate_kernel.hip
--- a/libdeflate_amd/csrc/deflate_kernel.hip
+++ b/libdeflate_amd/csrc/deflate_kernel.hip
@@ -33,7 +33,6 @@
 #define S3_TAIL 256u
 #define S3_CLAIM 24u
 #define S3_RA_DEPTH 2u
-#define S6_ALWAYS_FLUSH 0
 #define S3_HALF_SHIFT 1
 #define S3_HALF 1
 #define P1_PASSES 0xFFFFFFFFu
@@ -176,75 +175,6 @@
 	return __builtin_amdgcn_inverse_ballot_w64(uniform_mask);
 }
 
-static __device__ __forceinline__ u32 rank_below(u64 uniform_mask)
-{
-	return __builtin_amdgcn_mbcnt_hi((u32)(uniform_mask >> 32),
-					 __builtin_amdgcn_mbcnt_lo((u32)uniform_mask, 0));
-}
-
-static __device__ u32 block_scan(lds_t *L, u32 v, u32 *total)
-{
-	const u32 lane = threadIdx.x & 63, wave = threadIdx.x >> 6;
-	u32 incl = wave_scan_incl(v);
-
-	if (lane == 63)
-		L->scan[0][wave] = incl;
-	__syncthreads();
-	const u32 sw = lane < NWAVES ? L->scan[0][lane] : 0;
-	const u32 iw = wave_scan_incl(sw);
-	const u32 base = bcast_lane(iw - sw, wave);
-	__syncthreads();
-	*total = bcast_lane(iw, NWAVES - 1);
-	return base + incl - v;
-}
-
-static __device__ u32 block_scan1(lds_t *L, u32 v, u32 *total,
-				  u32 *tog)
-{
-	const u32 lane = threadIdx.x & 63, wave = threadIdx.x >> 6;
-	u32 incl = wave_scan_incl(v);
-	u32 *sc = L->scan[*tog];
-
-	*tog ^= 1;
-	if (lane == 63)
-		sc[wave] = incl;
-	__syncthreads();
-	const u32 sw = lane < NWAVES ? sc[lane] : 0;
-	const u32 iw = wave_scan_incl(sw);
-	*total = bcast_lane(iw, NWAVES - 1);
-	return bcast_lane(iw - sw, wave) + incl - v;
-}
-
-static __device__ __forceinline__ void
-length_code(u32 len, u32 *slot, u32 *xbits, u32 *xval)
-{
-	u32 l = len - 3;
-	if (l < 8) {
-		*slot = l; *xbits = 0; *xval = 0;
-	} else if (len == 258) {
-		*slot = 28; *xbits = 0; *xval = 0;
-	} else {
-		u32 hb = 31 - __builtin_clz(l);
-		*xbits = hb - 2;
-		*slot = 4 * (hb - 1) + ((l >> (hb - 2)) & 3);
-		*xval = l & ((1u << (hb - 2)) - 1);
-	}
-}
-
-static __device__ __forceinline__ void
-dist_code(u32 dist, u32 *slot, u32 *xbits, u32 *xval)
-{
-	u32 d = dist - 1;
-	if (d < 4) {
-		*slot = d; *xbits = 0; *xval = 0;
-	} else {
-		u32 hb = 31 - __builtin_clz(d);
-		*xbits = hb - 1;
-		*slot = 2 * hb + ((d >> (hb - 1)) & 1);
-		*xval = d & ((1u << (hb - 1)) - 1);
-	}
-}
-
 static __device__ u32 choose_min_len(u32 used_literals, u32 depth)
 {
 	u32 m = used_literals >= 80 ? 3 : used_literals >= 45 ? 4 :
@@ -316,93 +246,9 @@
 	return l0 == 0 ? 1 : st;
 }
 
+#include "deflate_huffman.h"
+#include "deflate_blockend.h"
 #include "deflate_opt.h"
-#include "deflate_huffman.h"
-
-
-struct outstate {
-	u8 *out;
-	u64 avail;
-	u64 sg;
-	u64 bits;
-};
-
-static __device__ __forceinline__ u32 *stg_of(lds_t *L)
-{
-	return (u32 *)L->nxtA;
-}
-
-static __device__ __forceinline__ void
-stg_put(lds_t *L, const struct outstate *os, u64 bitpos, u64 code,
-	u32 nbits)
-{
-	if (!nbits)
-		return;
-	u64 rel = bitpos - 8 * os->sg;
-	u32 w = (u32)(rel >> 5), s = (u32)rel & 31;
-	u32 *stg = stg_of(L);
-	u64 lo = code << s;
-	atomicOr((u32 *)&stg[w], (u32)lo);
-	if (s + nbits > 32)
-		atomicOr((u32 *)&stg[w + 1], (u32)(lo >> 32));
-	if (s + nbits > 64)
-		atomicOr((u32 *)&stg[w + 2], (u32)(code >> (64 - s)));
-}
-
-static __device__ __forceinline__ void
-stg_flush(lds_t *L, struct outstate *os, bool final)
-{
-	u32 *stg = stg_of(L);
-	u8 *stgb = (u8 *)stg;
-	const u32 tid = threadIdx.x;
-	u64 done_bytes = final ? (os->bits + 7) / 8 : os->bits / 8;
-	u64 rel_end = done_bytes - os->sg;
-	s64 first = -(s64)os->sg;
-	u32 start = first > 0 ? (u32)first : 0;
-	u32 units = final ? (u32)((rel_end + 15) / 16) : (u32)(rel_end / 16);
-
-	__syncthreads();
-	for (u32 u = tid; u < units; u += NT) {
-		u32 b0 = u * 16, b1 = b0 + 16;
-		u8 *g = os->out + (s64)(os->sg + b0);
-		if (b0 >= start && b1 <= rel_end) {
-			*(uint4 *)g = *(const uint4 *)(stgb + b0);
-		} else {
-			for (u32 b = b0 < start ? start : b0; b < b1 && b < rel_end; b++)
-				g[b - b0] = stgb[b];
-		}
-	}
-	u32 keep_from = units * 16;
-	u32 total_words = (u32)((os->bits - 8 * os->sg + 31) / 32) + 1;
-	u32 keep_words = final ? 0 : total_words - keep_from / 4;
-	u32 v = 0;
-	if (tid < keep_words && keep_from / 4 + tid < STG_WORDS + 8)
-		v = stg[keep_from / 4 + tid];
-	__syncthreads();
-	for (u32 i = tid; i < STG_WORDS + 8; i += NT)
-		stg[i] = 0;
-	if (tid < keep_words)
-		stg[tid] = v;
-	os->sg += keep_from;
-}
-
-static __device__ __forceinline__ void stg_restore(lds_t *L)
-{
-	u32 *stg = stg_of(L);
-
-	__syncthreads();
-	for (u32 i = threadIdx.x; i < STG_WORDS + 8; i += NT)
-		stg[i] = i < 6 ? L->carry[i] : 0;
-	__syncthreads();
-}
-
-static __device__ __forceinline__ void stg_save(lds_t *L, struct outstate *os)
-{
-	stg_flush(L, os, false);
-	if (threadIdx.x < 6)
-		L->carry[threadIdx.x] = stg_of(L)[threadIdx.x];
-	__syncthreads();
-}
 
 
 static __device__ __forceinline__ u32 lds_mskor_rtn(u32 byteaddr, u32 mask, u32 val)
@@ -1617,7 +1463,7 @@
 #endif
 
 
-template <bool OPT> static __device__ __forceinline__ void
+template <bool OPT, bool SPLIT = false> static __device__ __forceinline__ void
 deflate_batch_body(u8 *lds_raw, u64 n_chunks, int format, int level, u32 depth,
 		   u32 nice, u32 mode,
 		   const u8 *__restrict__ in_base,
@@ -1631,14 +1477,16 @@
 		   u64 *__restrict__ seq_scratch,
 		   const u32 *__restrict__ seg_info,
 		   u32 *__restrict__ next_chunk,
-		   const u8 *__restrict__ dict_pre)
-{
+		   const u8 *__restrict__ dict_pre,
+		   u32 *__restrict__ tok_buf = NULL, u32 *__restrict__ blk_buf = NULL,
+		   u32 tok_stride = 0, u32 blk_stride = 0, u32 *__restrict__ fused_cnt = NULL)
+{
+	static_assert(!(OPT && SPLIT), "levels 10-12 keep the fused block end");
 	lds_t *L = (lds_t *)(uintptr_t)0;
 	const u32 tid = threadIdx.x;
 	if ((u32)(uintptr_t)(__attribute__((address_space(3))) u8 *)lds_raw != 0)
 		__builtin_trap();
 	u64 *__restrict__ seqg = seq_scratch + (size_t)blockIdx.x * SEQ_STRIDE;
-	u32 *__restrict__ tokg = (u32 *)seqg;
 	u32 *__restrict__ msave = (u32 *)(seqg + SEQ_GCAP);
 	u32 *__restrict__ fsave = msave + TILE + 8;
 	u32 *__restrict__ bsave = fsave + 640;
@@ -1651,16 +1499,23 @@
 		length_code(i + 3, &sl, &xb, &xv);
 		L->lslot[i] = (u8)sl;
 	}
+	const u32 *__restrict__ only = !SPLIT && blk_buf ? blk_buf + LDA_BLK_LIST(n_chunks) : NULL;
+	const u64 n_todo = only ? bcast_first(*fused_cnt) : n_chunks;
 	for (;;) {
 		__syncthreads();
 		if (tid == 0)
 			L->vars[V_TMP0] = atomicAdd(next_chunk, 1u);
 		__syncthreads();
-		const u64 c = bcast_first(L->vars[V_TMP0]);
-		if (c >= n_chunks)
+		const u64 i_todo = bcast_first(L->vars[V_TMP0]);
+		if (i_todo >= n_todo)
 			break;
+		const u64 c = only ? bcast_first(only[i_todo]) : i_todo;
 		const u8 *inp = in_base + in_offsets[c];
 		u64 n64 = in_nbytes[c];
+		u32 *__restrict__ const tokg = SPLIT ? tok_buf + c * tok_stride : (u32 *)seqg;
+		u32 *__restrict__ const blk_desc = SPLIT ?
+			blk_buf + LDA_BLK_HDR_WORDS(n_chunks) + c * blk_stride * LDA_BLK_WORDS : NULL;
+		u32 nblocks = 0, blk_tok0 = 0;
 		const u32 sinfo = dict_pre ? (n64 ? ((const u32 *)dict_pre)[0] : 0x80000000u) :
 				  seg_info ? seg_info[c] : 0x80000000u;
 		const u32 dict_len = sinfo & 0xFFFFu;
@@ -1686,6 +1541,9 @@
 		if (n64 > RING)
 			overflow = true;
 #endif
+		const bool over_bound = SPLIT && n64 > tok_stride;
+		if (over_bound)
+			overflow = true;
 		const u32 n = (u32)n64;
 
 		__syncthreads();
@@ -1713,31 +1571,12 @@
 		os.bits = 0;
 		__syncthreads();
 
-		if (!overflow && hdr_bytes) {
-			if (tid == 0) {
-				if (format == LDA_FMT_GZIP) {
-					u32 xfl = level < 2 ? 4 : level >= 8 ? 2 : 0;
-					stg_put(L, &os, 0, 0x00088B1Full, 32);
-					stg_put(L, &os, 32, 0, 32);
-					stg_put(L, &os, 64, xfl | (0xFFu << 8), 16);
-				} else {
-					u32 fl = level < 2 ? 0 : level < 6 ? 1 :
-						 level < 8 ? 2 : 3;
-					u32 h = (0x78u << 8) | (fl << 6);
-					if (dict_pre) {
-						h |= 0x20;
-						h += (31 - h % 31) % 31;
-						stg_put(L, &os, 16, __builtin_bswap32(((const u32 *)dict_pre)[1]), 32);
-					} else {
-						h |= 31 - (h % 31);
-					}
-					stg_put(L, &os, 0, ((h & 0xFF) << 8) | (h >> 8), 16);
-				}
-			}
-			os.bits = 8 * hdr_bytes;
-		}
-		__syncthreads();
-		stg_save(L, &os);
+		if (!SPLIT) {
+			if (!overflow && hdr_bytes)
+				put_container_header(L, &os, format, level, dict_pre, hdr_bytes, tid);
+			__syncthreads();
+			stg_save(L, &os);
+		}
 
 		u32 loaded = 0;
 		u32 block_start = dict_len;
@@ -2131,7 +1970,7 @@
 				nseq_now = stored_only ? 0 : bcast_first(pv.x);
 			}
 			bool end_block = last_tile || splitv ||
-				(!stored_only && nseq_now + 2 * TOK_TILE_MAX > TOK_CAP) ||
+				(!stored_only && nseq_now - blk_tok0 + 2 * TOK_TILE_MAX > TOK_CAP) ||
 				walkpos - block_start > MAX_BLOCK_LEN;
 			if (!end_block)
 				continue;
@@ -2145,6 +1984,27 @@
 			const u32 nseq_all = nseq_now;
 			const u32 nseq = retro ? bcast_first(L->vars[V_NSEQ_PRE]) : nseq_all;
 			const u32 is_final = last_tile && seg_last ? 1 : 0;
+			if (SPLIT) {
+				u32 *d = blk_desc + (size_t)nblocks * LDA_BLK_WORDS;
+				for (u32 i = tid; i < 320; i += NT) {
+					const u32 f = L->freq[i], fp = retro ? fsave[i] : f;
+					d[LDA_BLK_FREQ + i] = fp;
+					L->freq[i] = f - fp;
+				}
+				if (tid == 0) {
+					d[LDA_BLK_TOK0] = blk_tok0;
+					d[LDA_BLK_NTOK] = nseq - blk_tok0;
+					d[LDA_BLK_START] = bstart;
+					d[LDA_BLK_END] = bend;
+					d[LDA_BLK_FLAGS] = is_final | (stored_only ? LDA_BLK_STORED : 0);
+				}
+				nblocks++;
+				blk_tok0 = nseq;
+				carryv = 0;
+				block_start = bend;
+				__syncthreads();
+				continue;
+			}
 			if (retro) {
 				for (u32 i = tid; i < 320; i += NT) {
 					u32 f = L->freq[i], fp = fsave[i];
@@ -2154,386 +2014,18 @@
 				__syncthreads();
 			}
 
-			u32 btype = 0;
-			if (!stored_only) {
-				if (mx_pending) {
-					const AS3 u32 *MXs = (const AS3 u32 *)L->nxtB;
-					for (u32 i = tid; i < TILE; i += NT)
-						msave[4 + i] = MXs[4 + i];
-				}
-				if (tid == 0)
-					L->freq[256]++;
-				__syncthreads();
-				{
-					u32 *keys = L->M;
-					u32 *usedv = L->M + 320;
-					u16 *sortedO = (u16 *)(L->M + 324);
-					if (tid < 2)
-						usedv[tid] = 0;
-					__syncthreads();
-					for (u32 vt = tid; vt < 320; vt += NT) {
-						const u32 f = L->freq[vt];
-						if (f) {
-							if (vt < 288)
-								keys[atomicAdd(&usedv[0], 1u)] = (f << 9) | vt;
-							else
-								keys[288 + atomicAdd(&usedv[1], 1u)] =
-									(f << 9) | (vt - 288);
-						}
-					}
-					__syncthreads();
-					{
-						const u32 m1 = usedv[0], m2 = usedv[1];
-						for (u32 i = tid; i < m1 + m2; i += NT) {
-							const bool lit = i < m1;
-							const u32 lo = lit ? 0 : 288, m = lit ? m1 : m2;
-							const u32 key = keys[lit ? i : 288 + i - m1];
-							u32 r = 0;
-							for (u32 q = 0; q < m; q++)
-								r += keys[lo + q] < key;
-							if (lit)
-								L->sorted[r] = (u16)(key & 511);
-							else
-								sortedO[r] = (u16)(key & 511);
-						}
-					}
-					__syncthreads();
-					PROF_MARK(10);
-					if (wave == 0)
-						make_code(L->freq, 288, 15, L->lens, L->codes,
-							  L->sorted, HUFF_LITLEN(L),
-							  usedv[0], true, lane);
-					else if (wave == 1)
-						make_code(L->freq + 288, 32, 15, L->lens + 288,
-							  L->codes + 288, sortedO,
-							  (huff_scratch<32> *)L->hw,
-							  usedv[1], true, lane);
-				}
-				__syncthreads();
-				PROF_MARK(11);
-				{
-					u32 *starts = L->M;
-					if (tid == 0) {
-						L->vars[V_TMP1] = 257;
-						L->vars[V_TMP2] = 1;
-					}
-					if (tid < 19)
-						L->pre_freq[tid] = 0;
-					__syncthreads();
-					for (u32 vt = tid; vt < 320; vt += NT) {
-						if (vt < 288 && vt >= 257 && L->lens[vt])
-							atomicMax((u32 *)&L->vars[V_TMP1], vt + 1);
-						if (vt >= 288 && L->lens[vt])
-							atomicMax((u32 *)&L->vars[V_TMP2], vt - 288 + 1);
-					}
-					__syncthreads();
-					const u32 nlit = L->vars[V_TMP1], noff = L->vars[V_TMP2];
-					const u32 total = nlit + noff;
-					u32 isst[VPT], nst = 0;
-#pragma unroll
-					for (u32 j = 0; j < VPT; j++) {
-						const u32 e = tid * VPT + j;
-						isst[j] = 0;
-						if (e < total) {
-							u32 v = L->lens[e < nlit ? e : 288 + (e - nlit)];
-							u32 pv = 0xFF;
-							if (e)
-								pv = L->lens[e - 1 < nlit ? e - 1 :
-									     288 + (e - 1 - nlit)];
-							isst[j] = pv != v;
-						}
-						nst += isst[j];
-					}
-					u32 nruns;
-					u32 ridx = block_scan(L, nst, &nruns);
-#pragma unroll
-					for (u32 j = 0; j < VPT; j++) {
-						if (isst[j])
-							starts[ridx] = tid * VPT + j;
-						ridx += isst[j];
-					}
-					if (tid == 0)
-						starts[nruns] = total;
-					__syncthreads();
-					u32 rv[VPT], rlen[VPT], nitems[VPT], nit = 0;
-#pragma unroll
-					for (u32 j = 0; j < VPT; j++) {
-						const u32 r = tid * VPT + j;
-						rv[j] = rlen[j] = nitems[j] = 0;
-						if (r < nruns) {
-							u32 st = starts[r];
-							rlen[j] = starts[r + 1] - st;
-							rv[j] = L->lens[st < nlit ? st : 288 + (st - nlit)];
-							if (rv[j] == 0) {
-								u32 full = rlen[j] / 138, rem = rlen[j] % 138;
-								nitems[j] = full + (rem >= 3 ? 1 : rem);
-							} else if (rlen[j] >= 4) {
-								u32 l1 = rlen[j] - 1;
-								nitems[j] = 1 + l1 / 6 + (l1 % 6 >= 3 ? 1 : l1 % 6);
-							} else {
-								nitems[j] = rlen[j];
-							}
-						}
-						nit += nitems[j];
-					}
-					u32 ni;
-					u32 at = block_scan(L, nit, &ni);
-#pragma unroll
-					for (u32 j = 0; j < VPT; j++) {
-						if (tid * VPT + j < nruns) {
-							u32 left = rlen[j];
-							const u32 rvj = rv[j];
-							if (rvj == 0) {
-								while (left >= 11) {
-									u32 r = left > 138 ? 138 : left;
-									L->pre_items[at++] = 18 | ((r - 11) << 5);
-									atomicAdd((u32 *)&L->pre_freq[18], 1u);
-									left -= r;
-								}
-								if (left >= 3) {
-									L->pre_items[at++] = 17 | ((left - 3) << 5);
-									atomicAdd((u32 *)&L->pre_freq[17], 1u);
-									left = 0;
-								}
-							} else if (left >= 4) {
-								L->pre_items[at++] = (u16)rvj;
-								left--;
-								u32 n16 = 0;
-								while (left >= 3) {
-									u32 r = left > 6 ? 6 : left;
-									L->pre_items[at++] = 16 | ((r - 3) << 5);
-									n16++;
-									left -= r;
-								}
-								atomicAdd((u32 *)&L->pre_freq[16], n16);
-								atomicAdd((u32 *)&L->pre_freq[rvj], 1u);
-							}
-							if (left)
-								atomicAdd((u32 *)&L->pre_freq[rvj], left);
-							while (left) {
-								L->pre_items[at++] = (u16)rvj;
-								left--;
-							}
-						}
-					}
-					if (tid == 0)
-						L->vars[V_NPRE] = ni;
-				}
-				__syncthreads();
-				PROF_MARK(23);
-				if (wave == 0)
-					make_code(L->pre_freq, 19, 7, L->pre_lens, L->pre_codes,
-						  L->sorted, (huff_scratch<32> *)L->hw,
-						  0, false, lane);
-				__syncthreads();
-				PROF_MARK(22);
-				u32 dyn = 0, stat = 0;
-				for (u32 vt = tid; vt < 320; vt += NT) {
-					u32 f = L->freq[vt];
-					u32 xb = 0, sl = 8;
-					if (vt < 288) {
-						sl = vt < 144 ? 8 : vt < 256 ? 9 : vt < 280 ? 7 : 8;
-						if (vt >= 265 && vt < 285)
-							xb = (vt - 261) >> 2;
-					} else {
-						u32 ds = vt - 288;
-						sl = 5;
-						if (ds >= 4)
-							xb = (ds >> 1) - 1;
-					}
-					dyn += f * (L->lens[vt] + xb);
-					stat += f * (sl + xb);
-				}
-				if (tid < 19) {
-					u32 xb = tid == 16 ? 2 : tid == 17 ? 3 : tid == 18 ? 7 : 0;
-					dyn += L->pre_freq[tid] * (L->pre_lens[tid] + xb);
-				}
-				u32 dyn_tot, stat_tot;
-				(void)block_scan(L, dyn, &dyn_tot);
-				(void)block_scan(L, stat, &stat_tot);
-				static const u8 perm[19] = { 16, 17, 18, 0, 8, 7, 9, 6, 10,
-							     5, 11, 4, 12, 3, 13, 2, 14,
-							     1, 15 };
-				u32 nexp = 19;
-				while (nexp > 4 && L->pre_lens[perm[nexp - 1]] == 0)
-					nexp--;
-				u32 cost_dyn = 3 + 5 + 5 + 4 + 3 * nexp + dyn_tot;
-				u32 cost_stat = 3 + stat_tot;
-				u32 pieces = blen ? (blen + 65534) / 65535 : 1;
-				u32 pad = (u32)((0 - (os.bits + 3)) & 7);
-				u64 cost_stored = 3 + pad + 32 + 8ull * blen +
-						  (u64)(pieces - 1) * 40;
-				u64 best = cost_stored;
-				btype = 0;
-				if (cost_stat < best) {
-					best = cost_stat;
-					btype = 1;
-				}
-				if (cost_dyn < best) {
-					best = cost_dyn;
-					btype = 2;
-				}
-				if ((os.bits + best + 7) / 8 + ftr_bytes > os.avail)
-					overflow = true;
-				L->vars[V_TMP3] = nexp;
-			} else {
-				u32 pieces = blen ? (blen + 65534) / 65535 : 1;
-				u64 cost = (u64)pieces * 40 + 8ull * blen;
-				if ((os.bits + cost + 7) / 8 + ftr_bytes > os.avail)
-					overflow = true;
-			}
-			if (overflow)
+			if (!stored_only && mx_pending) {
+				const AS3 u32 *MXs = (const AS3 u32 *)L->nxtB;
+				for (u32 i = tid; i < TILE; i += NT)
+					msave[4 + i] = MXs[4 + i];
+			}
+			PROF_MARK(10);
+			if (!block_emit(L, &os, tokg, nseq, inp, bstart, blen, is_final, stored_only,
+					ftr_bytes, &tog, tid, lane, wave)) {
+				overflow = true;
 				break;
-
-			PROF_MARK(7);
-			stg_restore(L);
-			if (btype == 0) {
-				u32 done = 0;
-				do {
-					u32 piece = blen - done > 65535 ? 65535 : blen - done;
-					u32 fin = (is_final && done + piece == blen) ? 1 : 0;
-					u32 pad = (u32)((0 - (os.bits + 3)) & 7);
-					if (tid == 0) {
-						stg_put(L, &os, os.bits, fin, 3);
-						u64 b = os.bits + 3 + pad;
-						stg_put(L, &os, b, piece | ((u64)(piece ^ 0xFFFF) << 16), 32);
-					}
-					os.bits += 3 + pad + 32;
-					__syncthreads();
-					for (u32 w0 = 0; w0 < piece; w0 += 2048) {
-						u32 cnt = piece - w0 < 2048 ? piece - w0 : 2048;
-						stg_flush(L, &os, false);
-						__syncthreads();
-						for (u32 j = tid; j < cnt; j += NT) {
-							u32 pos = bstart + done + w0 + j;
-							stg_put(L, &os, os.bits + 8ull * j, inp[pos], 8);
-						}
-						os.bits += 8ull * cnt;
-						__syncthreads();
-					}
-					done += piece;
-				} while (done < blen);
-				stg_flush(L, &os, false);
-			} else {
-				if (btype == 1) {
-					__syncthreads();
-					for (u32 s = tid; s < 320; s += NT)
-						L->lens[s] = s < 144 ? 8 : s < 256 ? 9 :
-							     s < 280 ? 7 : s < 288 ? 8 : 5;
-					__syncthreads();
-					if (tid == 0) {
-						u32 nc[16] = { 0 }, bl[16] = { 0 };
-						for (u32 s = 0; s < 288; s++)
-							bl[L->lens[s]]++;
-						u32 code = 0;
-						for (u32 d = 1; d < 16; d++) {
-							code = (code + bl[d - 1]) << 1;
-							nc[d] = code;
-						}
-						for (u32 s = 0; s < 288; s++) {
-							u32 l = L->lens[s];
-							L->codes[s] = (u16)(__brev(nc[l]++) >> (32 - l));
-						}
-						for (u32 s = 0; s < 32; s++)
-							L->codes[288 + s] = (u16)(__brev(s) >> 27);
-					}
-					__syncthreads();
-				}
-				{
-					u64 hcode[VPT];
-					u32 hbits[VPT], hsum = 0;
-					const u32 nexp = btype == 2 ? L->vars[V_TMP3] : 0;
-					const u32 ni = btype == 2 ? L->vars[V_NPRE] : 0;
-#pragma unroll
-					for (u32 j = 0; j < VPT; j++) {
-						const u32 vt = tid * VPT + j;
-						hcode[j] = 0;
-						hbits[j] = 0;
-						if (vt == 0) {
-							hcode[j] = is_final | (btype << 1);
-							hbits[j] = 3;
-							if (btype == 2) {
-								u32 nlit = L->vars[V_TMP1], noff = L->vars[V_TMP2];
-								hcode[j] |= (u64)((nlit - 257) | ((noff - 1) << 5) |
-										  ((nexp - 4) << 10)) << 3;
-								hbits[j] = 17;
-							}
-						} else if (vt <= nexp) {
-							static const u8 perm2[19] = { 16, 17, 18, 0, 8, 7,
-								9, 6, 10, 5, 11, 4, 12, 3, 13, 2, 14, 1, 15 };
-							hcode[j] = L->pre_lens[perm2[vt - 1]];
-							hbits[j] = 3;
-						} else if (vt <= nexp + ni) {
-							u32 it = L->pre_items[vt - nexp - 1];
-							u32 sym = it & 31, ex = it >> 5;
-							u32 l = L->pre_lens[sym];
-							u32 xb = sym == 16 ? 2 : sym == 17 ? 3 :
-								 sym == 18 ? 7 : 0;
-							hcode[j] = L->pre_codes[sym] | ((u64)ex << l);
-							hbits[j] = l + xb;
-						}
-						hsum += hbits[j];
-					}
-					u32 htot;
-					u32 hoff = block_scan(L, hsum, &htot);
-#pragma unroll
-					for (u32 j = 0; j < VPT; j++) {
-						stg_put(L, &os, os.bits + hoff, hcode[j], hbits[j]);
-						hoff += hbits[j];
-					}
-					os.bits += htot;
-				}
-				stg_flush(L, &os, false);
-
-				PROF_MARK(9);
-				__builtin_amdgcn_fence(__ATOMIC_ACQUIRE, "workgroup");
-				u32 tok_nxt = tid < nseq ? tokg[tid] : 0;
-				for (u32 b0 = 0; b0 < nseq; b0 += NT) {
-					u64 code = 0;
-					u32 nb = 0;
-					const u32 tok = tok_nxt;
-					if (b0 + NT + tid < nseq)
-						tok_nxt = tokg[b0 + NT + tid];
-					if (b0 + tid < nseq) {
-						if (tok & TOK_MATCH) {
-							const u32 len = (tok & 0xFF) + 3, dist = ((tok >> 8) & 0x7FFF) + 1;
-							u32 sl, xb, xv, ds, dxb, dxv;
-							length_code(len, &sl, &xb, &xv);
-							dist_code(dist, &ds, &dxb, &dxv);
-							u32 ll = L->lens[257 + sl];
-							u32 dl = L->lens[288 + ds];
-							u64 v = L->codes[257 + sl];
-							u32 sh = ll;
-							v |= (u64)xv << sh;
-							sh += xb;
-							v |= (u64)L->codes[288 + ds] << sh;
-							sh += dl;
-							v |= (u64)dxv << sh;
-							sh += dxb;
-							code = v;
-							nb = sh;
-						} else {
-							code = L->codes[tok];
-							nb = L->lens[tok];
-						}
-					}
-					u32 tot;
-					u32 off = block_scan1(L, nb, &tot, &tog);
-					stg_put(L, &os, os.bits + off, code, nb);
-					os.bits += tot;
-					if (S6_ALWAYS_FLUSH || os.bits - 8 * os.sg + 48 * NT + 64 > 32 * STG_WORDS)
-						stg_flush(L, &os, false);
-				}
-				stg_flush(L, &os, false);
-				__syncthreads();
-				if (tid == 0)
-					stg_put(L, &os, os.bits, L->codes[256], L->lens[256]);
-				os.bits += L->lens[256];
-				__syncthreads();
-			}
-
-			stg_save(L, &os);
-			PROF_MARK(8);
+			}
+			PROF_START();
 			if (OPT && mode == 3 && tid < 256)
 				bsave[tid] = 0;
 			if (retro) {
@@ -2569,40 +2061,18 @@
 			__syncthreads();
 		}
 
-		__syncthreads();
-		if (!overflow && !seg_last &&
-		    (os.bits + 3 + 7) / 8 + 4 > os.avail)
-			overflow = true;
-		if (!overflow) {
-			stg_restore(L);
-			if (!seg_last) {
-				u64 fb = 8 * ((os.bits + 3 + 7) / 8);
-				if (tid == 0)
-					stg_put(L, &os, fb, 0xFFFF0000ull, 32);
-				os.bits = fb + 32;
-				__syncthreads();
-			}
-			if (ftr_bytes) {
-				u32 sum = sums ? sums[c] : 0;
-				u64 fb = 8 * ((os.bits + 7) / 8);
-				if (tid == 0) {
-					if (format == LDA_FMT_GZIP) {
-						stg_put(L, &os, fb, sum, 32);
-						stg_put(L, &os, fb + 32, n, 32);
-					} else {
-						stg_put(L, &os, fb, __builtin_bswap32(sum), 32);
-					}
-				}
-				os.bits = fb + 8 * ftr_bytes;
-				__syncthreads();
-			}
-			stg_flush(L, &os, true);
-			if (tid == 0)
-				out_nbytes[c] = (os.bits + 7) / 8;
-		} else if (tid == 0) {
-			out_nbytes[c] = 0;
-		}
-		__syncthreads();
+		if (SPLIT) {
+			__syncthreads();
+			if (tid == 0) {
+				blk_buf[c] = over_bound ? LDA_BLK_FUSED :
+					     overflow ? LDA_BLK_OVERFLOW : nblocks;
+				if (over_bound)
+					blk_buf[LDA_BLK_LIST(n_chunks) + atomicAdd(fused_cnt, 1u)] = (u32)c;
+			}
+		} else {
+			finish_stream(L, &os, overflow, seg_last, format, ftr_bytes, sums, c, n,
+				      out_nbytes, tid);
+		}
 	}
 }
 
@@ -2646,10 +2116,22 @@
 LDA_PROF_DEFINE_READER(libdeflate_amd_profile_read_deflate_small)
 #else
 extern "C" __global__ void __launch_bounds__(NT)
-lda_deflate_batch_kernel(DEFLATE_KERNEL_PARAMS)
+lda_deflate_batch_kernel(DEFLATE_KERNEL_PARAMS, u32 *__restrict__ tok_buf,
+			 u32 *__restrict__ blk_buf, u32 tok_stride, u32 blk_stride,
+			 u32 *__restrict__ fused_cnt)
 {
 	extern __shared__ __attribute__((aligned(16))) u8 lds_raw[];
-	deflate_batch_body<false>(DEFLATE_KERNEL_ARGS);
+	deflate_batch_body<false, true>(DEFLATE_KERNEL_ARGS, tok_buf, blk_buf, tok_stride,
+					blk_stride, fused_cnt);
+}
+
+extern "C" __global__ void __launch_bounds__(NT)
+lda_deflate_fused_kernel(DEFLATE_KERNEL_PARAMS, const u32 *__restrict__ blk_buf,
+			 const u32 *__restrict__ fused_cnt)
+{
+	extern __shared__ __attribute__((aligned(16))) u8 lds_raw[];
+	deflate_batch_body<false>(DEFLATE_KERNEL_ARGS, NULL, (u32 *)blk_buf, 0, 0,
+				  (u32 *)fused_cnt);
 }
 
 extern "C" __global__ void __launch_bounds__(NT)
diff --git a/libdeflate_amd/csrc/host_compress.hip b/libdeflate_amd/csrc/host_compress.hip
--- a/libdeflate_amd/csrc/host_compress.hip
+++ b/libdeflate_amd/csrc/host_compress.hip
@@ -128,6 +128,51 @@
 	return d;
 }
 
+#define LDA_SPLIT_SCRATCH ((size_t)1280 << 20)
+#define LDA_SPLIT_MIN_PER_CU 4
+
+struct batch_plan {
+	bool small, split;
+	size_t grid, per_slice, nslices;
+	uint32_t tok_stride, blk_stride;
+	size_t cnt_at, sums_at, tok_at, blk_at, dict_at, total;
+};
+
+static batch_plan plan_batch(const struct libdeflate_compressor *c, size_t n,
+			     size_t max_in, bool seg, bool dict)
+{
+	batch_plan p = {};
+	p.small = max_in <= lda_deflate_small_max() && c->level <= 9 && !seg && !dict &&
+		  !env_cfg().no_small;
+	const size_t tile = lda_deflate_tile();
+	const size_t tok_stride = align_up(max_in, 16);
+	const size_t blk_stride = std::max<size_t>(1, (tok_stride + tile - 1) / tile);
+	const size_t per_buf = tok_stride * 4 + blk_stride * LDA_BLK_WORDS * 4 + 4;
+	const size_t num_cus = (size_t)device_ctx()->num_cus;
+	p.split = !p.small && c->level <= 9 && !dict && max_in != SIZE_MAX &&
+		  n >= LDA_SPLIT_MIN_PER_CU * num_cus &&
+		  per_buf <= LDA_SPLIT_SCRATCH && tok_stride <= 0xFFFFFFF0u;
+	p.per_slice = p.split ? std::min(n, LDA_SPLIT_SCRATCH / per_buf) : n;
+	p.per_slice = std::max<size_t>(p.per_slice, 1);
+	p.nslices = (n + p.per_slice - 1) / p.per_slice;
+	const size_t grid_max = num_cus * (p.small ? lda_deflate_small_wgs() : 1);
+	p.grid = std::min(p.per_slice, grid_max);
+	p.cnt_at = p.grid * lda_deflate_seq_words() * 8;
+	p.sums_at = p.cnt_at + align_up(12 * p.nslices, 16);
+	p.dict_at = p.tok_at = align_up(p.sums_at + n * 4, 64);
+	p.total = p.sums_at + n * 4;
+	if (dict)
+		p.total = p.dict_at + LDA_DICT_BLK_HDR + dict_window();
+	if (p.split) {
+		p.tok_stride = (uint32_t)tok_stride;
+		p.blk_stride = (uint32_t)blk_stride;
+		p.blk_at = align_up(p.tok_at + p.per_slice * tok_stride * 4, 64);
+		p.total = p.blk_at + (LDA_BLK_HDR_WORDS(p.per_slice) +
+				      p.per_slice * blk_stride * LDA_BLK_WORDS) * 4;
+	}
+	return p;
+}
+
 static int
 compress_batch_impl(struct libdeflate_compressor *c, int format, size_t n,
 		    const void *d_in, const uint64_t *d_in_offsets,
@@ -158,22 +203,18 @@
 		return LIBDEFLATE_AMD_BAD_ARG;
 	}
 	const bool dict = d_dict && dict_nbytes;
-	const bool small = max_in_nbytes <= lda_deflate_small_max() &&
-			   c->level <= 9 && !d_seg_info && !dict && !env_cfg().no_small;
-	size_t grid_max = (size_t)ctx->num_cus * (small ? lda_deflate_small_wgs() : 1);
-	size_t grid = n < grid_max ? n : grid_max;
-	size_t seq_bytes = grid * lda_deflate_seq_words() * 8;
-	const size_t blk_at = align_up(seq_bytes + 16 + n * 4, 64);
-	uint8_t *scr = (uint8_t *)c->scratch.reserve(
-		dict ? blk_at + LDA_DICT_BLK_HDR + dict_window() : seq_bytes + 16 + n * 4);
+	const batch_plan pl = plan_batch(c, n, max_in_nbytes, d_seg_info != NULL, dict);
+	const bool small = pl.small;
+	uint8_t *scr = (uint8_t *)c->scratch.reserve(pl.total);
 	if (!scr)
 		return LIBDEFLATE_AMD_OOM;
-	uint32_t *next_chunk = (uint32_t *)(scr + seq_bytes);
-	LDA_HIP_TRY(hipMemsetAsync(next_chunk, 0, 16, st), LIBDEFLATE_AMD_NO_DEVICE);
+	uint32_t *next_chunk = (uint32_t *)(scr + pl.cnt_at);
+	LDA_HIP_TRY(hipMemsetAsync(next_chunk, 0, align_up(12 * pl.nslices, 16), st),
+		    LIBDEFLATE_AMD_NO_DEVICE);
 	uint8_t *blk = NULL;
 	if (dict) {
 		const dict_shape sh = shape_dict(c->level, dict_nbytes);
-		blk = scr + blk_at;
+		blk = scr + pl.dict_at;
 		hipLaunchKernelGGL(lda_dict_prep_kernel, dim3(1), dim3(256), 0, st,
 				   (const uint8_t *)d_dict, (uint64_t)dict_nbytes, sh.tail,
 				   sh.pre_len, sh.sinfo, blk);
@@ -188,7 +229,7 @@
 	}
 	uint32_t *sums = NULL;
 	if (format != LIBDEFLATE_AMD_DEFLATE) {
-		sums = (uint32_t *)(scr + seq_bytes + 16);
+		sums = (uint32_t *)(scr + pl.sums_at);
 		int rc = format == LIBDEFLATE_AMD_GZIP ?
 			libdeflate_amd_crc32_batch(n, d_in, d_in_offsets,
 						   d_in_nbytes, NULL, sums, stream) :
@@ -211,19 +252,67 @@
 				(const void *)lda_deflate_opt_kernel,
 				hipFuncAttributeMaxDynamicSharedMemorySize,
 				(int)lda_deflate_lds_bytes()), LIBDEFLATE_AMD_NO_DEVICE);
+		LDA_HIP_TRY(hipFuncSetAttribute(
+				(const void *)lda_deflate_fused_kernel,
+				hipFuncAttributeMaxDynamicSharedMemorySize,
+				(int)lda_deflate_lds_bytes()), LIBDEFLATE_AMD_NO_DEVICE);
 		ctx->deflate_attr_set.store(true, std::memory_order_release);
 	}
 	const level_cfg &lv = k_levels[c->level];
-	hipLaunchKernelGGL(small ? lda_deflate_small_kernel :
-			   lv.mode == 3 ? lda_deflate_opt_kernel :
-					  lda_deflate_batch_kernel, dim3((unsigned)grid),
-			   dim3(small ? LDA_DEFLATE_SMALL_THREADS : LDA_DEFLATE_THREADS),
-			   lds, st, (uint64_t)n, format, c->level,
-			   lv.depth, lv.nice, lv.mode, (const uint8_t *)d_in,
-			   d_in_offsets, d_in_nbytes, (uint8_t *)d_out,
-			   d_out_offsets, d_out_avail, d_out_nbytes, sums,
-			   (uint64_t *)scr, d_seg_info, next_chunk, (const uint8_t *)blk);
-	LDA_HIP_TRY(hipGetLastError(), LIBDEFLATE_AMD_NO_DEVICE);
+	if (!pl.split && (small || lv.mode == 3)) {
+		hipLaunchKernelGGL(small ? lda_deflate_small_kernel : lda_deflate_opt_kernel,
+				   dim3((unsigned)pl.grid),
+				   dim3(small ? LDA_DEFLATE_SMALL_THREADS : LDA_DEFLATE_THREADS),
+				   lds, st, (uint64_t)n, format, c->level,
+				   lv.depth, lv.nice, lv.mode, (const uint8_t *)d_in,
+				   d_in_offsets, d_in_nbytes, (uint8_t *)d_out,
+				   d_out_offsets, d_out_avail, d_out_nbytes, sums,
+				   (uint64_t *)scr, d_seg_info, next_chunk, (const uint8_t *)blk);
+		LDA_HIP_TRY(hipGetLastError(), LIBDEFLATE_AMD_NO_DEVICE);
+		return LIBDEFLATE_AMD_OK;
+	}
+	if (!pl.split) {
+		hipLaunchKernelGGL(lda_deflate_fused_kernel, dim3((unsigned)pl.grid),
+				   dim3(LDA_DEFLATE_THREADS), lds, st, (uint64_t)n, format,
+				   c->level, lv.depth, lv.nice, lv.mode, (const uint8_t *)d_in,
+				   d_in_offsets, d_in_nbytes, (uint8_t *)d_out,
+				   d_out_offsets, d_out_avail, d_out_nbytes, sums,
+				   (uint64_t *)scr, d_seg_info, next_chunk, (const uint8_t *)blk,
+				   (const uint32_t *)NULL, (const uint32_t *)NULL);
+		LDA_HIP_TRY(hipGetLastError(), LIBDEFLATE_AMD_NO_DEVICE);
+		return LIBDEFLATE_AMD_OK;
+	}
+	uint32_t *tok = (uint32_t *)(scr + pl.tok_at), *bd = (uint32_t *)(scr + pl.blk_at);
+	for (size_t k = 0; k < pl.nslices; k++) {
+		const size_t lo = k * pl.per_slice, nk = std::min(pl.per_slice, n - lo);
+		const uint32_t *sk = sums ? sums + lo : NULL;
+		const uint32_t *gk = d_seg_info ? d_seg_info + lo : NULL;
+		hipLaunchKernelGGL(lda_deflate_batch_kernel, dim3((unsigned)std::min(nk, pl.grid)),
+				   dim3(LDA_DEFLATE_THREADS), lds, st, (uint64_t)nk, format,
+				   c->level, lv.depth, lv.nice, lv.mode, (const uint8_t *)d_in,
+				   d_in_offsets + lo, d_in_nbytes + lo, (uint8_t *)d_out,
+				   d_out_offsets + lo, d_out_avail + lo, d_out_nbytes + lo, sk,
+				   (uint64_t *)scr, gk, next_chunk + k, (const uint8_t *)NULL,
+				   tok, bd, pl.tok_stride, pl.blk_stride, next_chunk + 2 * pl.nslices + k);
+		LDA_HIP_TRY(hipGetLastError(), LIBDEFLATE_AMD_NO_DEVICE);
+		hipLaunchKernelGGL(lda_deflate_entropy_kernel, dim3((unsigned)nk),
+				   dim3(LDA_DEFLATE_ENTROPY_THREADS), lda_deflate_entropy_lds_bytes(),
+				   st, (uint64_t)nk, format, c->level, (const uint8_t *)d_in,
+				   d_in_offsets + lo, d_in_nbytes + lo, (uint8_t *)d_out,
+				   d_out_offsets + lo, d_out_avail + lo, d_out_nbytes + lo, sk, gk,
+				   (const uint32_t *)tok, (const uint32_t *)bd, pl.tok_stride,
+				   pl.blk_stride);
+		LDA_HIP_TRY(hipGetLastError(), LIBDEFLATE_AMD_NO_DEVICE);
+		hipLaunchKernelGGL(lda_deflate_fused_kernel, dim3((unsigned)std::min(nk, pl.grid)),
+				   dim3(LDA_DEFLATE_THREADS), lds, st, (uint64_t)nk, format,
+				   c->level, lv.depth, lv.nice, lv.mode, (const uint8_t *)d_in,
+				   d_in_offsets + lo, d_in_nbytes + lo, (uint8_t *)d_out,
+				   d_out_offsets + lo, d_out_avail + lo, d_out_nbytes + lo, sk,
+				   (uint64_t *)scr, gk, next_chunk + pl.nslices + k,
+				   (const uint8_t *)NULL, (const uint32_t *)bd,
+				   (const uint32_t *)(next_chunk + 2 * pl.nslices + k));
+		LDA_HIP_TRY(hipGetLastError(), LIBDEFLATE_AMD_NO_DEVICE);
+	}
 	return LIBDEFLATE_AMD_OK;
 }
 
@@ -385,11 +474,7 @@
 		size_t max_nk = 0;
 		for (size_t k = 0; k < ns; k++)
 			max_nk = bounds[k + 1] - bounds[k] > max_nk ? bounds[k + 1] - bounds[k] : max_nk;
-		const bool small = max_in <= lda_deflate_small_max() && c->level <= 9 &&
-				   !env_cfg().no_small;
-		const size_t grid_max = (size_t)device_ctx()->num_cus * (small ? lda_deflate_small_wgs() : 1);
-		const size_t grid = max_nk < grid_max ? max_nk : grid_max;
-		if (!c->scratch.reserve(grid * lda_deflate_seq_words() * 8 + 16 + max_nk * 4))
+		if (!c->scratch.reserve(plan_batch(c, max_nk, max_in, false, false).total))
 			return LIBDEFLATE_AMD_OOM;
 	}
 	uint64_t *h_back = (uint64_t *)c->meta.ensure((n + ncmp) * 8);
@@ -525,6 +610,7 @@
 	const size_t tile = lda_deflate_tile();
 	const size_t D = dict_window();
 	const size_t nseg = n ? (n + S - 1) / S : 1;
+	const size_t seg_bound = S + (D + tile - 1) / tile * tile;
 	const size_t slot = align_up(libdeflate_deflate_compress_bound(c, S) + 32, 16);
 	const dict_shape dsh = shape_dict(c->level, dict ? dict_nbytes : 0);
 	const size_t pre = dict && n ? dsh.pre_len : 0;
@@ -557,8 +643,8 @@
 		return 0;
 	}
 	{
-		const size_t g = std::min<size_t>(std::min(per_slice, nseg), (size_t)ctx->num_cus);
-		if (!c->scratch.reserve(g * lda_deflate_seq_words() * 8 + 16 + std::min(per_slice, nseg) * 4)) {
+		if (!c->scratch.reserve(plan_batch(c, std::min(per_slice, nseg), seg_bound, true,
+						   false).total)) {
 			complain("libdeflate_*_compress (device memory)", LIBDEFLATE_AMD_OOM);
 			return 0;
 		}
@@ -638,7 +724,7 @@
 		int rc = compress_batch_impl(c, LIBDEFLATE_AMD_DEFLATE, nk, st, d_desc + lo,
 					     d_desc + nseg + lo, st, d_desc + 2 * nseg + lo,
 					     d_desc + 3 * nseg + lo, d_desc + 4 * nseg + lo, s_comp,
-					     d_seg + lo);
+					     d_seg + lo, seg_bound);
 		if (rc == LIBDEFLATE_AMD_OK && ftr)
 			rc = format == LIBDEFLATE_AMD_GZIP ?
 				libdeflate_amd_crc32_batch(nk, st, d_desc + 5 * nseg + lo,
diff --git a/libdeflate_amd/csrc/kernels.h b/libdeflate_amd/csrc/kernels.h
--- a/libdeflate_amd/csrc/kernels.h
+++ b/libdeflate_amd/csrc/kernels.h
@@ -50,6 +50,18 @@
 			    uint64_t *actual_out);
 
 #define LDA_DEFLATE_THREADS 1024
+#define LDA_BLK_TOK0 0
+#define LDA_BLK_NTOK 1
+#define LDA_BLK_START 2
+#define LDA_BLK_END 3
+#define LDA_BLK_FLAGS 4
+#define LDA_BLK_STORED 2u
+#define LDA_BLK_FREQ 8
+#define LDA_BLK_WORDS (LDA_BLK_FREQ + 320)
+#define LDA_BLK_OVERFLOW 0xFFFFFFFFu
+#define LDA_BLK_FUSED 0xFFFFFFFEu
+#define LDA_BLK_LIST(n) (((n) + 15) / 16 * 16)
+#define LDA_BLK_HDR_WORDS(n) (2 * LDA_BLK_LIST(n))
 extern "C" __global__ void
 lda_deflate_batch_kernel(uint64_t n_chunks, int format, int level,
 			 uint32_t depth, uint32_t nice, uint32_t mode,
@@ -58,7 +70,30 @@
 			 const uint64_t *out_offsets, const uint64_t *out_avail,
 			 uint64_t *out_nbytes, const uint32_t *sums,
 			 uint64_t *seq_scratch, const uint32_t *seg_info,
-			 uint32_t *next_chunk, const uint8_t *dict_pre);
+			 uint32_t *next_chunk, const uint8_t *dict_pre,
+			 uint32_t *tok_buf, uint32_t *blk_buf, uint32_t tok_stride,
+			 uint32_t blk_stride, uint32_t *fused_cnt);
+extern "C" __global__ void
+lda_deflate_fused_kernel(uint64_t n_chunks, int format, int level,
+			 uint32_t depth, uint32_t nice, uint32_t mode,
+			 const uint8_t *in_base, const uint64_t *in_offsets,
+			 const uint64_t *in_nbytes, uint8_t *out_base,
+			 const uint64_t *out_offsets, const uint64_t *out_avail,
+			 uint64_t *out_nbytes, const uint32_t *sums,
+			 uint64_t *seq_scratch, const uint32_t *seg_info,
+			 uint32_t *next_chunk, const uint8_t *dict_pre,
+			 const uint32_t *blk_buf, const uint32_t *fused_cnt);
+#define LDA_DEFLATE_ENTROPY_THREADS 256
+extern "C" __global__ void
+lda_deflate_entropy_kernel(uint64_t n_chunks, int format, int level,
+			   const uint8_t *in_base, const uint64_t *in_offsets,
+			   const uint64_t *in_nbytes, uint8_t *out_base,
+			   const uint64_t *out_offsets, const uint64_t *out_avail,
+			   uint64_t *out_nbytes, const uint32_t *sums,
+			   const uint32_t *seg_info, const uint32_t *tok_buf,
+			   const uint32_t *blk_buf, uint32_t tok_stride,
+			   uint32_t blk_stride);
+extern "C" size_t lda_deflate_entropy_lds_bytes(void);
 extern "C" __global__ void
 lda_deflate_opt_kernel(uint64_t n_chunks, int format, int level,
 		       uint32_t depth, uint32_t nice, uint32_t mode,
```
